# spaceandtimefdn/blitzar

Measured on NVIDIA H100. Metric: MSM throughput (scalar*point terms/sec), ristretto255, n=2^20 per GPU, higher is better.
Workload: dtype u32 limbs (integer modular arithmetic)

## Files before the change

### blitzar_b200/api.py

```python
import ctypes as C
import os

import numpy as np

_HERE = os.path.dirname(os.path.abspath(__file__))
LIB_PATH = os.path.join(_HERE, "lib", "libblitzar_b200.so")

SXT_CPU_BACKEND, SXT_GPU_BACKEND = 1, 2
SXT_CURVE_RISTRETTO255, SXT_CURVE_BLS_381, SXT_CURVE_BN_254, SXT_CURVE_GRUMPKIN = 0, 1, 2, 3
CURVE_SIZES = {0: (160, 160, 32), 1: (144, 104, 48), 2: (96, 72, 72), 3: (96, 72, 72)}
COMPACT_BYTES = {0: 120, 1: 96, 2: 64, 3: 64}

SXT_SYMBOLS = [
    "sxt_init", "sxt_curve25519_compute_pedersen_commitments",
    "sxt_curve25519_compute_pedersen_commitments_with_generators",
    "sxt_bls12_381_g1_compute_pedersen_commitments_with_generators",
    "sxt_bn254_g1_uncompressed_compute_pedersen_commitments_with_generators",
    "sxt_grumpkin_uncompressed_compute_pedersen_commitments_with_generators",
    "sxt_ristretto255_get_generators", "sxt_curve25519_get_one_commit",
    "sxt_curve25519_prove_inner_product", "sxt_curve25519_verify_inner_product",
    "sxt_multiexp_handle_new", "sxt_multiexp_handle_new_from_file",
    "sxt_multiexp_handle_write_to_file", "sxt_multiexp_handle_free",
    "sxt_fixed_multiexponentiation", "sxt_fixed_packed_multiexponentiation",
    "sxt_fixed_vlen_multiexponentiation", "sxt_prove_sumcheck",
]
B200_SYMBOLS = [
    "b200_set_device", "b200_launch_count", "b200_point_bytes", "b200_malloc", "b200_free",
    "b200_memcpy_h2d", "b200_memcpy_d2h", "b200_synchronize", "b200_event_create",
    "b200_event_record", "b200_event_elapsed_ms", "b200_event_destroy", "b200_commit_device",
    "b200_combine_partials_device", "b200_fixed_msm_device",
    "b200_combine_partials_projective_device", "b200_set_tuning", "b200_profile_accumulate",
    "b200_profile_read", "b200_set_reduce_groups", "b200_stream",
    "b200_synthetic_generators_device", "b200_commit_host_partials",
    "b200_fixed_msm_host_partials", "b200_multiexp_handle_new_device",
    "b200_selftest_lane_arithmetic", "b200_field_op", "b200_selftest_sort",
    "b200_partition_table_device",
    "b200_multiexp_handle_write_partition_table",
    "b200_compute_pedersen_commitments_with_offsets", "b200_commit_device_with_offsets",
    "b200_multiexp_handle_add_partition_table", "b200_multiexp_handle_partition_window",
    "b200_curve25519_prove_inner_products", "b200_curve25519_verify_inner_products",
]


class sxt_config(C.Structure):
    _fields_ = [("backend", C.c_int), ("num_precomputed_generators", C.c_uint64)]


class sxt_sequence_descriptor(C.Structure):
    _fields_ = [("element_nbytes", C.c_uint8), ("n", C.c_uint64), ("data", C.c_void_p),
                ("is_signed", C.c_int)]


_lib = None


def lib():
    global _lib
    if _lib is None:
        if not os.path.exists(LIB_PATH):
            raise RuntimeError(f"{LIB_PATH} is missing: run `python -m blitzar_b200.build` "
                               "(blitzar_b200 has no CPU fallback)")
        L = C.CDLL(LIB_PATH)
        L.sxt_init.restype = C.c_int
        L.sxt_ristretto255_get_generators.restype = C.c_int
        L.sxt_curve25519_get_one_commit.restype = C.c_int
        L.sxt_multiexp_handle_new.restype = C.c_void_p
        L.sxt_multiexp_handle_new_from_file.restype = C.c_void_p
        L.b200_launch_count.restype = C.c_ulonglong
        L.b200_point_bytes.restype = C.c_uint
        L.b200_malloc.restype = C.c_void_p
        L.b200_multiexp_handle_new_device.restype = C.c_void_p
        L.b200_event_create.restype = C.c_void_p
        L.b200_stream.restype = C.c_void_p
        L.b200_event_elapsed_ms.restype = C.c_float
        _lib = L
    return _lib


_initialized = False


def sxt_init(backend=SXT_GPU_BACKEND, num_precomputed_generators=0, device=None):
    global _initialized
    if _initialized:
        return 0
    if device is not None:
        lib().b200_set_device(C.c_int(device))
    cfg = sxt_config(backend, num_precomputed_generators)
    rc = lib().sxt_init(C.byref(cfg))
    if rc == 0:
        _initialized = True
    return rc


def make_descriptors(columns, device_ptrs=None):
    arr = (sxt_sequence_descriptor * max(1, len(columns)))()
    keep = []
    for i, (data, is_signed) in enumerate(columns):
        data = np.ascontiguousarray(data, dtype=np.uint8)
        keep.append(data)
        arr[i].element_nbytes = data.shape[1]
        arr[i].n = data.shape[0]
        if device_ptrs is not None:
            arr[i].data = device_ptrs[i]
        else:
            arr[i].data = data.ctypes.data if data.shape[0] else None
        arr[i].is_signed = int(is_signed)
    return arr, keep


def _ptr(a):
    return C.c_void_p(a.ctypes.data) if a is not None else C.c_void_p(None)


def compute_pedersen_commitments(curve_id, columns, generators=None, offset_generators=0):
    L = lib()
    desc, keep = make_descriptors(columns)
    out = np.zeros((len(columns), CURVE_SIZES[curve_id][2]), dtype=np.uint8)
    num = C.c_uint32(len(columns))
    if curve_id == SXT_CURVE_RISTRETTO255:
        if generators is None:
            L.sxt_curve25519_compute_pedersen_commitments(_ptr(out), num, desc,
                                                          C.c_uint64(offset_generators))
        else:
            L.sxt_curve25519_compute_pedersen_commitments_with_generators(_ptr(out), num, desc,
                                                                          _ptr(generators))
    else:
        fn = {1: L.sxt_bls12_381_g1_compute_pedersen_commitments_with_generators,
              2: L.sxt_bn254_g1_uncompressed_compute_pedersen_commitments_with_generators,
              3: L.sxt_grumpkin_uncompressed_compute_pedersen_commitments_with_generators}[curve_id]
        fn(_ptr(out), num, desc, _ptr(generators))
    return out


def _offsets(offsets, num):
    if offsets is None:
        return None
    offsets = np.ascontiguousarray(offsets, dtype=np.uint64)
    if offsets.shape != (num,):
        raise ValueError(f"offsets must hold one entry per column ({num})")
    return offsets


def compute_pedersen_commitments_with_offsets(curve_id, columns, offsets, generators=None):
    desc, keep = make_descriptors(columns)
    offsets = _offsets(offsets, len(columns))
    out = np.zeros((len(columns), CURVE_SIZES[curve_id][2]), dtype=np.uint8)
    lib().b200_compute_pedersen_commitments_with_offsets(
        C.c_uint(curve_id), _ptr(out), C.c_uint32(len(columns)), desc, _ptr(generators),
        _ptr(offsets))
    return out


def get_generators(num_generators, offset_generators=0):
    out = np.zeros((num_generators, 160), dtype=np.uint8)
    rc = lib().sxt_ristretto255_get_generators(_ptr(out), C.c_uint64(num_generators),
                                               C.c_uint64(offset_generators))
    if rc != 0:
        raise RuntimeError("sxt_ristretto255_get_generators failed")
    return out


def get_one_commit(n):
    out = np.zeros((1, 160), dtype=np.uint8)
    rc = lib().sxt_curve25519_get_one_commit(_ptr(out), C.c_uint64(n))
    if rc != 0:
        raise RuntimeError("sxt_curve25519_get_one_commit failed")
    return out


class MultiexpHandle:

    def __init__(self, curve_id, generators=None, filename=None, device_ptr=None, n=None):
        self.curve_id = curve_id
        if device_ptr is not None:
            self.h = lib().b200_multiexp_handle_new_device(C.c_uint(curve_id),
                                                           C.c_void_p(device_ptr), C.c_uint(n))
        elif filename is not None:
            self.h = lib().sxt_multiexp_handle_new_from_file(C.c_uint(curve_id),
                                                             filename.encode())
        else:
            generators = np.ascontiguousarray(generators, dtype=np.uint8)
            self.h = lib().sxt_multiexp_handle_new(C.c_uint(curve_id), _ptr(generators),
                                                   C.c_uint(generators.shape[0]))

    def write_to_file(self, filename):
        lib().sxt_multiexp_handle_write_to_file(C.c_void_p(self.h), filename.encode())

    def write_partition_table(self, filename, window_width=0):
        lib().b200_multiexp_handle_write_partition_table(C.c_void_p(self.h), filename.encode(),
                                                         C.c_uint(window_width))

    def add_partition_table(self, window_width=0):
        return int(lib().b200_multiexp_handle_add_partition_table(C.c_void_p(self.h),
                                                                  C.c_uint(window_width)))

    @property
    def partition_window(self):
        return int(lib().b200_multiexp_handle_partition_window(C.c_void_p(self.h)))

    def free(self):
        if self.h:
            lib().sxt_multiexp_handle_free(C.c_void_p(self.h))
            self.h = None

    def _res(self, num_outputs):
        return np.zeros((num_outputs, CURVE_SIZES[self.curve_id][0]), dtype=np.uint8)

    def fixed_multiexponentiation(self, element_num_bytes, num_outputs, n, scalars):
        res = self._res(num_outputs)
        scalars = np.ascontiguousarray(scalars, dtype=np.uint8)
        lib().sxt_fixed_multiexponentiation(_ptr(res), C.c_void_p(self.h),
                                            C.c_uint(element_num_bytes), C.c_uint(num_outputs),
                                            C.c_uint(n), _ptr(scalars))
        return res

    def fixed_packed_multiexponentiation(self, output_bit_table, n, scalars):
        num_outputs = len(output_bit_table)
        res = self._res(num_outputs)
        bt = (C.c_uint * num_outputs)(*output_bit_table)
        scalars = np.ascontiguousarray(scalars, dtype=np.uint8)
        lib().sxt_fixed_packed_multiexponentiation(_ptr(res), C.c_void_p(self.h), bt,
                                                   C.c_uint(num_outputs), C.c_uint(n),
                                                   _ptr(scalars))
        return res

    def fixed_vlen_multiexponentiation(self, output_bit_table, output_lengths, scalars):
        num_outputs = len(output_bit_table)
        res = self._res(num_outputs)
        bt = (C.c_uint * num_outputs)(*output_bit_table)
        ol = (C.c_uint * num_outputs)(*output_lengths)
        scalars = np.ascontiguousarray(scalars, dtype=np.uint8)
        lib().sxt_fixed_vlen_multiexponentiation(_ptr(res), C.c_void_p(self.h), bt, ol,
                                                 C.c_uint(num_outputs), _ptr(scalars))
        return res


class DeviceBuffer:
    def __init__(self, nbytes=None, host=None):
        if host is not None:
            host = np.ascontiguousarray(host)
            nbytes = host.nbytes
        self.nbytes = nbytes
        self.ptr = lib().b200_malloc(C.c_uint64(max(nbytes, 16)))
        if host is not None and nbytes:
            lib().b200_memcpy_h2d(C.c_void_p(self.ptr), _ptr(host), C.c_uint64(nbytes))

    def to_host(self, shape=None, dtype=np.uint8):
        out = np.zeros(self.nbytes, dtype=np.uint8)
        lib().b200_memcpy_d2h(_ptr(out), C.c_void_p(self.ptr), C.c_uint64(self.nbytes))
        out = out.view(dtype)
        return out.reshape(shape) if shape is not None else out

    def free(self):
        if self.ptr:
            lib().b200_free(C.c_void_p(self.ptr))
            self.ptr = None


class Event:
    def __init__(self):
        self.e = lib().b200_event_create()

    def record(self):
        lib().b200_event_record(C.c_void_p(self.e))

    def elapsed_ms(self, stop):
        return float(lib().b200_event_elapsed_ms(C.c_void_p(self.e), C.c_void_p(stop.e)))


def commit_device(curve_id, columns_shape, scalar_ptrs, generators_ptr, out_commit_ptr=None,
                  out_partial_ptr=None, offset_generators=0):
    num = len(columns_shape)
    arr = (sxt_sequence_descriptor * max(1, num))()
    for i, (n, nbytes, is_signed) in enumerate(columns_shape):
        arr[i].element_nbytes = nbytes
        arr[i].n = n
        arr[i].data = scalar_ptrs[i]
        arr[i].is_signed = int(is_signed)
    lib().b200_commit_device(C.c_uint(curve_id), C.c_void_p(out_commit_ptr),
                             C.c_void_p(out_partial_ptr), C.c_uint32(num), arr,
                             C.c_void_p(generators_ptr), C.c_uint64(offset_generators))


def commit_device_with_offsets(curve_id, columns_shape, scalar_ptrs, generators_ptr, offsets,
                               out_commit_ptr=None, out_partial_ptr=None):
    num = len(columns_shape)
    arr = (sxt_sequence_descriptor * max(1, num))()
    for i, (n, nbytes, is_signed) in enumerate(columns_shape):
        arr[i].element_nbytes = nbytes
        arr[i].n = n
        arr[i].data = scalar_ptrs[i]
        arr[i].is_signed = int(is_signed)
    offsets = _offsets(offsets, num)
    lib().b200_commit_device_with_offsets(C.c_uint(curve_id), C.c_void_p(out_commit_ptr),
                                          C.c_void_p(out_partial_ptr), C.c_uint32(num), arr,
                                          C.c_void_p(generators_ptr), _ptr(offsets))


def selftest_lane_arithmetic(warps=64, seed=1):
    lib().b200_selftest_lane_arithmetic.restype = C.c_uint
    return int(lib().b200_selftest_lane_arithmetic(C.c_uint(warps), C.c_uint(seed)))


FIELD_LIMBS = {0: 8, 1: 12, 2: 8, 3: 8, 4: 8, 5: 10}
FIELD_OPS = {name: code for code, name in enumerate([
    "add", "sub", "neg", "dbl", "mul", "mul_ref", "sqr", "mul_lat", "canonical", "is_negative",
    "invert", "pow22523", "from_radix51", "to_radix51", "sqrt_ratio_m1", "invert_eea", "from_mont",
    "to_mont", "lexicographically_largest", "carry1", "sub2p", "sub4p", "slice", "gather"])}
_BINARY_OPS = {"add", "sub", "mul", "mul_ref", "mul_lat", "sqrt_ratio_m1", "sub2p", "sub4p"}


def field_op_shape(field, op):
    n = FIELD_LIMBS[field]
    a = {"from_radix51": 10, "slice": 8}.get(op, n)
    out = {"is_negative": 1, "lexicographically_largest": 1, "to_radix51": 10,
           "sqrt_ratio_m1": n + 1, "gather": 8}.get(op, n)
    return a, (n if op in _BINARY_OPS else 0), out


def call_field_op(entry, field, op, a, b=None):
    wa, wb, wout = field_op_shape(field, op)
    a = np.ascontiguousarray(a, dtype=np.uint32).reshape(-1, wa)
    n = a.shape[0]
    if wb:
        b = np.ascontiguousarray(b, dtype=np.uint32).reshape(n, wb)
    out = np.zeros((n, wout), dtype=np.uint32)
    entry.restype = C.c_uint
    rc = entry(C.c_uint(field), C.c_uint(FIELD_OPS[op]), C.c_uint64(n), _ptr(a),
               _ptr(b if wb else None), _ptr(out))
    if rc == 0xFFFFFFFF:
        raise ValueError(f"field {field} does not offer {op}")
    return out


def field_op(field, op, a, b=None):
    return call_field_op(lib().b200_field_op, field, op, a, b)


def selftest_sort(columns_shape, scalar_ptrs, window_bits=0):
    num = len(columns_shape)
    arr = (sxt_sequence_descriptor * max(1, num))()
    for i, (n, nbytes, is_signed) in enumerate(columns_shape):
        arr[i].element_nbytes = nbytes
        arr[i].n = n
        arr[i].data = scalar_ptrs[i]
        arr[i].is_signed = int(is_signed)
    lib().b200_selftest_sort.restype = C.c_uint
    return int(lib().b200_selftest_sort(arr, C.c_uint(num), C.c_uint(window_bits)))


def synthetic_generators_device(curve_id, out_ptr, n, first=0, projective=False):
    lib().b200_synthetic_generators_device(C.c_uint(curve_id), C.c_void_p(out_ptr), C.c_uint64(n),
                                           C.c_uint64(first), C.c_int(1 if projective else 0))


def partition_table_bytes(curve_id, n, window_width):
    return -(-n // window_width) * (COMPACT_BYTES[curve_id] << window_width)


def partition_table_device(curve_id, out_ptr, gens_ptr, n, window_width=0):
    lib().b200_partition_table_device(C.c_uint(curve_id), C.c_void_p(out_ptr), C.c_void_p(gens_ptr),
                                      C.c_uint64(n), C.c_uint(window_width))


def synthetic_generators(curve_id, n, first=0, projective=False):
    stride = CURVE_SIZES[curve_id][0 if (projective or curve_id == 0) else 1]
    buf = DeviceBuffer(n * stride)
    synthetic_generators_device(curve_id, buf.ptr, n, first, projective)
    out = buf.to_host((n, stride))
    buf.free()
    return out


def commit_host_partials(curve_id, columns, generators, out_partial_ptr, offset_generators=0):
    desc, keep = make_descriptors(columns)
    lib().b200_commit_host_partials(C.c_uint(curve_id), C.c_void_p(out_partial_ptr),
                                    C.c_uint32(len(columns)), desc, _ptr(generators),
                                    C.c_uint64(offset_generators))


def fixed_msm_device(handle, out_res_ptr, out_partial_ptr, element_num_bytes, num_outputs, n,
                     scalars_ptr, bit_table=None, lengths=None):
    mode, bt, ol = 0, None, None
    if bit_table is not None:
        if len(bit_table) != num_outputs or (lengths is not None and len(lengths) != num_outputs):
            raise ValueError(f"bit_table and lengths must hold one entry per output ({num_outputs})")
        mode = 1 if lengths is None else 2
        bt = (C.c_uint * num_outputs)(*bit_table)
        ol = None if lengths is None else (C.c_uint * num_outputs)(*lengths)
    elif lengths is not None:
        raise ValueError("lengths need a bit_table")
    lib().b200_fixed_msm_device(C.c_void_p(out_res_ptr), C.c_void_p(out_partial_ptr),
                                C.c_void_p(handle.h), C.c_int(mode), C.c_uint(element_num_bytes),
                                bt, ol, C.c_uint(num_outputs), C.c_uint(n),
                                C.c_void_p(scalars_ptr))


def fixed_msm_host_partials(handle, out_partial_ptr, element_num_bytes, num_outputs, n, scalars):
    lib().b200_fixed_msm_host_partials(C.c_void_p(out_partial_ptr), C.c_void_p(handle.h),
                                       C.c_int(0), C.c_uint(element_num_bytes), None, None,
                                       C.c_uint(num_outputs), C.c_uint(n), _ptr(scalars))


def combine_partials_projective_device(curve_id, out_ptr, partials_ptr, num_parts, count):
    lib().b200_combine_partials_projective_device(C.c_uint(curve_id), C.c_void_p(out_ptr),
                                                  C.c_void_p(partials_ptr), C.c_uint32(num_parts),
                                                  C.c_uint32(count))


def synchronize():
    lib().b200_synchronize()


def launch_count():
    return int(lib().b200_launch_count())


def profile_accumulate(enable):
    lib().b200_profile_accumulate(C.c_int(1 if enable else 0))


def profile_read():
    ms, cnt = C.c_float(0), C.c_uint(0)
    lib().b200_profile_read(C.byref(ms), C.byref(cnt))
    return float(ms.value), int(cnt.value)


def set_tuning(window_bits=0, chunk1=0, chunkn=0):
    lib().b200_set_tuning(C.c_uint(window_bits), C.c_uint(chunk1), C.c_uint(chunkn))


def combine_partials_device(curve_id, out_ptr, partials_ptr, num_parts, count):
    lib().b200_combine_partials_device(C.c_uint(curve_id), C.c_void_p(out_ptr),
                                       C.c_void_p(partials_ptr), C.c_uint32(num_parts),
                                       C.c_uint32(count))


def point_bytes(curve_id):
    return int(lib().b200_point_bytes(C.c_uint(curve_id)))


def set_reduce_groups(g1=0, gn=0):
    lib().b200_set_reduce_groups(C.c_uint(g1), C.c_uint(gn))


def stream_ptr():
    return int(lib().b200_stream())


def prove_inner_product(transcript, a, b, generators_offset=0):
    n = a.shape[0]
    rounds = max(0, (n - 1).bit_length())
    lv = np.zeros((max(rounds, 1), 32), dtype=np.uint8)
    rv = np.zeros((max(rounds, 1), 32), dtype=np.uint8)
    ap = np.zeros(32, dtype=np.uint8)
    a = np.ascontiguousarray(a, dtype=np.uint8)
    b = np.ascontiguousarray(b, dtype=np.uint8)
    lib().sxt_curve25519_prove_inner_product(_ptr(lv), _ptr(rv), _ptr(ap), _ptr(transcript),
                                             C.c_uint64(n), C.c_uint64(generators_offset),
                                             _ptr(a), _ptr(b))
    return lv[:rounds], rv[:rounds], ap


def verify_inner_product(transcript, b, product, a_commit, l_vector, r_vector, ap_value,
                         generators_offset=0):
    n = b.shape[0]
    b = np.ascontiguousarray(b, dtype=np.uint8)
    lv = np.ascontiguousarray(l_vector if len(l_vector) else np.zeros((1, 32), np.uint8))
    rv = np.ascontiguousarray(r_vector if len(r_vector) else np.zeros((1, 32), np.uint8))
    lib().sxt_curve25519_verify_inner_product.restype = C.c_int
    return int(lib().sxt_curve25519_verify_inner_product(
        _ptr(transcript), C.c_uint64(n), C.c_uint64(generators_offset), _ptr(b),
        _ptr(np.ascontiguousarray(product)), _ptr(np.ascontiguousarray(a_commit)), _ptr(lv),
        _ptr(rv), _ptr(np.ascontiguousarray(ap_value))))


def _ipa_batch_inputs(vectors, offsets):
    n = np.array([v.shape[0] for v in vectors], dtype=np.uint64)
    offs = np.zeros(len(vectors), np.uint64) if offsets is None else \
        np.ascontiguousarray(offsets, dtype=np.uint64)
    if offs.shape != n.shape:
        raise ValueError("one generators offset per proof")
    flat = np.ascontiguousarray(np.concatenate([np.asarray(v, np.uint8).reshape(-1, 32)
                                                for v in vectors])) if len(vectors) else \
        np.zeros((1, 32), np.uint8)
    rounds = [max(0, (int(m) - 1).bit_length()) for m in n]
    return n, offs, flat, rounds


def prove_inner_products(transcripts, a_list, b_list, offsets=None):
    return call_prove_inner_products(lib().b200_curve25519_prove_inner_products, transcripts,
                                     a_list, b_list, offsets)


def verify_inner_products(transcripts, b_list, products, a_commits, l_list, r_list, ap_values,
                          offsets=None):
    lib().b200_curve25519_verify_inner_products.restype = C.c_uint32
    return call_verify_inner_products(lib().b200_curve25519_verify_inner_products, transcripts,
                                      b_list, products, a_commits, l_list, r_list, ap_values,
                                      offsets)


def call_prove_inner_products(entry, transcripts, a_list, b_list, offsets=None):
    if len(a_list) != len(b_list) or any(a.shape[0] != b.shape[0] for a, b in zip(a_list, b_list)):
        raise ValueError("a_list and b_list must hold vectors of equal lengths")
    if transcripts.shape != (len(a_list), 203) or not transcripts.flags.c_contiguous:
        raise ValueError("transcripts must be a contiguous uint8 [P, 203] array")
    n, offs, a, rounds = _ipa_batch_inputs(a_list, offsets)
    _, _, b, _ = _ipa_batch_inputs(b_list, offsets)
    nk = sum(rounds)
    lv = np.zeros((max(nk, 1), 32), dtype=np.uint8)
    rv = np.zeros((max(nk, 1), 32), dtype=np.uint8)
    ap = np.zeros((max(len(a_list), 1), 32), dtype=np.uint8)
    entry(C.c_uint32(len(a_list)), _ptr(lv), _ptr(rv), _ptr(ap), _ptr(transcripts), _ptr(n),
          _ptr(offs), _ptr(a), _ptr(b))
    out, k0 = [], 0
    for p, k in enumerate(rounds):
        out.append((lv[k0:k0 + k], rv[k0:k0 + k], ap[p]))
        k0 += k
    return out


def call_verify_inner_products(entry, transcripts, b_list, products, a_commits, l_list, r_list,
                               ap_values, offsets=None):
    P = len(b_list)
    if transcripts.shape != (P, 203) or not transcripts.flags.c_contiguous:
        raise ValueError("transcripts must be a contiguous uint8 [P, 203] array")
    n, offs, b, _ = _ipa_batch_inputs(b_list, offsets)
    lrs = [np.concatenate([np.asarray(v, np.uint8).reshape(-1, 32) for v in vs] +
                          [np.zeros((1, 32), np.uint8)]) for vs in (l_list, r_list)]
    results = np.zeros(max(P, 1), dtype=np.int32)
    entry(C.c_uint32(P), _ptr(results), _ptr(transcripts), _ptr(n), _ptr(offs), _ptr(b),
          _ptr(np.ascontiguousarray(products, np.uint8)),
          _ptr(np.ascontiguousarray(a_commits, np.uint8)), _ptr(np.ascontiguousarray(lrs[0])),
          _ptr(np.ascontiguousarray(lrs[1])), _ptr(np.ascontiguousarray(ap_values, np.uint8)))
    return results[:P]
```

### blitzar_b200/csrc/api.cu

```cuda
#include <algorithm>
#include <cctype>
#include <cstdint>
#include <cstdio>
#include <cstdlib>
#include <cstring>
#include <condition_variable>
#include <functional>
#include <mutex>
#include <thread>
#include <memory>
#include <string>
#include <vector>

#include "engine_api.cuh"

using namespace b200;

namespace {

struct State {
  bool initialized = false;
  int device = -1;
  cudaStream_t stream = nullptr;
  cudaStream_t copy_stream = nullptr;
  cudaStream_t tail_stream = nullptr;
  cudaEvent_t range_events[16] = {};
  cudaEvent_t alloc_event = nullptr;
  void* builtin = nullptr;
  uint64_t num_builtin = 0;
  unsigned builtin_window_bits = 0, builtin_windows = 0;
  MsmOptions opt;
};
State g_state;
EngineCtx ctx_of(const State& st) {
  EngineCtx c{st.stream, g_state.opt, st.builtin, st.num_builtin};
  c.builtin_window_bits = st.builtin_window_bits;
  c.builtin_windows = st.builtin_windows;
  static const bool tail_on = [] {
    const char* env = std::getenv("BLITZAR_B200_TAIL_STREAM");
    return env != nullptr && std::atoi(env) != 0;
  }();
  if (tail_on)
    c.tail = st.tail_stream;
  if (const char* env = std::getenv("BLITZAR_B200_GROUP_ENTRIES"))
    c.opt.max_group_entries = std::strtoull(env, nullptr, 10);
  if (const char* env = std::getenv("BLITZAR_B200_UNIFORM_ADD"))
    c.opt.uniform_add = (u32)std::atoi(env);
  if (const char* env = std::getenv("BLITZAR_B200_LANE_TAIL"))
    c.opt.lane_tail = (u32)std::atoi(env);
  if (const char* env = std::getenv("BLITZAR_B200_SCATTER_WM"))
    c.opt.scatter_window_major = (u32)std::atoi(env);
  if (const char* env = std::getenv("BLITZAR_B200_SORT"))
    c.opt.sort_path = (u32)std::atoi(env);
  if (const char* env = std::getenv("BLITZAR_B200_NORMALIZE_GENS"))
    c.opt.normalize_gens = (u32)std::atoi(env);
  if (const char* env = std::getenv("BLITZAR_B200_PAIR_LEVELS"))
    c.opt.pair_levels = std::atoi(env);
  if (const char* env = std::getenv("BLITZAR_B200_PAIR_BATCH"))
    c.opt.pair_batch = (u32)std::atoi(env);
  if (const char* env = std::getenv("BLITZAR_B200_TABLE_POLICY"))
    c.opt.table_policy = (u32)std::atoi(env);
  if (const char* env = std::getenv("BLITZAR_B200_PARTITION_POLICY"))
    c.partition_policy = (u32)std::atoi(env);
  return c;
}
EngineCtx ctx() { return ctx_of(g_state); }
std::mutex g_mutex;

void init_device_state(State& st) {
  B200_CUDA(cudaSetDevice(st.device));
  B200_CUDA(cudaStreamCreateWithFlags(&st.stream, cudaStreamNonBlocking));
  B200_CUDA(cudaStreamCreateWithFlags(&st.copy_stream, cudaStreamNonBlocking));
  int prio_low = 0, prio_high = 0;
  B200_CUDA(cudaDeviceGetStreamPriorityRange(&prio_low, &prio_high));
  B200_CUDA(cudaStreamCreateWithPriority(&st.tail_stream, cudaStreamNonBlocking, prio_high));
  for (auto& e : st.range_events)
    B200_CUDA(cudaEventCreateWithFlags(&e, cudaEventDisableTiming));
  B200_CUDA(cudaEventCreateWithFlags(&st.alloc_event, cudaEventDisableTiming));
  cudaMemPool_t pool;
  B200_CUDA(cudaDeviceGetDefaultMemPool(&pool, st.device));
  uint64_t threshold = UINT64_MAX;
  B200_CUDA(cudaMemPoolSetAttribute(pool, cudaMemPoolAttrReleaseThreshold, &threshold));
}

void ensure_device() {
  if (g_state.stream)
    return;
  int count = 0;
  cudaError_t e = cudaGetDeviceCount(&count);
  if (e != cudaSuccess || count == 0)
    die("no supported GPUs found (this library has no CPU fallback)", __FILE__, __LINE__);
  if (g_state.device < 0) {
    const char* env = std::getenv("BLITZAR_B200_DEVICE");
    if (env)
      g_state.device = std::atoi(env);
    else
      B200_CUDA(cudaGetDevice(&g_state.device));
  }
  init_device_state(g_state);
}

unsigned choose_table_window(uint64_t n, size_t gen_bytes) {
  if (const char* env = std::getenv("BLITZAR_B200_TABLE_WINDOW")) {
    const int c = std::atoi(env);
    if (c <= 0)
      return 0;
    const unsigned cc = (unsigned)std::min(22, std::max(8, c));
    return (uint64_t)(256 / cc + 1) * n < (1ull << 31) ? cc : 0;
  }
  size_t free_b = 0, total_b = 0;
  B200_CUDA(cudaMemGetInfo(&free_b, &total_b));
  return table_window_bits(n, gen_bytes, 0.4 * (double)free_b);
}

void make_builtin_table(State& st, uint64_t np) {
  const CurveVTable& V = kVTableEd25519;
  const unsigned c = choose_table_window(np, V.gen_bytes);
  const unsigned windows = c ? 256 / c + 1 : 1;
  B200_CUDA(cudaMalloc(&st.builtin, (size_t)np * windows * V.gen_bytes));
  EngineCtx cx = ctx_of(st);
  launch_builtin_generators(cx, st.builtin, 0, np);
  V.build_table(cx, st.builtin, np, c, windows);
  stream_sync(st.stream);
  st.num_builtin = np;
  st.builtin_window_bits = c;
  st.builtin_windows = windows;
}

void require_init(const char* fn) {
  if (!g_state.initialized) {
    std::fprintf(stderr, "blitzar_b200: backend uninitialized in `%s`\n", fn);
    std::abort();
  }
  B200_CUDA(cudaSetDevice(g_state.device));
}
struct Entry {
  std::lock_guard<std::mutex> lock{g_mutex};
  explicit Entry(const char* fn) { require_init(fn); }
};


class HostStager {
public:
  static HostStager& get() {
    static thread_local HostStager s;
    return s;
  }
  void copy(void* dst_dev, const void* src_host, size_t bytes, cudaStream_t sc) {
    if (bytes == 0)
      return;
    cudaPointerAttributes attr;
    bool pinned = cudaPointerGetAttributes(&attr, src_host) == cudaSuccess &&
                  (attr.type == cudaMemoryTypeHost || attr.type == cudaMemoryTypeManaged);
    cudaGetLastError();
    static const bool enabled = [] {
      const char* env = std::getenv("BLITZAR_B200_STAGER");
      return env == nullptr || std::atoi(env) != 0;
    }();
    if (!enabled || pinned || bytes < (1u << 20)) {
      B200_CUDA(cudaMemcpyAsync(dst_dev, src_host, bytes, cudaMemcpyHostToDevice, sc));
      return;
    }
    init();
    const unsigned char* src = static_cast<const unsigned char*>(src_host);
    unsigned char* dst = static_cast<unsigned char*>(dst_dev);
    for (size_t off = 0; off < bytes; off += kChunk) {
      const size_t len = std::min(kChunk, bytes - off);
      const int slot = next_++ % kSlots;
      B200_CUDA(cudaEventSynchronize(done_[slot]));
      parallel_memcpy(staging_[slot], src + off, len);
      B200_CUDA(cudaMemcpyAsync(dst + off, staging_[slot], len, cudaMemcpyHostToDevice, sc));
      B200_CUDA(cudaEventRecord(done_[slot], sc));
    }
  }

private:
  static constexpr size_t kChunk = 8u << 20;
  static constexpr int kSlots = 4;
  const int kWorkers = [] {
    const char* env = std::getenv("BLITZAR_B200_STAGER_THREADS");
    const int v = env ? std::atoi(env) : 4;
    return std::max(1, std::min(32, v));
  }();
  unsigned char* staging_[kSlots] = {};
  cudaEvent_t done_[kSlots] = {};
  unsigned next_ = 0;
  bool ready_ = false;
  std::vector<std::thread> workers_;
  std::mutex m_;
  std::condition_variable cv_work_, cv_done_;
  struct Job {
    void* d;
    const void* s;
    size_t n;
  };
  std::vector<Job> jobs_;
  int pending_ = 0;
  bool stop_ = false;

  void init() {
    if (ready_)
      return;
    for (int i = 0; i < kSlots; ++i) {
      B200_CUDA(cudaHostAlloc((void**)&staging_[i], kChunk, cudaHostAllocDefault));
      B200_CUDA(cudaEventCreateWithFlags(&done_[i], cudaEventDisableTiming));
    }
    for (int w = 0; w < kWorkers - 1; ++w)
      workers_.emplace_back([this] { worker(); });
    ready_ = true;
  }
  void worker() {
    for (;;) {
      Job j;
      {
        std::unique_lock<std::mutex> lk(m_);
        cv_work_.wait(lk, [this] { return stop_ || !jobs_.empty(); });
        if (stop_ && jobs_.empty())
          return;
        j = jobs_.back();
        jobs_.pop_back();
      }
      std::memcpy(j.d, j.s, j.n);
      {
        std::lock_guard<std::mutex> lk(m_);
        if (--pending_ == 0)
          cv_done_.notify_all();
      }
    }
  }
  void parallel_memcpy(void* d, const void* s, size_t n) {
    const size_t slice = (n + kWorkers - 1) / kWorkers;
    size_t own = std::min(slice, n);
    {
      std::lock_guard<std::mutex> lk(m_);
      for (size_t off = own; off < n; off += slice) {
        jobs_.push_back(Job{(char*)d + off, (const char*)s + off, std::min(slice, n - off)});
        ++pending_;
      }
    }
    cv_work_.notify_all();
    std::memcpy(d, s, own);
    std::unique_lock<std::mutex> lk(m_);
    cv_done_.wait(lk, [this] { return pending_ == 0; });
  }
  ~HostStager() {
    {
      std::lock_guard<std::mutex> lk(m_);
      stop_ = true;
    }
    cv_work_.notify_all();
    for (auto& t : workers_)
      t.join();
    for (int i = 0; i < kSlots; ++i) {
      if (staging_[i])
        cudaFreeHost(staging_[i]);
      if (done_[i])
        cudaEventDestroy(done_[i]);
    }
  }
};

struct RangeWaitState {
  uint64_t n;
  uint32_t num_ranges;
  int skew;
  const State* st;
  uint32_t uploaded;
  std::function<void(uint32_t)> upload;
};
void wait_for_range(void* user, uint64_t begin, uint64_t end) {
  auto* w = static_cast<RangeWaitState*>(user);
  for (uint32_t r = 0; r < w->num_ranges; ++r) {
    const uint64_t rb = range_begin(w->n, r, w->num_ranges, w->skew);
    const uint64_t re = range_begin(w->n, r + 1, w->num_ranges, w->skew);
    if (rb < end && begin < re) {
      while (w->uploaded <= std::min(r + 1, w->num_ranges - 1))
        w->upload(w->uploaded++);
      B200_CUDA(cudaStreamWaitEvent(w->st->stream, w->st->range_events[r], 0));
    }
  }
}

void commit_on(const State& st, unsigned curve_id, void* commitments, uint32_t num,
               const sxt_sequence_descriptor* d, const void* generators,
               uint64_t offset_generators, void* out_partials_dev = nullptr,
               const uint64_t* offsets = nullptr) {
  const CurveVTable& V = curve_vtable(curve_id);
  StageRange nvtx("commit (host buffers)");
  cudaStream_t s = st.stream, sc = st.copy_stream;
  const uint64_t n = check_descriptors(d, num);
  size_t total_scalar_bytes = 0;
  for (uint32_t i = 0; i < num; ++i)
    total_scalar_bytes += (size_t)d[i].n * d[i].element_nbytes + 32;
  const GenLayout layout(d, num, offsets);
  DevBuf<unsigned char> raw_gens(generators ? layout.total * V.abi_gen_bytes : 1, s);
  DevBuf<unsigned char> scal(total_scalar_bytes, s);
  DevBuf<unsigned char> out((size_t)num * V.abi_commit_bytes, s);
  std::vector<sxt_sequence_descriptor> dd(d, d + num);
  std::vector<size_t> col_off(num);
  size_t off = 0;
  for (uint32_t i = 0; i < num; ++i) {
    col_off[i] = off;
    dd[i].data = scal.p + off;
    off += ((size_t)d[i].n * d[i].element_nbytes + 31) & ~(size_t)31;
  }
  uint32_t num_ranges = (uint32_t)std::min<uint64_t>(n >> 18, num == 1 ? 8 : 4);
  if (num == 1 && n >= (1ull << 18))
    num_ranges = std::max(num_ranges, 2u);
  if (curve_id != SXT_CURVE_RISTRETTO255)
    num_ranges = (uint32_t)std::min<uint64_t>(n >> 21, 4);
  num_ranges = std::max(num_ranges, 1u);
  if (const char* env = std::getenv("BLITZAR_B200_RANGES"))
    num_ranges = (uint32_t)std::max(1, std::min(16, std::atoi(env)));
  int skew = 0;
  if (const char* env = std::getenv("BLITZAR_B200_RANGE_SKEW"))
    skew = std::atoi(env);
  B200_CUDA(cudaEventRecord(st.alloc_event, s));
  B200_CUDA(cudaStreamWaitEvent(sc, st.alloc_event, 0));
  static const bool trace = std::getenv("BLITZAR_B200_TRACE") != nullptr;
  std::vector<cudaEvent_t> tev;
  auto mark = [&](cudaStream_t on) {
    if (!trace)
      return;
    cudaEvent_t e;
    B200_CUDA(cudaEventCreate(&e));
    B200_CUDA(cudaEventRecord(e, on));
    tev.push_back(e);
  };
  mark(sc);
  auto upload = [&](uint32_t r) {
    const uint64_t b = range_begin(n, r, num_ranges, skew), e = range_begin(n, r + 1, num_ranges, skew);
    for (uint32_t i = 0; i < num; ++i) {
      const uint64_t lo = std::min<uint64_t>(b, d[i].n), hi = std::min<uint64_t>(e, d[i].n);
      HostStager::get().copy(scal.p + col_off[i] + lo * d[i].element_nbytes,
                             d[i].data + lo * d[i].element_nbytes,
                             (hi - lo) * d[i].element_nbytes, sc);
    }
    if (generators)
      for (const GenLayout::Piece& p : layout.needed(b, e))
        HostStager::get().copy(raw_gens.p + p.pos * V.abi_gen_bytes,
                               static_cast<const unsigned char*>(generators) + p.src * V.abi_gen_bytes,
                               p.count * V.abi_gen_bytes, sc);
    B200_CUDA(cudaEventRecord(st.range_events[r], sc));
    mark(sc);
  };
  B200_LOG(2, "commit: curve %u, %u columns, n = %llu, device %d, %u upload pieces, generators %s",
           curve_id, num, (unsigned long long)n, st.device, num_ranges,
           generators ? "from the caller" : "built in");
  RangeWaitState w{n, num_ranges, skew, &st, 0, upload};
  EngineCtx cx = ctx_of(st);
  cx.opt.range_skew = skew;
  if (offsets)
    V.commit_device_offsets(cx, out_partials_dev ? nullptr : out.p, out_partials_dev, num, dd.data(),
                            generators ? raw_gens.p : nullptr, offsets, true, num_ranges,
                            &wait_for_range, &w);
  else
    V.commit_device(cx, out_partials_dev ? nullptr : out.p, out_partials_dev, num, dd.data(),
                    generators ? raw_gens.p : nullptr, offset_generators, num_ranges, &wait_for_range,
                    &w);
  mark(s);
  if (!out_partials_dev)
    copy_d2h(commitments, out.p, (size_t)num * V.abi_commit_bytes, s);
  stream_sync(s);
  if (trace) {
    std::fprintf(stderr, "blitzar_b200 trace: n=%llu cols=%u pieces=%u:", (unsigned long long)n, num,
                 num_ranges);
    for (size_t i = 1; i < tev.size(); ++i) {
      float ms = 0;
      B200_CUDA(cudaEventElapsedTime(&ms, tev[0], tev[i]));
      std::fprintf(stderr, " %s%.3f", i + 1 == tev.size() ? "compute_done=" : "upload=", ms);
    }
    std::fprintf(stderr, " ms\n");
    for (auto e : tev)
      cudaEventDestroy(e);
  }
}

class Worker {
public:
  State st;
  explicit Worker(int device) {
    st.device = device;
    th_ = std::thread([this] { run(); });
  }
  void submit(std::function<void()> f) {
    {
      std::lock_guard<std::mutex> lk(m_);
      task_ = std::move(f);
      busy_ = true;
    }
    cv_.notify_all();
  }
  void wait() {
    std::unique_lock<std::mutex> lk(m_);
    cv_.wait(lk, [this] { return !busy_; });
  }
  ~Worker() {
    {
      std::lock_guard<std::mutex> lk(m_);
      stop_ = true;
    }
    cv_.notify_all();
    if (th_.joinable())
      th_.join();
  }

private:
  std::thread th_;
  std::mutex m_;
  std::condition_variable cv_;
  std::function<void()> task_;
  bool busy_ = false, stop_ = false;
  void run() {
    B200_CUDA(cudaSetDevice(st.device));
    for (;;) {
      std::function<void()> f;
      {
        std::unique_lock<std::mutex> lk(m_);
        cv_.wait(lk, [this] { return stop_ || task_; });
        if (stop_ && !task_)
          return;
        f = std::move(task_);
        task_ = nullptr;
      }
      f();
      {
        std::lock_guard<std::mutex> lk(m_);
        busy_ = false;
      }
      cv_.notify_all();
    }
  }
};
std::vector<std::unique_ptr<Worker>> g_workers;

struct Gather {
  void* buf = nullptr;
  size_t capacity = 0;
  void* ensure(size_t bytes) {
    if (bytes > capacity) {
      if (buf) {
        B200_CUDA(cudaStreamSynchronize(g_state.stream));
        B200_CUDA(cudaFree(buf));
      }
      capacity = std::max<size_t>(bytes, 1u << 16);
      B200_CUDA(cudaMalloc(&buf, capacity));
    }
    return buf;
  }
};
Gather g_gather;

size_t range_parts(uint64_t n) {
  static const uint64_t min_terms = [] {
    const char* env = std::getenv("BLITZAR_B200_MIN_SHARD_TERMS");
    return env ? std::strtoull(env, nullptr, 10) : (1ull << 15);
  }();
  return (size_t)std::max<uint64_t>(1, std::min<uint64_t>(g_workers.size() + 1, n / std::max<uint64_t>(min_terms, 1)));
}
State& state_of(size_t part) { return part == 0 ? g_state : g_workers[part - 1]->st; }
template <class F> void on_devices(size_t parts, F f) {
  for (size_t p = 1; p < parts; ++p)
    g_workers[p - 1]->submit([=] { f(p); });
  f(0);
  for (size_t p = 1; p < parts; ++p)
    g_workers[p - 1]->wait();
  B200_CUDA(cudaSetDevice(g_state.device));
}
template <class F>
void sum_over_devices(const CurveVTable& V, size_t parts, uint32_t count, void* sum, F run) {
  const size_t bytes = (size_t)count * V.point_bytes;
  unsigned char* gather = static_cast<unsigned char*>(g_gather.ensure(parts * bytes));
  on_devices(parts, [&](size_t p) {
    const State& st = state_of(p);
    DevBuf<unsigned char> partials(bytes, st.stream);
    run(st, p, partials.p);
    if (p == 0)
      B200_CUDA(cudaMemcpyAsync(gather, partials.p, bytes, cudaMemcpyDeviceToDevice, st.stream));
    else
      B200_CUDA(cudaMemcpyPeerAsync(gather + p * bytes, g_state.device, partials.p, st.device, bytes,
                                    st.stream));
    B200_CUDA(cudaStreamSynchronize(st.stream));
  });
  V.sum_parts(ctx(), gather, (uint32_t)parts, count, sum);
}
void store_to_host(const CurveVTable& V, const void* pts, uint32_t count, bool commit, void* host) {
  cudaStream_t s = g_state.stream;
  const size_t bytes = (size_t)count * (commit ? V.abi_commit_bytes : V.abi_proj_bytes);
  DevBuf<unsigned char> out(bytes, s);
  V.store(ctx(), pts, out.p, count, commit);
  copy_d2h(host, out.p, bytes, s);
  stream_sync(s);
}
void combine_partials(unsigned curve_id, void* out_dev, const void* partials, uint32_t num_parts,
                      uint32_t count, bool commit) {
  const CurveVTable& V = curve_vtable(curve_id);
  DevBuf<unsigned char> sum((size_t)count * V.point_bytes, g_state.stream);
  V.sum_parts(ctx(), partials, num_parts, count, sum.p);
  V.store(ctx(), sum.p, out_dev, count, commit);
}

void commit_host(unsigned curve_id, void* commitments, uint32_t num,
                 const sxt_sequence_descriptor* d, const void* generators,
                 uint64_t offset_generators, const char* fn, void* out_partials_dev = nullptr,
                 const uint64_t* offsets = nullptr) {
  if (num == 0)
    return;
  const Entry entry(fn);
  B200_REQUIRE(commitments != nullptr || out_partials_dev != nullptr, "commitments == nullptr");
  const uint64_t n = check_descriptors(d, num);
  if (curve_id != SXT_CURVE_RISTRETTO255)
    B200_REQUIRE(generators != nullptr, "generators == nullptr");
  if (offsets)
    (void)GenLayout(d, num, offsets);
  const CurveVTable& V = curve_vtable(curve_id);
  const size_t stride = V.abi_commit_bytes;
  const size_t devices = g_workers.size() + 1;
  if (devices <= 1 || out_partials_dev) {
    commit_on(g_state, curve_id, commitments, num, d, generators, offset_generators,
              out_partials_dev, offsets);
    return;
  }
  if (num >= devices) {
    const size_t parts = devices;
    std::vector<uint64_t> prefix(num + 1, 0);
    for (uint32_t i = 0; i < num; ++i)
      prefix[i + 1] = prefix[i] + d[i].n * d[i].element_nbytes + 1;
    std::vector<uint32_t> cut(parts + 1, num);
    cut[0] = 0;
    for (size_t p = 1; p < parts; ++p) {
      uint32_t c = cut[p - 1] + 1;
      while (c < num - (parts - p) && prefix[c] * parts < prefix[num] * p)
        ++c;
      cut[p] = c;
    }
    on_devices(parts, [&, curve_id, commitments, d, generators, offset_generators](size_t p) {
      commit_on(state_of(p), curve_id, static_cast<unsigned char*>(commitments) + cut[p] * stride,
                cut[p + 1] - cut[p], d + cut[p], generators, offset_generators, nullptr,
                offsets ? offsets + cut[p] : nullptr);
    });
    return;
  }
  const size_t parts = range_parts(n);
  if (parts <= 1) {
    commit_on(g_state, curve_id, commitments, num, d, generators, offset_generators, nullptr,
              offsets);
    return;
  }
  DevBuf<unsigned char> sum((size_t)num * V.point_bytes, g_state.stream);
  sum_over_devices(V, parts, num, sum.p, [&](const State& st, size_t p, void* partials) {
    const uint64_t lo = n * p / parts, hi = n * (p + 1) / parts;
    std::vector<sxt_sequence_descriptor> dd(d, d + num);
    std::vector<uint64_t> part_offsets(offsets ? num : 0);
    for (uint32_t j = 0; j < num; ++j) {
      auto& c = dd[j];
      const uint64_t b = std::min<uint64_t>(lo, c.n), e = std::min<uint64_t>(hi, c.n);
      c.data = c.data ? c.data + b * c.element_nbytes : nullptr;
      c.n = e - b;
      if (offsets)
        part_offsets[j] = offsets[j] + b;
    }
    const unsigned char* g = static_cast<const unsigned char*>(generators);
    if (offsets)
      commit_on(st, curve_id, nullptr, num, dd.data(), g, 0, partials, part_offsets.data());
    else
      commit_on(st, curve_id, nullptr, num, dd.data(), g ? g + lo * V.abi_gen_bytes : nullptr,
                offset_generators + lo, partials);
  });
  store_to_host(V, sum.p, num, true, commitments);
}

struct HandleSet {
  unsigned curve_id = 0, n = 0;
  std::vector<Handle*> shards;
  std::vector<unsigned> first;
};
HandleSet* handle_of(const sxt_multiexp_handle* handle) {
  B200_REQUIRE(handle != nullptr, "null handle");
  return reinterpret_cast<HandleSet*>(const_cast<sxt_multiexp_handle*>(handle));
}

Handle* shard_new(const State& st, unsigned curve_id, const void* generators, unsigned n,
                  bool device_resident, unsigned compact_window, size_t compact_bytes) {
  const CurveVTable& V = curve_vtable(curve_id);
  cudaStream_t s = st.stream;
  Handle* h = new Handle{curve_id, n, nullptr};
  h->window_bits = choose_table_window(n, V.gen_bytes);
  h->windows = h->window_bits ? 256 / h->window_bits + 1 : 1;
  B200_CUDA(cudaMalloc(&h->gens, (size_t)(n ? n : 1) * h->windows * V.gen_bytes));
  if (n) {
    B200_REQUIRE(generators != nullptr, "generators == nullptr");
    const EngineCtx cx = ctx_of(st);
    if (compact_window) {
      DevBuf<unsigned char> raw(compact_bytes, s);
      HostStager::get().copy(raw.p, generators, compact_bytes, s);
      V.ingest_compact_table(cx, raw.p, compact_window, h->gens, n);
    } else if (device_resident) {
      V.ingest_projective(cx, generators, h->gens, n);
    } else {
      DevBuf<unsigned char> raw((size_t)n * V.abi_proj_bytes, s);
      HostStager::get().copy(raw.p, generators, (size_t)n * V.abi_proj_bytes, s);
      V.ingest_projective(cx, raw.p, h->gens, n);
    }
    V.build_table(cx, h->gens, n, h->window_bits, h->windows);
    stream_sync(s);
  }
  return h;
}

unsigned partition_window(unsigned w) {
  if (w == 0) {
    const char* env = std::getenv("BLITZAR_PARTITION_WINDOW_WIDTH");
    w = env ? (unsigned)std::strtoul(env, nullptr, 10) : 16u;
  }
  B200_REQUIRE(w >= 1 && w <= 24, "partition table window width must be in 1..24");
  return w;
}
uint64_t partition_chunk_groups(const CurveVTable& V, unsigned w) {
  uint64_t bytes = 64ull << 20;
  if (const char* env = std::getenv("BLITZAR_B200_PTABLE_CHUNK_BYTES"))
    bytes = std::strtoull(env, nullptr, 10);
  return std::max<uint64_t>(1, bytes / ((uint64_t)V.abi_compact_bytes << w));
}
void drop_partition_table(const State& st, Handle* h) {
  stream_sync(st.stream);
  B200_CUDA(cudaFree(h->ptable));
  h->ptable = nullptr;
  h->ptable_w = 0;
  h->ptable_groups = 0;
}
bool shard_add_partition_table(const State& st, Handle* h, unsigned w) {
  const CurveVTable& V = curve_vtable(h->curve_id);
  cudaStream_t s = st.stream;
  drop_partition_table(st, h);
  const uint64_t groups = ((uint64_t)h->n + w - 1) / w;
  if (groups == 0)
    return false;
  size_t free_b = 0, total_b = 0;
  B200_CUDA(cudaMemGetInfo(&free_b, &total_b));
  const double bytes = std::ldexp((double)groups * V.gen_bytes, (int)w);
  if (bytes > 0.4 * (double)free_b)
    return false;
  if (cudaMalloc(&h->ptable, (size_t)bytes) != cudaSuccess) {
    cudaGetLastError();
    h->ptable = nullptr;
    return false;
  }
  const uint64_t step = partition_chunk_groups(V, w);
  for (uint64_t g = 0; g < groups; g += step)
    V.partition_gens(ctx_of(st), h->gens, h->n, w, g, std::min(step, groups - g),
                     static_cast<unsigned char*>(h->ptable) + ((size_t)g << w) * V.gen_bytes);
  stream_sync(s);
  h->ptable_w = w;
  h->ptable_groups = groups;
  return true;
}

unsigned handle_add_partition_table(HandleSet* hs, unsigned window_width) {
  const unsigned w = partition_window(window_width);
  std::vector<char> ok(hs->shards.size(), 0);
  on_devices(hs->shards.size(), [&, hs, w](size_t p) {
    ok[p] = shard_add_partition_table(state_of(p), hs->shards[p], w) ? 1 : 0;
  });
  if (std::find(ok.begin(), ok.end(), 0) == ok.end())
    return w;
  on_devices(hs->shards.size(),
             [hs](size_t p) { drop_partition_table(state_of(p), hs->shards[p]); });
  B200_LOG(1, "partition table of width %u does not fit in 40 %% of the free HBM", w);
  return 0;
}

HandleSet* handle_new(unsigned curve_id, const void* generators, unsigned n,
                      bool device_resident = false, unsigned compact_window = 0) {
  const CurveVTable& V = curve_vtable(curve_id);
  HandleSet* hs = new HandleSet;
  hs->curve_id = curve_id;
  hs->n = n;
  size_t parts = device_resident ? 1 : range_parts(n);
  const unsigned align = compact_window ? compact_window : 1;
  hs->shards.assign(parts, nullptr);
  hs->first.assign(parts + 1, n);
  for (size_t p = 0; p < parts; ++p)
    hs->first[p] = (unsigned)(((uint64_t)n * p / parts) / align * align);
  on_devices(parts, [&, curve_id, generators, device_resident, compact_window](size_t p) {
    const unsigned lo = hs->first[p], cnt = hs->first[p + 1] - lo;
    const unsigned char* g = static_cast<const unsigned char*>(generators);
    size_t off = 0, cbytes = 0;
    if (compact_window) {
      const size_t group_bytes = (size_t)V.abi_compact_bytes << compact_window;
      off = (size_t)(lo / compact_window) * group_bytes;
      cbytes = (size_t)((cnt + compact_window - 1) / compact_window) * group_bytes;
    } else {
      off = (size_t)lo * V.abi_proj_bytes;
    }
    hs->shards[p] = shard_new(state_of(p), curve_id, g ? g + off : nullptr, cnt, device_resident,
                              compact_window, cbytes);
  });
  if (const char* env = std::getenv("BLITZAR_B200_PARTITION_HANDLES"))
    if (std::atoi(env) == 1)
      handle_add_partition_table(hs, 0);
  return hs;
}

struct FixedCall {
  int mode;
  unsigned element_num_bytes;
  const unsigned* bit_table;
  const unsigned* lengths;
  unsigned num_outputs, rows;
  uint64_t row_bytes;
};

void fixed_on(const State& st, void* res, const Handle* h, const FixedCall& c, unsigned lo,
              const uint8_t* scalars, void* out_partials_dev) {
  cudaStream_t s = st.stream;
  const CurveVTable& V = curve_vtable(h->curve_id);
  const unsigned hi = std::min<uint64_t>((uint64_t)lo + h->n, c.rows);
  const unsigned rows = hi > lo ? hi - lo : 0;
  std::vector<unsigned> lens;
  if (c.mode == 2) {
    lens.resize(c.num_outputs);
    for (unsigned j = 0; j < c.num_outputs; ++j)
      lens[j] = c.lengths[j] > lo ? std::min(c.lengths[j] - lo, rows) : 0u;
  }
  const size_t bytes = (size_t)c.row_bytes * rows;
  DevBuf<unsigned char> scal(bytes + 64, s);
  DevBuf<unsigned char> out((size_t)c.num_outputs * V.abi_proj_bytes, s);
  HostStager::get().copy(scal.p, scalars + (size_t)c.row_bytes * lo, bytes, s);
  V.fixed_device(ctx_of(st), out_partials_dev ? nullptr : out.p, out_partials_dev, h, c.mode,
                 c.element_num_bytes, c.bit_table, c.mode == 2 ? lens.data() : nullptr,
                 c.num_outputs, rows, scal.p);
  if (!out_partials_dev)
    copy_d2h(res, out.p, (size_t)c.num_outputs * V.abi_proj_bytes, s);
  stream_sync(s);
}

void fixed_host(void* res, const HandleSet* hs, int mode, unsigned element_num_bytes,
                const unsigned* bit_table, const unsigned* lengths, unsigned num_outputs,
                unsigned n, const uint8_t* scalars, void* out_partials_dev = nullptr) {
  if (num_outputs == 0)
    return;
  FixedCall c{mode, element_num_bytes, bit_table, lengths, num_outputs, n,
              fixed_row_bytes(mode, element_num_bytes, bit_table, num_outputs)};
  if (mode == 2) {
    for (unsigned j = 1; j < num_outputs; ++j)
      B200_REQUIRE(lengths[j] >= lengths[j - 1], "output lengths must be sorted in ascending order");
    c.rows = lengths[num_outputs - 1];
  }
  B200_REQUIRE(c.rows <= hs->n, "more scalars than generators in the handle");
  B200_REQUIRE(c.row_bytes * c.rows == 0 || scalars != nullptr, "scalars == nullptr");
  const size_t parts = hs->shards.size();
  if (parts == 1) {
    fixed_on(g_state, res, hs->shards[0], c, 0, scalars, out_partials_dev);
    return;
  }
  const CurveVTable& V = curve_vtable(hs->curve_id);
  auto shard = [&](const State& st, size_t p, void* partials) {
    fixed_on(st, nullptr, hs->shards[p], c, hs->first[p], scalars, partials);
  };
  if (out_partials_dev) {
    sum_over_devices(V, parts, num_outputs, out_partials_dev, shard);
    stream_sync(g_state.stream);
    return;
  }
  DevBuf<unsigned char> sum((size_t)num_outputs * V.point_bytes, g_state.stream);
  sum_over_devices(V, parts, num_outputs, sum.p, shard);
  store_to_host(V, sum.p, num_outputs, false, res);
}

const uint32_t kHandleMagic = 0x44483242u;

}

extern "C" {

int sxt_init(const struct sxt_config* config) {
  std::lock_guard<std::mutex> lock(g_mutex);
  if (config == nullptr)
    die("config input to `sxt_init` is null", __FILE__, __LINE__);
  if (g_state.initialized)
    die("trying to reinitialize the backend in `sxt_init`", __FILE__, __LINE__);
  int backend = config->backend;
  if (const char* env = std::getenv("BLITZAR_BACKEND")) {
    std::string v(env);
    for (auto& ch : v)
      ch = (char)std::tolower(ch);
    if (v == "cpu")
      backend = SXT_CPU_BACKEND;
    else if (v == "gpu")
      backend = SXT_GPU_BACKEND;
    else
      die("invalid BLITZAR_BACKEND value", __FILE__, __LINE__);
  }
  if (backend == SXT_CPU_BACKEND) {
    std::fprintf(stderr, "blitzar_b200: this library provides only the gpu backend "
                         "(SXT_GPU_BACKEND); link the reference libblitzar for the cpu backend\n");
    return 2;
  }
  if (backend != SXT_GPU_BACKEND)
    return 1;
  ensure_device();
  g_state.initialized = true;
  uint64_t np = config->num_precomputed_generators;
  if (np)
    make_builtin_table(g_state, np);
  if (const char* env = std::getenv("BLITZAR_B200_DEVICES")) {
    int want = std::atoi(env), count = 0;
    B200_CUDA(cudaGetDeviceCount(&count));
    const char* shared = std::getenv("BLITZAR_B200_SHARED_DEVICES");
    if (!(shared && std::atoi(shared) != 0))
      want = std::min(want, count);
    for (int k = 1; k < want; ++k) {
      auto w = std::make_unique<Worker>((g_state.device + k) % count);
      Worker* wp = w.get();
      wp->submit([wp, np] {
        init_device_state(wp->st);
        if (np)
          make_builtin_table(wp->st, np);
        wp->st.initialized = true;
      });
      wp->wait();
      g_workers.push_back(std::move(w));
    }
    B200_CUDA(cudaSetDevice(g_state.device));
  }
  return 0;
}

void sxt_curve25519_compute_pedersen_commitments(struct sxt_ristretto255_compressed* commitments,
                                                 uint32_t num_sequences,
                                                 const struct sxt_sequence_descriptor* descriptors,
                                                 uint64_t offset_generators) {
  commit_host(SXT_CURVE_RISTRETTO255, commitments, num_sequences, descriptors, nullptr,
              offset_generators, "sxt_curve25519_compute_pedersen_commitments");
}
void sxt_curve25519_compute_pedersen_commitments_with_generators(
    struct sxt_ristretto255_compressed* commitments, uint32_t num_sequences,
    const struct sxt_sequence_descriptor* descriptors, const struct sxt_ristretto255* generators) {
  commit_host(SXT_CURVE_RISTRETTO255, commitments, num_sequences, descriptors, generators, 0,
              "sxt_curve25519_compute_pedersen_commitments_with_generators");
}
void sxt_bls12_381_g1_compute_pedersen_commitments_with_generators(
    struct sxt_bls12_381_g1_compressed* commitments, uint32_t num_sequences,
    const struct sxt_sequence_descriptor* descriptors, const struct sxt_bls12_381_g1* generators) {
  commit_host(SXT_CURVE_BLS_381, commitments, num_sequences, descriptors, generators, 0,
              "sxt_bls12_381_g1_compute_pedersen_commitments_with_generators");
}
void sxt_bn254_g1_uncompressed_compute_pedersen_commitments_with_generators(
    struct sxt_bn254_g1* commitments, uint32_t num_sequences,
    const struct sxt_sequence_descriptor* descriptors, const struct sxt_bn254_g1* generators) {
  commit_host(SXT_CURVE_BN_254, commitments, num_sequences, descriptors, generators, 0,
              "sxt_bn254_g1_uncompressed_compute_pedersen_commitments_with_generators");
}
void sxt_grumpkin_uncompressed_compute_pedersen_commitments_with_generators(
    struct sxt_grumpkin* commitments, uint32_t num_sequences,
    const struct sxt_sequence_descriptor* descriptors, const struct sxt_grumpkin* generators) {
  commit_host(SXT_CURVE_GRUMPKIN, commitments, num_sequences, descriptors, generators, 0,
              "sxt_grumpkin_uncompressed_compute_pedersen_commitments_with_generators");
}

int sxt_ristretto255_get_generators(struct sxt_ristretto255* generators, uint64_t num_generators,
                                    uint64_t offset_generators) {
  const Entry entry("sxt_ristretto255_get_generators");
  if (num_generators == 0)
    return 0;
  if (generators == nullptr)
    return 1;
  const CurveVTable& V = kVTableEd25519;
  cudaStream_t s = g_state.stream;
  DevBuf<unsigned char> out(num_generators * V.abi_proj_bytes, s);
  V.synth_generators(ctx(), out.p, num_generators, offset_generators, true);
  copy_d2h(generators, out.p, num_generators * V.abi_proj_bytes, s);
  stream_sync(s);
  return 0;
}

int sxt_curve25519_get_one_commit(struct sxt_ristretto255* one_commit, uint64_t n) {
  const Entry entry("sxt_curve25519_get_one_commit");
  B200_REQUIRE(one_commit != nullptr, "one_commit == nullptr");
  B200_REQUIRE(n < (1ull << 31), "n too large");
  const CurveVTable& V = kVTableEd25519;
  cudaStream_t s = g_state.stream;
  DevBuf<unsigned char> ones(n + 32, s);
  B200_CUDA(cudaMemsetAsync(ones.p, 1, n + 32, s));
  sxt_sequence_descriptor d{1, n, ones.p, 0};
  DevBuf<unsigned char> pt(V.point_bytes, s);
  V.commit_device(ctx(), nullptr, pt.p, 1, &d, nullptr, 0, 1, nullptr, nullptr);
  store_to_host(V, pt.p, 1, false, one_commit);
  return 0;
}

void sxt_curve25519_prove_inner_product(struct sxt_ristretto255_compressed* l_vector,
                                        struct sxt_ristretto255_compressed* r_vector,
                                        struct sxt_curve25519_scalar* ap_value,
                                        struct sxt_transcript* transcript, uint64_t n,
                                        uint64_t generators_offset,
                                        const struct sxt_curve25519_scalar* a_vector,
                                        const struct sxt_curve25519_scalar* b_vector) {
  const Entry entry("sxt_curve25519_prove_inner_product");
  B200_REQUIRE(transcript != nullptr, "transcript must not be null");
  B200_REQUIRE(ap_value != nullptr, "ap_value must not be null");
  B200_REQUIRE(b_vector != nullptr && a_vector != nullptr, "a_vector / b_vector must not be null");
  B200_REQUIRE(n > 0, "a_vector and b_vector lengths must be greater than zero");
  B200_REQUIRE(n == 1 || (l_vector != nullptr && r_vector != nullptr),
               "l_vector and r_vector must not be null when n > 1");
  B200_REQUIRE(n < (1ull << 30), "n too large");
  ipa_prove(ctx(), reinterpret_cast<uint8_t*>(l_vector), reinterpret_cast<uint8_t*>(r_vector),
            ap_value->bytes, transcript->bytes, n, generators_offset,
            reinterpret_cast<const uint8_t*>(a_vector), reinterpret_cast<const uint8_t*>(b_vector));
}
int sxt_curve25519_verify_inner_product(struct sxt_transcript* transcript, uint64_t n,
                                        uint64_t generators_offset,
                                        const struct sxt_curve25519_scalar* b_vector,
                                        const struct sxt_curve25519_scalar* product,
                                        const struct sxt_ristretto255* a_commit,
                                        const struct sxt_ristretto255_compressed* l_vector,
                                        const struct sxt_ristretto255_compressed* r_vector,
                                        const struct sxt_curve25519_scalar* ap_value) {
  const Entry entry("sxt_curve25519_verify_inner_product");
  B200_REQUIRE(transcript != nullptr, "transcript must not be null");
  B200_REQUIRE(ap_value != nullptr && product != nullptr && a_commit != nullptr &&
                   b_vector != nullptr,
               "ap_value / product / a_commit / b_vector must not be null");
  B200_REQUIRE(n > 0, "b_vector length must be greater than zero");
  B200_REQUIRE(n == 1 || (l_vector != nullptr && r_vector != nullptr),
               "l_vector and r_vector must not be null when n > 1");
  B200_REQUIRE(n < (1ull << 30), "n too large");
  return ipa_verify(ctx(), transcript->bytes, n, generators_offset,
                    reinterpret_cast<const uint8_t*>(b_vector), product->bytes,
                    reinterpret_cast<const uint8_t*>(a_commit),
                    reinterpret_cast<const uint8_t*>(l_vector),
                    reinterpret_cast<const uint8_t*>(r_vector), ap_value->bytes);
}
namespace {
unsigned ipa_rounds(uint64_t n) {
  unsigned k = 0;
  while ((1ull << k) < n)
    ++k;
  return k;
}
void check_ipa_batch(uint32_t num_proofs, const uint64_t* n, const uint64_t* generators_offsets,
                     const void* transcripts, bool prover) {
  B200_REQUIRE(transcripts != nullptr && n != nullptr && generators_offsets != nullptr,
               "transcripts / n / generators_offsets must not be null");
  uint64_t arena = 0;
  for (uint32_t p = 0; p < num_proofs; ++p) {
    B200_REQUIRE(n[p] > 0, "a_vector and b_vector lengths must be greater than zero");
    B200_REQUIRE(n[p] < (1ull << 30), "n too large");
    const unsigned k = ipa_rounds(n[p]);
    arena += prover ? (1ull << k) + 1 : (1ull << k) + 2 * k + 3;
  }
  B200_REQUIRE(arena < (1ull << 31), "proofs of the batch need too many generators for one call");
}
bool any_rounds(uint32_t num_proofs, const uint64_t* n) {
  for (uint32_t p = 0; p < num_proofs; ++p)
    if (n[p] > 1)
      return true;
  return false;
}
}

void b200_curve25519_prove_inner_products(
    uint32_t num_proofs, struct sxt_ristretto255_compressed* l_vectors,
    struct sxt_ristretto255_compressed* r_vectors, struct sxt_curve25519_scalar* ap_values,
    struct sxt_transcript* transcripts, const uint64_t* n, const uint64_t* generators_offsets,
    const struct sxt_curve25519_scalar* a_vectors, const struct sxt_curve25519_scalar* b_vectors) {
  const Entry entry("b200_curve25519_prove_inner_products");
  if (num_proofs == 0)
    return;
  check_ipa_batch(num_proofs, n, generators_offsets, transcripts, true);
  B200_REQUIRE(ap_values != nullptr, "ap_values must not be null");
  B200_REQUIRE(b_vectors != nullptr && a_vectors != nullptr, "a_vectors / b_vectors must not be null");
  B200_REQUIRE(!any_rounds(num_proofs, n) || (l_vectors != nullptr && r_vectors != nullptr),
               "l_vectors and r_vectors must not be null when some n > 1");
  ipa_prove_batch(ctx(), num_proofs, reinterpret_cast<uint8_t*>(l_vectors),
                  reinterpret_cast<uint8_t*>(r_vectors), ap_values->bytes, transcripts->bytes, n,
                  generators_offsets, reinterpret_cast<const uint8_t*>(a_vectors),
                  reinterpret_cast<const uint8_t*>(b_vectors));
}
uint32_t b200_curve25519_verify_inner_products(
    uint32_t num_proofs, int* results, struct sxt_transcript* transcripts, const uint64_t* n,
    const uint64_t* generators_offsets, const struct sxt_curve25519_scalar* b_vectors,
    const struct sxt_curve25519_scalar* products, const struct sxt_ristretto255* a_commits,
    const struct sxt_ristretto255_compressed* l_vectors,
    const struct sxt_ristretto255_compressed* r_vectors,
    const struct sxt_curve25519_scalar* ap_values) {
  const Entry entry("b200_curve25519_verify_inner_products");
  if (num_proofs == 0)
    return 0;
  check_ipa_batch(num_proofs, n, generators_offsets, transcripts, false);
  B200_REQUIRE(results != nullptr, "results must not be null");
  B200_REQUIRE(ap_values != nullptr && products != nullptr && a_commits != nullptr &&
                   b_vectors != nullptr,
               "ap_values / products / a_commits / b_vectors must not be null");
  B200_REQUIRE(!any_rounds(num_proofs, n) || (l_vectors != nullptr && r_vectors != nullptr),
               "l_vectors and r_vectors must not be null when some n > 1");
  return ipa_verify_batch(ctx(), num_proofs, results, transcripts->bytes, n, generators_offsets,
                          reinterpret_cast<const uint8_t*>(b_vectors), products->bytes,
                          reinterpret_cast<const uint8_t*>(a_commits),
                          reinterpret_cast<const uint8_t*>(l_vectors),
                          reinterpret_cast<const uint8_t*>(r_vectors), ap_values->bytes);
}

void sxt_prove_sumcheck(void*, void*, unsigned, const struct sumcheck_descriptor*, void*, void*) {
  die("sxt_prove_sumcheck is not provided by blitzar_b200 (MSM hot path only)", __FILE__,
      __LINE__);
}

struct sxt_multiexp_handle* sxt_multiexp_handle_new(unsigned curve_id, const void* generators,
                                                    unsigned n) {
  const Entry entry("sxt_multiexp_handle_new");
  return reinterpret_cast<sxt_multiexp_handle*>(handle_new(curve_id, generators, n));
}

void sxt_multiexp_handle_free(struct sxt_multiexp_handle* handle) {
  if (!handle)
    return;
  std::lock_guard<std::mutex> lock(g_mutex);
  HandleSet* hs = handle_of(handle);
  on_devices(hs->shards.size(), [hs](size_t p) {
    drop_partition_table(state_of(p), hs->shards[p]);
    B200_CUDA(cudaFree(hs->shards[p]->gens));
    delete hs->shards[p];
  });
  delete hs;
}

void sxt_multiexp_handle_write_to_file(const struct sxt_multiexp_handle* handle,
                                       const char* filename) {
  const Entry entry("sxt_multiexp_handle_write_to_file");
  const HandleSet* h = handle_of(handle);
  B200_REQUIRE(filename != nullptr, "null filename");
  const CurveVTable& V = curve_vtable(h->curve_id);
  size_t bytes = (size_t)h->n * V.abi_proj_bytes;
  std::vector<unsigned char> host(bytes);
  on_devices(h->shards.size(), [&, h](size_t p) {
    const State& st = state_of(p);
    const Handle* sh = h->shards[p];
    const size_t sb = (size_t)sh->n * V.abi_proj_bytes;
    DevBuf<unsigned char> out(sb + 16, st.stream);
    V.gens_to_projective(ctx_of(st), sh->gens, out.p, sh->n);
    copy_d2h(host.data() + (size_t)h->first[p] * V.abi_proj_bytes, out.p, sb, st.stream);
    stream_sync(st.stream);
  });
  FILE* f = std::fopen(filename, "wb");
  B200_REQUIRE(f != nullptr, "cannot open handle file for writing");
  uint32_t hdr[4] = {kHandleMagic, 1u, h->curve_id, h->n};
  B200_REQUIRE(std::fwrite(hdr, sizeof(hdr), 1, f) == 1, "short write");
  B200_REQUIRE(bytes == 0 || std::fwrite(host.data(), bytes, 1, f) == 1, "short write");
  std::fclose(f);
}

struct sxt_multiexp_handle* sxt_multiexp_handle_new_from_file(unsigned curve_id,
                                                              const char* filename) {
  const Entry entry("sxt_multiexp_handle_new_from_file");
  B200_REQUIRE(filename != nullptr, "null filename");
  FILE* f = std::fopen(filename, "rb");
  B200_REQUIRE(f != nullptr, "cannot open handle file");
  uint32_t hdr[4] = {0, 0, 0, 0};
  B200_REQUIRE(std::fread(hdr, sizeof(uint32_t), 1, f) == 1, "short handle file");
  if (hdr[0] != kHandleMagic) {
    const unsigned w = hdr[0];
    const size_t esz = curve_vtable(curve_id).abi_compact_bytes;
    B200_REQUIRE(w >= 1 && w <= 24, "not a handle file (bad window width)");
    std::fseek(f, 0, SEEK_END);
    const size_t bytes = (size_t)std::ftell(f) - sizeof(uint32_t);
    std::fseek(f, sizeof(uint32_t), SEEK_SET);
    B200_REQUIRE(bytes % (esz << w) == 0, "partition table size does not match the curve");
    const size_t groups = bytes / (esz << w);
    B200_REQUIRE(groups * w < (1ull << 31), "partition table too large");
    std::vector<unsigned char> host(bytes);
    B200_REQUIRE(bytes == 0 || std::fread(host.data(), bytes, 1, f) == 1, "short handle file");
    std::fclose(f);
    return reinterpret_cast<sxt_multiexp_handle*>(
        handle_new(curve_id, host.data(), (unsigned)(groups * w), false, w));
  }
  B200_REQUIRE(std::fread(hdr + 1, 3 * sizeof(uint32_t), 1, f) == 1, "short handle file");
  B200_REQUIRE(hdr[1] == 1u, "unsupported blitzar_b200 handle file version");
  B200_REQUIRE(hdr[2] == curve_id, "handle file is for another curve");
  size_t bytes = (size_t)hdr[3] * curve_vtable(curve_id).abi_proj_bytes;
  std::vector<unsigned char> host(bytes);
  B200_REQUIRE(bytes == 0 || std::fread(host.data(), bytes, 1, f) == 1, "short handle file");
  std::fclose(f);
  return reinterpret_cast<sxt_multiexp_handle*>(handle_new(curve_id, host.data(), hdr[3]));
}

void sxt_fixed_multiexponentiation(void* res, const struct sxt_multiexp_handle* handle,
                                   unsigned element_num_bytes, unsigned num_outputs, unsigned n,
                                   const uint8_t* scalars) {
  const Entry entry("sxt_fixed_multiexponentiation");
  fixed_host(res, handle_of(handle), 0, element_num_bytes, nullptr, nullptr, num_outputs, n, scalars);
}
void sxt_fixed_packed_multiexponentiation(void* res, const struct sxt_multiexp_handle* handle,
                                          const unsigned* output_bit_table, unsigned num_outputs,
                                          unsigned n, const uint8_t* scalars) {
  const Entry entry("sxt_fixed_packed_multiexponentiation");
  fixed_host(res, handle_of(handle), 1, 0, output_bit_table, nullptr, num_outputs, n, scalars);
}
void sxt_fixed_vlen_multiexponentiation(void* res, const struct sxt_multiexp_handle* handle,
                                        const unsigned* output_bit_table,
                                        const unsigned* output_lengths, unsigned num_outputs,
                                        const uint8_t* scalars) {
  const Entry entry("sxt_fixed_vlen_multiexponentiation");
  fixed_host(res, handle_of(handle), 2, 0, output_bit_table, output_lengths, num_outputs, 0, scalars);
}

void b200_set_device(int device) {
  std::lock_guard<std::mutex> lock(g_mutex);
  B200_REQUIRE(g_state.stream == nullptr, "b200_set_device must precede sxt_init");
  g_state.device = device;
}
unsigned long long b200_launch_count(void) { return LaunchCounter::value(); }
unsigned b200_point_bytes(unsigned curve_id) { return curve_vtable(curve_id).point_bytes; }
void* b200_malloc(uint64_t bytes) {
  const Entry entry("b200_malloc");
  void* p = nullptr;
  B200_CUDA(cudaMalloc(&p, bytes ? bytes : 16));
  return p;
}
void b200_free(void* p) {
  std::lock_guard<std::mutex> lock(g_mutex);
  if (p) {
    B200_CUDA(cudaSetDevice(g_state.device));
    B200_CUDA(cudaStreamSynchronize(g_state.stream));
    B200_CUDA(cudaFree(p));
  }
}
void b200_memcpy_h2d(void* d, const void* h, uint64_t bytes) {
  const Entry entry("b200_memcpy_h2d");
  copy_h2d(d, h, bytes, g_state.stream);
  stream_sync(g_state.stream);
}
void b200_memcpy_d2h(void* h, const void* d, uint64_t bytes) {
  const Entry entry("b200_memcpy_d2h");
  copy_d2h(h, d, bytes, g_state.stream);
  stream_sync(g_state.stream);
}
void* b200_stream(void) {
  require_init("b200_stream");
  return (void*)g_state.stream;
}
void b200_synchronize(void) {
  const Entry entry("b200_synchronize");
  stream_sync(g_state.stream);
}
void* b200_event_create(void) {
  require_init("b200_event_create");
  cudaEvent_t e;
  B200_CUDA(cudaEventCreate(&e));
  return (void*)e;
}
void b200_event_record(void* e) {
  std::lock_guard<std::mutex> lock(g_mutex);
  B200_CUDA(cudaEventRecord((cudaEvent_t)e, g_state.stream));
}
float b200_event_elapsed_ms(void* a, void* b) {
  float ms = 0;
  B200_CUDA(cudaEventSynchronize((cudaEvent_t)b));
  B200_CUDA(cudaEventElapsedTime(&ms, (cudaEvent_t)a, (cudaEvent_t)b));
  return ms;
}
void b200_event_destroy(void* e) { B200_CUDA(cudaEventDestroy((cudaEvent_t)e)); }

void b200_commit_device(unsigned curve_id, void* out_commitments, void* out_partials,
                        uint32_t num_sequences, const struct sxt_sequence_descriptor* descriptors,
                        const void* generators, uint64_t offset_generators) {
  if (num_sequences == 0)
    return;
  const Entry entry("b200_commit_device");
  curve_vtable(curve_id).commit_device(ctx(), out_commitments, out_partials, num_sequences,
                                       descriptors, generators, offset_generators, 1, nullptr,
                                       nullptr);
}
void b200_compute_pedersen_commitments_with_offsets(unsigned curve_id, void* commitments,
                                                    uint32_t num_sequences,
                                                    const struct sxt_sequence_descriptor* descriptors,
                                                    const void* generators, const uint64_t* offsets) {
  commit_host(curve_id, commitments, num_sequences, descriptors, generators, 0,
              "b200_compute_pedersen_commitments_with_offsets", nullptr, offsets);
}
void b200_commit_device_with_offsets(unsigned curve_id, void* out_commitments, void* out_partials,
                                     uint32_t num_sequences,
                                     const struct sxt_sequence_descriptor* descriptors,
                                     const void* generators, const uint64_t* offsets) {
  if (num_sequences == 0)
    return;
  const Entry entry("b200_commit_device_with_offsets");
  const CurveVTable& V = curve_vtable(curve_id);
  if (offsets)
    V.commit_device_offsets(ctx(), out_commitments, out_partials, num_sequences, descriptors,
                            generators, offsets, false, 1, nullptr, nullptr);
  else
    V.commit_device(ctx(), out_commitments, out_partials, num_sequences, descriptors, generators,
                    0, 1, nullptr, nullptr);
}
void b200_commit_host_partials(unsigned curve_id, void* out_partials,
                               uint32_t num_sequences,
                               const struct sxt_sequence_descriptor* descriptors,
                               const void* generators, uint64_t offset_generators) {
  if (num_sequences == 0)
    return;
  const Entry entry("b200_commit_host_partials");
  B200_REQUIRE(out_partials != nullptr, "out_partials == nullptr");
  commit_on(g_state, curve_id, nullptr, num_sequences, descriptors, generators, offset_generators,
            out_partials);
}
void b200_fixed_msm_host_partials(void* out_partials, const struct sxt_multiexp_handle* handle,
                                  int mode, unsigned element_num_bytes,
                                  const unsigned* output_bit_table, const unsigned* output_lengths,
                                  unsigned num_outputs, unsigned n, const uint8_t* scalars) {
  if (num_outputs == 0)
    return;
  const Entry entry("b200_fixed_msm_host_partials");
  const HandleSet* h = handle_of(handle);
  B200_REQUIRE(out_partials != nullptr, "out_partials == nullptr");
  fixed_host(nullptr, h, mode, element_num_bytes, output_bit_table, output_lengths, num_outputs, n,
             scalars, out_partials);
}
struct sxt_multiexp_handle* b200_multiexp_handle_new_device(unsigned curve_id,
                                                            const void* generators_dev,
                                                            unsigned n) {
  const Entry entry("b200_multiexp_handle_new_device");
  return reinterpret_cast<sxt_multiexp_handle*>(handle_new(curve_id, generators_dev, n, true));
}
void b200_combine_partials_device(unsigned curve_id, void* out_commitments, const void* partials,
                                  uint32_t num_parts, uint32_t count) {
  const Entry entry("b200_combine_partials_device");
  combine_partials(curve_id, out_commitments, partials, num_parts, count, true);
}
void b200_combine_partials_projective_device(unsigned curve_id, void* out_res,
                                             const void* partials, uint32_t num_parts,
                                             uint32_t count) {
  const Entry entry("b200_combine_partials_projective_device");
  combine_partials(curve_id, out_res, partials, num_parts, count, false);
}
void b200_fixed_msm_device(void* out_res, void* out_partials,
                           const struct sxt_multiexp_handle* handle, int mode,
                           unsigned element_num_bytes, const unsigned* output_bit_table,
                           const unsigned* output_lengths, unsigned num_outputs, unsigned n,
                           const uint8_t* scalars) {
  if (num_outputs == 0)
    return;
  const Entry entry("b200_fixed_msm_device");
  const HandleSet* hs = handle_of(handle);
  B200_REQUIRE(hs->shards.size() == 1, "device-resident fixed MSM needs a single-device handle");
  const Handle* h = hs->shards[0];
  curve_vtable(h->curve_id).fixed_device(ctx(), out_res, out_partials, h, mode, element_num_bytes,
                                         output_bit_table, output_lengths, num_outputs, n, scalars);
}
void b200_synthetic_generators_device(unsigned curve_id, void* out_generators, uint64_t n,
                                      uint64_t first, int projective) {
  if (n == 0)
    return;
  const Entry entry("b200_synthetic_generators_device");
  B200_REQUIRE(out_generators != nullptr, "out_generators == nullptr");
  curve_vtable(curve_id).synth_generators(ctx(), out_generators, n, first, projective != 0);
}
void b200_partition_table_device(unsigned curve_id, void* out_table_dev, const void* generators_dev,
                                 uint64_t n, unsigned window_width) {
  const Entry entry("b200_partition_table_device");
  const CurveVTable& V = curve_vtable(curve_id);
  const unsigned w = partition_window(window_width);
  if (n == 0)
    return;
  B200_REQUIRE(out_table_dev != nullptr && generators_dev != nullptr,
               "out_table_dev / generators_dev must not be null");
  cudaStream_t s = g_state.stream;
  DevBuf<unsigned char> gens(n * V.gen_bytes, s);
  V.ingest_projective(ctx(), generators_dev, gens.p, n);
  const uint64_t groups = (n + w - 1) / w, step = partition_chunk_groups(V, w);
  const size_t group_bytes = (size_t)V.abi_compact_bytes << w;
  for (uint64_t g = 0; g < groups; g += step)
    V.partition_table(ctx(), gens.p, n, w, g, std::min(step, groups - g),
                      static_cast<unsigned char*>(out_table_dev) + g * group_bytes);
}
void b200_multiexp_handle_write_partition_table(const struct sxt_multiexp_handle* handle,
                                                const char* filename, unsigned window_width) {
  const Entry entry("b200_multiexp_handle_write_partition_table");
  const HandleSet* h = handle_of(handle);
  B200_REQUIRE(filename != nullptr, "null filename");
  const CurveVTable& V = curve_vtable(h->curve_id);
  const unsigned w = partition_window(window_width);
  cudaStream_t s = g_state.stream, sc = g_state.copy_stream;
  DevBuf<unsigned char> gens((size_t)(h->n ? h->n : 1) * V.gen_bytes, s);
  for (size_t p = 0; p < h->shards.size(); ++p) {
    const int device = state_of(p).device;
    const Handle* sh = h->shards[p];
    unsigned char* dst = gens.p + (size_t)h->first[p] * V.gen_bytes;
    const size_t bytes = (size_t)sh->n * V.gen_bytes;
    if (device == g_state.device)
      copy_d2d(dst, sh->gens, bytes, s);
    else if (bytes)
      B200_CUDA(cudaMemcpyPeerAsync(dst, g_state.device, sh->gens, device, bytes, s));
  }
  FILE* f = std::fopen(filename, "wb");
  B200_REQUIRE(f != nullptr, "cannot open partition table file for writing");
  const uint32_t hdr = w;
  B200_REQUIRE(std::fwrite(&hdr, sizeof(hdr), 1, f) == 1, "short write");
  const uint64_t groups = (h->n + w - 1) / w;
  const uint64_t step = std::min<uint64_t>(partition_chunk_groups(V, w), std::max<uint64_t>(groups, 1));
  const size_t group_bytes = (size_t)V.abi_compact_bytes << w, chunk_bytes = step * group_bytes;
  const uint64_t chunks = (groups + step - 1) / step;
  B200_LOG(2, "partition table file: curve %u, n = %u, w = %u, %llu chunks of %llu groups",
           h->curve_id, h->n, w, (unsigned long long)chunks, (unsigned long long)step);
  DevBuf<unsigned char> dev0(chunks ? chunk_bytes : 1, s), dev1(chunks > 1 ? chunk_bytes : 1, s);
  unsigned char* dev[2] = {dev0.p, dev1.p};
  unsigned char* host[2] = {nullptr, nullptr};
  cudaEvent_t built[2], copied[2];
  for (int k = 0; k < 2; ++k) {
    if (chunks > (uint64_t)k)
      B200_CUDA(cudaHostAlloc((void**)&host[k], chunk_bytes, cudaHostAllocDefault));
    B200_CUDA(cudaEventCreateWithFlags(&built[k], cudaEventDisableTiming));
    B200_CUDA(cudaEventCreateWithFlags(&copied[k], cudaEventDisableTiming));
  }
  auto chunk_size = [&](uint64_t i) { return std::min(step, groups - i * step) * group_bytes; };
  for (uint64_t i = 0; i <= chunks; ++i) {
    if (i < chunks) {
      const int k = (int)(i & 1);
      if (i >= 2)
        B200_CUDA(cudaStreamWaitEvent(s, copied[k], 0));
      V.partition_table(ctx(), gens.p, h->n, w, i * step, std::min(step, groups - i * step), dev[k]);
      B200_CUDA(cudaEventRecord(built[k], s));
      B200_CUDA(cudaStreamWaitEvent(sc, built[k], 0));
      copy_d2h(host[k], dev[k], chunk_size(i), sc);
      B200_CUDA(cudaEventRecord(copied[k], sc));
    }
    if (i >= 1) {
      const int k = (int)((i - 1) & 1);
      B200_CUDA(cudaEventSynchronize(copied[k]));
      B200_REQUIRE(std::fwrite(host[k], chunk_size(i - 1), 1, f) == 1, "short write");
    }
  }
  B200_REQUIRE(std::fclose(f) == 0, "short write");
  stream_sync(s);
  for (int k = 0; k < 2; ++k) {
    if (host[k])
      B200_CUDA(cudaFreeHost(host[k]));
    B200_CUDA(cudaEventDestroy(built[k]));
    B200_CUDA(cudaEventDestroy(copied[k]));
  }
}
unsigned b200_multiexp_handle_add_partition_table(struct sxt_multiexp_handle* handle,
                                                  unsigned window_width) {
  const Entry entry("b200_multiexp_handle_add_partition_table");
  return handle_add_partition_table(handle_of(handle), window_width);
}
unsigned b200_multiexp_handle_partition_window(const struct sxt_multiexp_handle* handle) {
  std::lock_guard<std::mutex> lock(g_mutex);
  const HandleSet* hs = handle_of(handle);
  return hs->shards.empty() ? 0u : hs->shards[0]->ptable_w;
}
unsigned b200_selftest_lane_arithmetic(unsigned warps, unsigned seed) {
  const Entry entry("b200_selftest_lane_arithmetic");
  return selftest_lane_arithmetic(ctx(), warps, seed);
}
unsigned b200_field_op(unsigned field, unsigned op, uint64_t n, const uint32_t* a,
                       const uint32_t* b, uint32_t* out) {
  const Entry entry("b200_field_op");
  B200_REQUIRE(n == 0 || (a != nullptr && out != nullptr), "null operand or result array");
  return field_op(ctx(), field, op, n, a, b, out);
}
unsigned b200_selftest_sort(const sxt_sequence_descriptor* columns, unsigned num,
                            unsigned window_bits) {
  const Entry entry("b200_selftest_sort");
  B200_REQUIRE(num == 0 || columns != nullptr, "columns == nullptr");
  B200_REQUIRE(window_bits <= 20, "window_bits in 0..20");
  return selftest_sort(ctx(), columns, num, window_bits);
}
void b200_set_reduce_groups(unsigned g1, unsigned gn) {
  std::lock_guard<std::mutex> lock(g_mutex);
  auto pow2 = [](unsigned v, unsigned dflt) {
    if (v < 2)
      return dflt;
    unsigned p = 2;
    while (p * 2 <= v)
      p *= 2;
    return p;
  };
  g_state.opt.reduce_g1 = pow2(g1, 16u);
  g_state.opt.reduce_gn = pow2(gn, 4u);
}
void b200_profile_accumulate(int enable) {
  std::lock_guard<std::mutex> lock(g_mutex);
  KernelTimer::get().enabled = enable != 0;
}
void b200_profile_read(float* total_ms, unsigned* launches) {
  std::lock_guard<std::mutex> lock(g_mutex);
  KernelTimer::get().read(total_ms, launches);
}
void b200_set_tuning(unsigned window_bits, unsigned chunk1, unsigned chunkn) {
  std::lock_guard<std::mutex> lock(g_mutex);
  g_state.opt.window_bits = window_bits;
  g_state.opt.chunk1 = chunk1;
  g_state.opt.chunkn = chunkn ? chunkn : 8;
}

}
```

### blitzar_b200/csrc/batch_affine.cuh

```cuda
#pragma once
#include "curve.cuh"
#include "runtime.cuh"

namespace b200 {

constexpr u32 kPadIndex = 0x7fffffffu;
B200_HD u64 make_entry(u32 key, u32 gen, bool negate) {
  return ((u64)key << 32) | (u64)((gen << 1) | (negate ? 1u : 0u));
}
B200_HD u64 pad_entry(u32 key) { return make_entry(key, kPadIndex, false); }
B200_HD u32 entry_key(u64 e) { return (u32)(e >> 32); }
B200_HD u32 entry_gen(u64 e) { return (u32)e >> 1; }
B200_HD bool entry_negate(u64 e) { return ((u32)e & 1u) != 0; }

constexpr u32 kBatchGroup = 8;
constexpr u32 kBatchTop = 4;

template <class F> struct BatchUpBody {
  static constexpr int kBlock = 128;
  const typename F::E* vals;
  typename F::E* pre;
  typename F::E* prod;
  u64 n;
  B200_HD void operator()(u64 j) const {
    const u64 b = j * kBatchGroup, e = b + kBatchGroup < n ? b + kBatchGroup : n;
    typename F::E acc = F::one();
    for (u64 i = b; i < e; ++i) {
      pre[i] = acc;
      F::mul(acc, acc, vals[i]);
    }
    prod[j] = acc;
  }
};
template <class F> struct BatchDownBody {
  static constexpr int kBlock = 128;
  typename F::E* vals;
  const typename F::E* pre;
  const typename F::E* prod;
  u64 n;
  B200_HD void operator()(u64 j) const {
    const u64 b = j * kBatchGroup, e = b + kBatchGroup < n ? b + kBatchGroup : n;
    typename F::E inv = prod[j];
    for (u64 i = e; i-- > b;) {
      typename F::E t, v = vals[i];
      F::mul(t, inv, pre[i]);
      F::mul(inv, inv, v);
      vals[i] = t;
    }
  }
};
template <class F> struct BatchTopBody {
  static constexpr int kBlock = 32;
  typename F::E* vals;
  B200_HD void operator()(u64 i) const {
    typename F::E inv;
    F::invert_eea(inv, vals[i]);
    vals[i] = inv;
  }
};
template <class F> inline void batch_invert(stream_t s, typename F::E* vals, u64 n) {
  typedef typename F::E E;
  if (n == 0)
    return;
  if (n <= kBatchTop) {
    launch(BatchTopBody<F>{vals}, n, s);
    return;
  }
  E* pre = (E*)dev_alloc(n * sizeof(E), s);
  const u64 m = (n + kBatchGroup - 1) / kBatchGroup;
  E* prod = (E*)dev_alloc(m * sizeof(E), s);
  launch(BatchUpBody<F>{vals, pre, prod, n}, m, s);
  batch_invert<F>(s, prod, m);
  launch(BatchDownBody<F>{vals, pre, prod, n}, m, s);
  dev_free(prod, s);
  dev_free(pre, s);
}

template <class C> struct PairLevel {
  typedef typename C::F F;
  typedef typename F::E fe;
  typedef typename C::Gen Gen;
  const u64* entries;
  const Gen* gens;
  const Gen* in;
  const u32* m_ptr;
  u32 level;
  u32 B;

  B200_HD u64 valid_pairs() const { return (u64)(*m_ptr) >> (level + 1); }
  B200_HD void load(Gen& a, u64 slot) const {
    if (in) {
      a = in[slot];
      return;
    }
    const u64 ent = entries[slot];
    const u32 idx = entry_gen(ent);
    if (idx == kPadIndex) {
      a.x = F::zero();
      a.y = F::zero();
      return;
    }
    a = gens[idx];
    if (entry_negate(ent) && !C::gen_is_identity(a))
      F::neg(a.y, a.y);
  }
  B200_HD int classify(fe& den, const Gen& a, const Gen& b) const {
    den = F::one();
    if (C::gen_is_identity(b))
      return 1;
    if (C::gen_is_identity(a))
      return 2;
    if (F::equal(a.x, b.x)) {
      fe s;
      F::add(s, a.y, b.y);
      if (F::is_zero(s))
        return 4;
      den = s;
      return 3;
    }
    F::sub(den, b.x, a.x);
    return 0;
  }
};

template <class C> struct PairPass1Body {
  static constexpr int kBlock = 128;
  typedef typename C::F F;
  typedef typename F::E fe;
  PairLevel<C> lv;
  fe* pre;
  fe* totals;
  u64 t0;
  B200_HD void operator()(u64 t) const {
    t += t0;
    const u64 np = lv.valid_pairs();
    const u64 b = t * lv.B, e = b + lv.B < np ? b + lv.B : np;
    fe acc = F::one();
    for (u64 p = b; p < e; ++p) {
      const u32 ia = entry_gen(lv.entries[2 * p]), ib = entry_gen(lv.entries[2 * p + 1]);
      fe den = F::one();
      if (ia != kPadIndex && ib != kPadIndex) {
        const fe xa = lv.gens[ia].x, xb = lv.gens[ib].x;
        if (F::equal(xa, xb) || F::is_zero(xa) || F::is_zero(xb)) {
          typename C::Gen ga, gb;
          lv.load(ga, 2 * p);
          lv.load(gb, 2 * p + 1);
          lv.classify(den, ga, gb);
        } else {
          F::sub(den, xb, xa);
        }
      }
      pre[p] = acc;
      F::mul(acc, acc, den);
    }
    totals[t] = acc;
  }
};

template <class C> struct PairPass2Body {
  static constexpr int kBlock = 128;
  static constexpr int kMinBlocks = C::F::N > 8 ? 2 : 3;
  typedef typename C::F F;
  typedef typename F::E fe;
  typedef typename C::Gen Gen;
  PairLevel<C> lv;
  const fe* pre;
  const fe* totals;
  Gen* out;
  fe* pre_next;
  fe* totals_next;
  u32 descending;
  u64 t0;
  B200_HD void add_pair(Gen& r, const Gen& x, const Gen& y, int kind, const fe& inv) const {
    if (kind == 1) {
      r = x;
    } else if (kind == 2) {
      r = y;
    } else if (kind == 4) {
      r.x = F::zero();
      r.y = F::zero();
    } else {
      fe num, lam, l2, dx;
      if (kind == 3) {
        fe xx;
        F::sqr(xx, x.x);
        F::add(num, xx, xx);
        F::add(num, num, xx);
      } else {
        F::sub(num, y.y, x.y);
      }
      F::mul(lam, num, inv);
      F::sqr(l2, lam);
      F::sub(l2, l2, x.x);
      F::sub(r.x, l2, y.x);
      F::sub(dx, x.x, r.x);
      F::mul(l2, lam, dx);
      F::sub(r.y, l2, x.y);
    }
  }
  B200_HD void operator()(u64 t) const {
    t += t0;
    const u64 np = lv.valid_pairs();
    const u64 b = t * lv.B, e = b + lv.B < np ? b + lv.B : np;
    if (b >= e) {
      if (pre_next)
        totals_next[t] = F::one();
      return;
    }
    const u64 cnt = e - b;
    fe inv_acc = totals[t], acc_next = F::one();
    Gen held;
    u64 p = descending ? e - 1 : b;
    Gen xn, yn;
    fe pn;
    lv.load(xn, 2 * p);
    lv.load(yn, 2 * p + 1);
    pn = pre[p];
    for (u64 k = 0; k < cnt; ++k) {
      const Gen x = xn, y = yn;
      const fe pr = pn;
      const u64 cur = p;
      if (k + 1 < cnt) {
        p = descending ? p - 1 : p + 1;
        lv.load(xn, 2 * p);
        lv.load(yn, 2 * p + 1);
        pn = pre[p];
      }
      fe den, inv;
      Gen r;
      const int kind = lv.classify(den, x, y);
      F::mul(inv, inv_acc, pr);
      F::mul(inv_acc, inv_acc, den);
      add_pair(r, x, y, kind, inv);
      out[cur] = r;
      if (pre_next) {
        const bool second = descending ? (cur & 1u) == 0 : (cur & 1u) != 0;
        if (!second) {
          held = r;
        } else {
          fe den2;
          if (descending)
            lv.classify(den2, r, held);
          else
            lv.classify(den2, held, r);
          pre_next[cur >> 1] = acc_next;
          F::mul(acc_next, acc_next, den2);
        }
      }
    }
    if (pre_next)
      totals_next[t] = acc_next;
  }
};

struct PadCountsBody {
  static constexpr int kBlock = 256;
  u32* counts;
  u32 mask;
  B200_HD void operator()(u64 k) const { counts[k] = (counts[k] + mask) & ~mask; }
};
struct FillPadsBody {
  static constexpr int kBlock = 128;
  const u32* starts;
  const u32* cursor;
  u64* entries;
  B200_HD void operator()(u64 k) const {
    const u64 pad = pad_entry((u32)k);
    for (u32 i = cursor[k]; i < starts[k + 1]; ++i)
      entries[i] = pad;
  }
};
struct FinalEntriesBody {
  static constexpr int kBlock = 256;
  const u64* entries0;
  const u32* m_ptr;
  u32 L;
  u64* entries;
  u32* m_out;
  B200_HD void operator()(u64 j) const {
    const u64 m = (u64)(*m_ptr) >> L;
    if (j == 0)
      *m_out = (u32)m;
    if (j < m)
      entries[j] = make_entry(entry_key(entries0[j << L]), (u32)j, false);
  }
};

template <class C> struct WalkInput {
  const typename C::Gen* gens;
  const u64* entries;
  const u32* m_ptr;
  u64 m_max;
};

template <class C>
WalkInput<C> run_pair_levels(stream_t s, u32 L, const u64* entries, const typename C::Gen* gens,
                             u32* d_m, u64 slots_max, u32 pair_batch) {
  typedef typename C::F F;
  typedef typename F::E fe;
  typedef typename C::Gen Gen;
  u32 B = pair_batch ? pair_batch : 32u;
  while (B < (1u << L))
    B *= 2;
  B = (B >> (L - 1)) << (L - 1);
  const u64 T = ((slots_max >> 1) + B - 1) / B;
  stream_t s2 = aux_stream();
  const u64 Ta = T / 2, Tb = T - Ta;
  const Gen* in = nullptr;
  fe* pre = (fe*)dev_alloc((slots_max >> 1) * sizeof(fe), s);
  fe* totals = (fe*)dev_alloc(T * sizeof(fe), s);
  std::vector<void*> level_bufs = {pre, totals};
  const PairLevel<C> lv0{entries, gens, nullptr, d_m, 0, B};
  launch(PairPass1Body<C>{lv0, pre, totals, 0}, Ta, s);
  stream_follow(s2, s);
  launch(PairPass1Body<C>{lv0, pre, totals, Ta}, Tb, s2);
  for (u32 l = 0; l < L; ++l) {
    const u64 npairs = slots_max >> (l + 1);
    const bool last = l + 1 == L;
    Gen* out = (Gen*)dev_alloc(npairs * sizeof(Gen), s);
    fe* pre_next = last ? nullptr : (fe*)dev_alloc((npairs >> 1) * sizeof(fe), s);
    fe* totals_next = last ? nullptr : (fe*)dev_alloc(T * sizeof(fe), s);
    level_bufs.insert(level_bufs.end(), {out, pre_next, totals_next});
    PairLevel<C> lv{l == 0 ? entries : nullptr, l == 0 ? gens : nullptr, in, d_m, l, B >> l};
    const u32 desc = (l & 1u) ? 0u : 1u;
    batch_invert<F>(s, totals, Ta);
    stream_follow(s, s2);
    launch(PairPass2Body<C>{lv, pre, totals, out, pre_next, totals_next, desc, 0}, Ta, s);
    batch_invert<F>(s2, totals + Ta, Tb);
    stream_follow(s2, s);
    launch(PairPass2Body<C>{lv, pre, totals, out, pre_next, totals_next, desc, Ta}, Tb, s2);
    in = out;
    pre = pre_next;
    totals = totals_next;
  }
  stream_follow(s, s2);
  for (void* ptr : level_bufs)
    if (ptr != (void*)in)
      dev_free(ptr, s);
  const u64 m_max = slots_max >> L;
  u64* entries_l = (u64*)dev_alloc(m_max * sizeof(u64), s);
  launch(FinalEntriesBody{entries, d_m, L, entries_l, d_m + 9}, m_max, s);
  return {in, entries_l, d_m + 9, m_max};
}

}
```

### blitzar_b200/csrc/curve_ed25519.cu

```cuda
#include "engine.cuh"
#include "field_op.cuh"
#include "ipa.cuh"
namespace b200 {
B200_DEFINE_CURVE_VTABLE(kVTableEd25519, Ed25519);

unsigned field_op_ed25519(const EngineCtx& ctx, unsigned field, unsigned op, uint64_t n,
                          const uint32_t* a, const uint32_t* b, uint32_t* out) {
  switch (field) {
  case 0: return run_field_op<F25519>(ctx, op, n, a, b, out);
  case 4: return run_field_op<FSc25>(ctx, op, n, a, b, out);
#ifdef B200_LANE_TAIL
  case 5: {
    const LaneFieldOpBody body{op, LaneFieldOpBody::shape(op), n, a, b, out};
    return run_elementwise(ctx, body, n, (n + 2) / 3 * 32, a, b, out);
  }
#endif
  default: return ~0u;
  }
}
void launch_builtin_generators(const EngineCtx& ctx, void* gens, uint64_t first, uint64_t n) {
  launch(BuiltinGeneratorBody{(Ed25519::Gen*)gens, first}, n, ctx.s);
}
unsigned selftest_lane_arithmetic(const EngineCtx& ctx, unsigned warps, unsigned seed) {
#ifdef B200_LANE_TAIL
  DevBuf<u32> bad(1, ctx.s);
  dev_zero(bad.p, sizeof(u32), ctx.s);
  launch(lane10::SelfTestBody{seed, bad.p}, (u64)warps * 32, ctx.s);
  u32 host = 0;
  copy_d2h(&host, bad.p, sizeof(u32), ctx.s);
  stream_sync(ctx.s);
  return host;
#else
  (void)ctx;
  (void)warps;
  (void)seed;
  return 0;
#endif
}
unsigned selftest_sort(const EngineCtx& ctx, const sxt_sequence_descriptor* d, unsigned num,
                       unsigned window_bits) {
  std::vector<ColumnDesc> cols(num);
  for (unsigned i = 0; i < num; ++i) {
    cols[i] = ColumnDesc{};
    cols[i].base = d[i].data;
    cols[i].row_stride = d[i].element_nbytes;
    cols[i].bit_width = 8u * d[i].element_nbytes;
    cols[i].n = (u32)d[i].n;
    cols[i].is_signed = d[i].is_signed ? 1u : 0u;
  }
  return sort_selftest(ctx.s, std::move(cols), window_bits);
}
void ipa_prove(const EngineCtx& ctx, uint8_t* l_vector, uint8_t* r_vector, uint8_t* ap_value,
               uint8_t* transcript203, uint64_t n, uint64_t generators_offset,
               const uint8_t* a_vector, const uint8_t* b_vector) {
  Ipa::prove(ctx, l_vector, r_vector, ap_value, transcript203, n, generators_offset, a_vector,
             b_vector);
}
int ipa_verify(const EngineCtx& ctx, uint8_t* transcript203, uint64_t n,
               uint64_t generators_offset, const uint8_t* b_vector, const uint8_t* product,
               const uint8_t* a_commit160, const uint8_t* l_vector, const uint8_t* r_vector,
               const uint8_t* ap_value) {
  int result = 0;
  IpaBatch::verify(ctx, 1, &result, transcript203, &n, &generators_offset, b_vector, product,
                   a_commit160, l_vector, r_vector, ap_value);
  return result;
}
void ipa_prove_batch(const EngineCtx& ctx, uint32_t num_proofs, uint8_t* l_vectors,
                     uint8_t* r_vectors, uint8_t* ap_values, uint8_t* transcripts,
                     const uint64_t* n, const uint64_t* generators_offsets,
                     const uint8_t* a_vectors, const uint8_t* b_vectors) {
  IpaBatch::prove(ctx, num_proofs, l_vectors, r_vectors, ap_values, transcripts, n,
                  generators_offsets, a_vectors, b_vectors);
}
uint32_t ipa_verify_batch(const EngineCtx& ctx, uint32_t num_proofs, int* results,
                          uint8_t* transcripts, const uint64_t* n,
                          const uint64_t* generators_offsets, const uint8_t* b_vectors,
                          const uint8_t* products, const uint8_t* a_commits,
                          const uint8_t* l_vectors, const uint8_t* r_vectors,
                          const uint8_t* ap_values) {
  return IpaBatch::verify(ctx, num_proofs, results, transcripts, n, generators_offsets, b_vectors,
                          products, a_commits, l_vectors, r_vectors, ap_values);
}
}
```

### blitzar_b200/csrc/engine_api.cuh

```cuda
#pragma once
#include <algorithm>
#include <cmath>
#include <cstdint>
#include <vector>

#include "../../include/blitzar_b200.h"
#include "runtime.cuh"

namespace b200 {

struct MsmOptions {
  u32 window_bits = 0;
  u32 chunk1 = 0;
  u32 chunkn = 8;
  u32 reduce_g1 = 16;
  u32 reduce_gn = 4;
  u64 quad_threshold = 32768;
  u64 max_group_entries = 1ull << 30;
  u64 max_range_entries = 1ull << 31;
  int pair_levels = -1;
  u32 pair_batch = 0;
  int range_skew = 0;
  u32 uniform_add = 2;
  u32 gens_normalized = 0;
  const u32* unit_veto = nullptr;
  u32 normalize_gens = 1;
  u32 lane_tail = 1;
  u32 scatter_window_major = 0;
  u32 sort_path = 1;
  u32 table_policy = 0;
};

struct EngineCtx {
  stream_t s;
  MsmOptions opt;
  const void* builtin;
  uint64_t num_builtin;
  stream_t tail = stream_t();
  u32 builtin_window_bits = 0, builtin_windows = 0;
  u32 partition_policy = 0;
};

struct Handle {
  unsigned curve_id;
  unsigned n;
  void* gens;
  unsigned window_bits = 0, windows = 1;
  void* ptable = nullptr;
  unsigned ptable_w = 0;
  uint64_t ptable_groups = 0;
};

inline unsigned table_window_bits(uint64_t n, size_t gen_bytes, double budget_bytes) {
  if (n < 1024)
    return 0;
  unsigned best = 0;
  double best_cost = 1e300;
  for (unsigned c = 10; c <= 20; ++c) {
    const double W = 256 / c + 1;
    if (W * (double)n * (double)gen_bytes > budget_bytes || W * (double)n >= 2147483648.0)
      continue;
    const double cost = W * (double)n + 2.5 * (double)(1u << (c - 1));
    if (cost < best_cost) {
      best_cost = cost;
      best = c;
    }
  }
  return best;
}

template <class T> struct DevBuf {
  T* p = nullptr;
  stream_t s;
  DevBuf(size_t count, stream_t s_) : s(s_) { p = (T*)dev_alloc(count * sizeof(T), s); }
  ~DevBuf() { dev_free(p, s); }
  DevBuf(const DevBuf&) = delete;
  DevBuf& operator=(const DevBuf&) = delete;
};

inline uint64_t range_begin(uint64_t n, uint32_t r, uint32_t num_ranges, int skew = 0) {
  if (r == 0)
    return 0;
  if (r >= num_ranges)
    return n;
  if (skew == 0 || n < 64ull * num_ranges)
    return n * r / num_ranges;
  const double t = (double)r / (double)num_ranges;
  const double f = skew > 0 ? 1.0 - (1.0 - t) * std::sqrt(1.0 - t) : t * std::sqrt(t);
  uint64_t b = (uint64_t)((double)n * f);
  const uint64_t lo = r, hi = n - (num_ranges - r);
  return b < lo ? lo : (b > hi ? hi : b);
}
typedef void (*range_wait_fn)(void* user, uint64_t begin, uint64_t end);

inline uint64_t check_descriptors(const sxt_sequence_descriptor* d, uint32_t num) {
  B200_REQUIRE(d != nullptr, "descriptors == nullptr");
  uint64_t longest = 0;
  for (uint32_t i = 0; i < num; ++i) {
    B200_REQUIRE(d[i].n == 0 || d[i].data != nullptr, "descriptor.n > 0 with data == nullptr");
    B200_REQUIRE(d[i].element_nbytes != 0 && d[i].element_nbytes <= 32,
                 "descriptor.element_nbytes must be in 1..32");
    if (d[i].is_signed)
      B200_REQUIRE(d[i].element_nbytes <= 16 &&
                       (d[i].element_nbytes & (d[i].element_nbytes - 1)) == 0,
                   "signed columns need a power-of-two element_nbytes <= 16");
    B200_REQUIRE(d[i].n < (1ull << 31), "column too long");
    longest = longest < d[i].n ? d[i].n : longest;
  }
  return longest;
}

inline uint64_t fixed_row_bytes(int mode, unsigned element_num_bytes, const unsigned* bit_table,
                                unsigned num_outputs) {
  uint64_t row_bits = 0;
  if (mode == 0) {
    B200_REQUIRE(element_num_bytes >= 1 && element_num_bytes <= 32, "element_num_bytes in 1..32");
    row_bits = 8ull * element_num_bytes * num_outputs;
  } else {
    for (unsigned j = 0; j < num_outputs; ++j) {
      B200_REQUIRE(bit_table[j] > 0 && bit_table[j] <= 256, "output bit width must be in 1..256");
      row_bits += bit_table[j];
    }
  }
  return (row_bits + 7) / 8;
}

struct GenLayout {
  struct Piece {
    uint64_t src, pos, count;
  };
  std::vector<Piece> segments;
  std::vector<uint32_t> base;
  uint64_t total = 0;
  uint64_t max_n = 0;

  GenLayout(const sxt_sequence_descriptor* d, uint32_t num, const uint64_t* offsets)
      : base(num, 0), n_(num, 0) {
    std::vector<uint32_t> order;
    for (uint32_t j = 0; j < num; ++j) {
      n_[j] = d[j].n;
      max_n = std::max<uint64_t>(max_n, d[j].n);
      if (d[j].n) {
        B200_REQUIRE(offset(offsets, j) <= ~0ull - d[j].n, "generator offset + column length overflows");
        order.push_back(j);
      }
    }
    std::stable_sort(order.begin(), order.end(), [offsets](uint32_t a, uint32_t b) {
      return offset(offsets, a) < offset(offsets, b);
    });
    for (uint32_t j : order) {
      const uint64_t lo = offset(offsets, j), hi = lo + n_[j];
      if (segments.empty() || lo > segments.back().src + segments.back().count) {
        const uint64_t pos = segments.empty() ? 0 : segments.back().pos + segments.back().count;
        segments.push_back({lo, pos, 0});
      }
      Piece& s = segments.back();
      s.count = std::max(s.count, hi - s.src);
      B200_REQUIRE(s.pos + s.count < (1ull << 31),
                   "merged generator intervals of 2^31 or more generators");
      base[j] = (uint32_t)(s.pos + (lo - s.src));
    }
    total = segments.empty() ? 0 : segments.back().pos + segments.back().count;
  }
  bool within(uint64_t limit) const {
    return segments.empty() || segments.back().src + segments.back().count <= limit;
  }
  std::vector<Piece> needed(uint64_t b, uint64_t e) const {
    std::vector<std::pair<uint64_t, uint64_t>> iv;
    for (size_t j = 0; j < base.size(); ++j)
      if (n_[j] > b)
        iv.push_back({base[j] + b, base[j] + std::min(e, n_[j])});
    std::sort(iv.begin(), iv.end());
    std::vector<Piece> out;
    size_t k = 0;
    for (auto& v : iv) {
      while (segments[k].pos + segments[k].count <= v.first)
        ++k;
      const Piece& s = segments[k];
      if (!out.empty() && out.back().pos + out.back().count >= v.first && out.back().pos >= s.pos) {
        out.back().count = std::max(out.back().count, v.second - out.back().pos);
        continue;
      }
      out.push_back({s.src + (v.first - s.pos), v.first, v.second - v.first});
    }
    return out;
  }

private:
  std::vector<uint64_t> n_;
  static uint64_t offset(const uint64_t* offsets, uint32_t j) { return offsets ? offsets[j] : 0; }
};

struct CurveVTable {
  unsigned curve_id, point_bytes, gen_bytes, abi_gen_bytes, abi_proj_bytes, abi_commit_bytes;
  void (*commit_device)(const EngineCtx&, void* out_commitments, void* out_partials, uint32_t num,
                        const sxt_sequence_descriptor* d, const void* generators_dev,
                        uint64_t offset_generators, uint32_t num_ranges, range_wait_fn wait,
                        void* wait_user);
  void (*commit_device_offsets)(const EngineCtx&, void* out_commitments, void* out_partials,
                                uint32_t num, const sxt_sequence_descriptor* d,
                                const void* generators_dev, const uint64_t* offsets, bool packed,
                                uint32_t num_ranges, range_wait_fn wait, void* wait_user);
  void (*fixed_device)(const EngineCtx&, void* out_res, void* out_partials, const Handle* h,
                       int mode, unsigned element_num_bytes, const unsigned* bit_table,
                       const unsigned* lengths, unsigned num_outputs, unsigned n,
                       const uint8_t* scalars_dev);
  void (*ingest_projective)(const EngineCtx&, const void* raw_dev, void* gens, uint64_t n);
  void (*gens_to_projective)(const EngineCtx&, const void* gens, void* out_dev, uint64_t n);
  void (*store)(const EngineCtx&, const void* pts, void* out_dev, uint64_t count, bool commit);
  void (*sum_parts)(const EngineCtx&, const void* parts, uint32_t nparts, uint32_t count,
                    void* out_pts);
  void (*synth_generators)(const EngineCtx&, void* out_dev, uint64_t n, uint64_t first,
                           bool projective);
  unsigned abi_compact_bytes;
  void (*ingest_compact_table)(const EngineCtx&, const void* table_dev, unsigned window_width,
                               void* gens, uint64_t n);
  void (*build_table)(const EngineCtx&, void* table, uint64_t n, unsigned window_bits,
                      unsigned windows);
  void (*partition_table)(const EngineCtx&, const void* gens, uint64_t n, unsigned w,
                          uint64_t first_group, uint64_t groups, void* out_dev);
  void (*partition_gens)(const EngineCtx&, const void* gens, uint64_t n, unsigned w,
                         uint64_t first_group, uint64_t groups, void* out_gens);
};
extern const CurveVTable kVTableEd25519, kVTableBls12381, kVTableBn254, kVTableGrumpkin;

inline const CurveVTable& curve_vtable(unsigned curve_id) {
  switch (curve_id) {
  case SXT_CURVE_RISTRETTO255:
    return kVTableEd25519;
  case SXT_CURVE_BLS_381:
    return kVTableBls12381;
  case SXT_CURVE_BN_254:
    return kVTableBn254;
  case SXT_CURVE_GRUMPKIN:
    return kVTableGrumpkin;
  default:
    die("unsupported curve id", __FILE__, __LINE__);
  }
}

void ipa_prove(const EngineCtx& ctx, uint8_t* l_vector, uint8_t* r_vector, uint8_t* ap_value,
               uint8_t* transcript203, uint64_t n, uint64_t generators_offset,
               const uint8_t* a_vector, const uint8_t* b_vector);
int ipa_verify(const EngineCtx& ctx, uint8_t* transcript203, uint64_t n,
               uint64_t generators_offset, const uint8_t* b_vector, const uint8_t* product,
               const uint8_t* a_commit160, const uint8_t* l_vector, const uint8_t* r_vector,
               const uint8_t* ap_value);
void ipa_prove_batch(const EngineCtx& ctx, uint32_t num_proofs, uint8_t* l_vectors,
                     uint8_t* r_vectors, uint8_t* ap_values, uint8_t* transcripts,
                     const uint64_t* n, const uint64_t* generators_offsets,
                     const uint8_t* a_vectors, const uint8_t* b_vectors);
uint32_t ipa_verify_batch(const EngineCtx& ctx, uint32_t num_proofs, int* results,
                          uint8_t* transcripts, const uint64_t* n,
                          const uint64_t* generators_offsets, const uint8_t* b_vectors,
                          const uint8_t* products, const uint8_t* a_commits,
                          const uint8_t* l_vectors, const uint8_t* r_vectors,
                          const uint8_t* ap_values);

unsigned selftest_lane_arithmetic(const EngineCtx& ctx, unsigned warps, unsigned seed);
unsigned selftest_sort(const EngineCtx& ctx, const sxt_sequence_descriptor* d, unsigned num,
                       unsigned window_bits);

unsigned field_op_ed25519(const EngineCtx& ctx, unsigned field, unsigned op, uint64_t n,
                          const uint32_t* a, const uint32_t* b, uint32_t* out);
unsigned field_op_bls12381(const EngineCtx& ctx, unsigned op, uint64_t n, const uint32_t* a,
                           const uint32_t* b, uint32_t* out);
unsigned field_op_bn254(const EngineCtx& ctx, unsigned op, uint64_t n, const uint32_t* a,
                        const uint32_t* b, uint32_t* out);
unsigned field_op_grumpkin(const EngineCtx& ctx, unsigned op, uint64_t n, const uint32_t* a,
                           const uint32_t* b, uint32_t* out);
inline unsigned field_op(const EngineCtx& ctx, unsigned field, unsigned op, uint64_t n,
                         const uint32_t* a, const uint32_t* b, uint32_t* out) {
  switch (field) {
  case 1: return field_op_bls12381(ctx, op, n, a, b, out);
  case 2: return field_op_bn254(ctx, op, n, a, b, out);
  case 3: return field_op_grumpkin(ctx, op, n, a, b, out);
  default: return field_op_ed25519(ctx, field, op, n, a, b, out);
  }
}

void launch_builtin_generators(const EngineCtx& ctx, void* gens, uint64_t first, uint64_t n);

}
```

### blitzar_b200/csrc/msm.cuh

```cuda
#pragma once
#include <algorithm>
#include <vector>

#include "batch_affine.cuh"
#include "curve.cuh"
#include "engine_api.cuh"
#include "lanefield.cuh"

namespace b200 {

struct ColumnDesc {
  const unsigned char* base;
  u64 row_stride;
  u32 bit_offset;
  u32 bit_width;
  u32 n;
  u32 is_signed;
  u32 first_window;
  u32 num_windows;
  u32 table_n;
  u32 gen_base;
};
B200_HD u32 bucket_windows(const ColumnDesc& col) { return col.table_n ? (col.num_windows ? 1u : 0u) : col.num_windows; }

B200_HD void load_scalar_bits(u32 v[8], bool& negative, const ColumnDesc& col, u64 i) {
  const unsigned char* row = col.base + i * col.row_stride;
#pragma unroll
  for (int k = 0; k < 8; ++k)
    v[k] = 0;
  const u32 width = col.bit_width;
  const unsigned char* p = row + (col.bit_offset >> 3);
  const u32 sh = col.bit_offset & 7u;
  if (sh == 0 && width == 256 && (((size_t)p) & 15u) == 0) {
    const uint4* q = (const uint4*)p;
    uint4 a = q[0], b = q[1];
    v[0] = a.x; v[1] = a.y; v[2] = a.z; v[3] = a.w;
    v[4] = b.x; v[5] = b.y; v[6] = b.z; v[7] = b.w;
  } else if (sh == 0 && (width & 31u) == 0 && (((size_t)p) & 3u) == 0) {
    const u32* q = (const u32*)p;
#pragma unroll
    for (int k = 0; k < 8; ++k)
      if ((u32)k < (width >> 5))
        v[k] = q[k];
  } else {
    const u32 nbytes = (sh + width + 7u) >> 3;
#pragma unroll
    for (int k = 0; k < 8; ++k) {
      u64 acc = 0;
#pragma unroll
      for (int b = 0; b < 5; ++b) {
        u32 idx = 4u * k + b;
        if (idx < nbytes)
          acc |= (u64)p[idx] << (8 * b);
      }
      v[k] = (u32)(acc >> sh);
    }
#pragma unroll
    for (int k = 0; k < 8; ++k) {
      int lo = 32 * k;
      if ((int)width <= lo)
        v[k] = 0;
      else if ((int)width < lo + 32)
        v[k] &= (1u << (width - lo)) - 1u;
    }
  }
  negative = false;
  if (col.is_signed) {
    u32 top = width - 1;
    bool neg = false;
#pragma unroll
    for (int k = 0; k < 8; ++k)
      if ((top >> 5) == (u32)k)
        neg = (v[k] >> (top & 31u)) & 1u;
    if (neg) {
      u64 c = 1;
#pragma unroll
      for (int k = 0; k < 8; ++k) {
        int lo = 32 * k;
        u32 m = 0;
        if ((int)width >= lo + 32)
          m = 0xffffffffu;
        else if ((int)width > lo)
          m = (1u << (width - lo)) - 1u;
        c += (u64)((~v[k]) & m);
        v[k] = (u32)c & m;
        c = (m == 0xffffffffu) ? (c >> 32) : 0;
      }
      negative = true;
    }
  }
}

constexpr u32 kAllWindows = 0xffffffffu;
template <class Fn>
B200_HD void for_each_digit(const u32 v[8], bool negative, const ColumnDesc& col, u32 c,
                            u32 nbuckets, Fn f, u32 only_window = kAllWindows) {
  const u32 half = nbuckets;
  const u32 mask = (1u << c) - 1u;
  u64 buf = 0;
  u32 nb = 0, w = 0, carry = 0;
  const u32 W = only_window == kAllWindows
                    ? col.num_windows
                    : (only_window < col.num_windows ? only_window + 1 : 0u);
  const auto step = [&] {
    u32 d = ((u32)buf & mask) + carry;
    buf >>= c;
    bool dneg = d > half;
    carry = dneg ? 1u : 0u;
    if (dneg)
      d = (1u << c) - d;
    if (d && (only_window == kAllWindows || w == only_window))
      f((col.first_window + (col.table_n ? 0u : w)) * nbuckets + (d - 1u), negative != dneg, w);
    ++w;
  };
#pragma unroll
  for (int k = 0; k < 8; ++k) {
    buf |= (u64)v[k] << nb;
    nb += 32;
    for (; nb >= c && w < W; nb -= c)
      step();
  }
  while (w < W)
    step();
}

B200_HD u32 column_of(const u64* col_start, u32 ncols, u64 tid) {
  u32 lo = 0, hi = ncols;
  while (hi - lo > 1) {
    const u32 mid = (lo + hi) >> 1;
    if (tid >= col_start[mid])
      lo = mid;
    else
      hi = mid;
  }
  return lo;
}
template <class Fn>
B200_HD void for_each_entry(const ColumnDesc* cols, const u64* col_start, u32 ncols, u32 c,
                            u32 nbuckets, u64 tid, Fn f, u32 only_window = kAllWindows) {
  const u32 j = column_of(col_start, ncols, tid);
  const ColumnDesc col = cols[j];
  if (only_window != kAllWindows && only_window >= col.num_windows)
    return;
  const u64 i = tid - col_start[j];
  u32 v[8];
  bool neg;
  load_scalar_bits(v, neg, col, i);
  const u32 ii = (u32)i + col.gen_base, tn = col.table_n;
  for_each_digit(v, neg, col, c, nbuckets, [&](u32 key, bool negate, u32 w) {
    f(key, make_entry(key, ii + w * tn, negate));
  }, only_window);
}

struct CountBody {
  static constexpr int kBlock = 256;
  const ColumnDesc* cols;
  const u64* col_start;
  u32 ncols, c, nbuckets;
  u32* counts;
  B200_HD void operator()(u64 tid) const {
    u32* cnt = counts;
    for_each_entry(cols, col_start, ncols, c, nbuckets, tid,
                   [cnt](u32 key, u64) { B200_ATOMIC_ADD(&cnt[key], 1u); });
  }
};

struct ScatterBody {
  static constexpr int kBlock = 256;
  const ColumnDesc* cols;
  const u64* col_start;
  u32 ncols, c, nbuckets;
  u32* cursor;
  u64* entries;
  u64 total_terms;
  B200_HD void operator()(u64 tid) const {
    u32 only = kAllWindows;
    if (total_terms) {
      only = (u32)(tid / total_terms);
      tid -= (u64)only * total_terms;
    }
    u32* cur = cursor;
    u64* en = entries;
    for_each_entry(cols, col_start, ncols, c, nbuckets, tid,
                   [cur, en](u32 key, u64 e) { en[B200_ATOMIC_ADD(&cur[key], 1u)] = e; }, only);
  }
};

constexpr u32 kScanChunk = 256, kScanChunkFirst = 64;
struct ScanUpBody {
  static constexpr int kBlock = 128;
  const u32* in;
  u64 n;
  u32* partial;
  u32 chunk;
  B200_HD void operator()(u64 t) const {
    u64 b = t * chunk, e = b + chunk < n ? b + chunk : n;
    u32 s = 0;
    for (u64 i = b; i < e; ++i)
      s += in[i];
    partial[t] = s;
  }
};
struct ScanTopBody {
  static constexpr int kBlock = 32;
  u32* data;
  u64 n;
  B200_HD void operator()(u64) const {
    u32 s = 0;
    for (u64 i = 0; i < n; ++i) {
      u32 v = data[i];
      data[i] = s;
      s += v;
    }
  }
};
struct ScanDownBody {
  static constexpr int kBlock = 128;
  u32* data;
  u64 n;
  const u32* partial_scanned;
  u32 chunk;
  B200_HD void operator()(u64 t) const {
    u64 b = t * chunk, e = b + chunk < n ? b + chunk : n;
    u32 s = partial_scanned[t];
    for (u64 i = b; i < e; ++i) {
      u32 v = data[i];
      data[i] = s;
      s += v;
    }
  }
};

inline void exclusive_scan(u32* data, u64 n, stream_t s, u32 chunk = kScanChunkFirst) {
  if (n <= kScanChunk) {
    launch(ScanTopBody{data, n}, 1, s);
    return;
  }
  u64 m = (n + chunk - 1) / chunk;
  u32* partial = (u32*)dev_alloc(m * sizeof(u32), s);
  launch(ScanUpBody{data, n, partial, chunk}, m, s);
  exclusive_scan(partial, m, s, kScanChunk);
  launch(ScanDownBody{data, n, partial, chunk}, m, s);
  dev_free(partial, s);
}

#if defined(__CUDACC__) && !defined(B200_EMULATE)
#define B200_BINNED_SORT 1
constexpr u32 kMicroBins = 16384, kBinCap = 8192, kBinSpan = 4096, kMaxBinShift = 12;
constexpr u64 kBinnedSortMinEntries = 1ull << 20;

template <int kBlock> __device__ u32 block_exclusive_scan(u32 v, u32* warp_sums, u32* total) {
  const u32 lane = threadIdx.x & 31u, warp = threadIdx.x >> 5;
  u32 x = v;
#pragma unroll
  for (int d = 1; d < 32; d <<= 1) {
    const u32 y = __shfl_up_sync(0xffffffffu, x, d);
    if (lane >= (u32)d)
      x += y;
  }
  if (lane == 31)
    warp_sums[warp] = x;
  __syncthreads();
  if (warp == 0) {
    u32 w = lane < kBlock / 32 ? warp_sums[lane] : 0u;
#pragma unroll
    for (int d = 1; d < 32; d <<= 1) {
      const u32 y = __shfl_up_sync(0xffffffffu, w, d);
      if (lane >= (u32)d)
        w += y;
    }
    if (lane < kBlock / 32)
      warp_sums[lane] = w;
  }
  __syncthreads();
  const u32 pre = (warp ? warp_sums[warp - 1] : 0u) + x - v;
  *total = warp_sums[kBlock / 32 - 1];
  __syncthreads();
  return pre;
}

struct MicroCountBody {
  static constexpr int kBlock = 512;
  const ColumnDesc* cols;
  const u64* col_start;
  u32 ncols, c, nbuckets;
  u64 total_terms;
  u32 tile, shift, nmicro;
  u32* micro_counts;
  __device__ void run(u32 b, unsigned char* smem) const {
    u32* h = (u32*)smem;
    for (u32 m = threadIdx.x; m < nmicro; m += kBlock)
      h[m] = 0;
    __syncthreads();
    const u64 lo = (u64)b * tile, hi = lo + tile < total_terms ? lo + tile : total_terms;
    const u32 sh = shift;
    for (u64 t = lo + threadIdx.x; t < hi; t += kBlock)
      for_each_entry(cols, col_start, ncols, c, nbuckets, t,
                     [h, sh](u32 key, u64) { atomicAdd(&h[key >> sh], 1u); });
    __syncthreads();
    for (u32 m = threadIdx.x; m < nmicro; m += kBlock)
      if (h[m])
        atomicAdd(&micro_counts[m], h[m]);
  }
};

struct PlanBinsBody {
  static constexpr int kBlock = 1024;
  const u32* micro_counts;
  u32 nmicro, span_micro;
  u64 nkeys;
  u32* bin_of;
  u32* bin_start;
  u32* bin_micro;
  u32* bin_cursor;
  u32* nbins_out;
  u32* counts;
  u32* d_m;
  __device__ bool starts_bin(const u32* st, u32 m) const {
    constexpr u32 H = kBinCap / 2;
    return m == 0 || m % span_micro == 0 || micro_counts[m] > H || micro_counts[m - 1] > H ||
           st[m] / H != st[m - 1] / H;
  }
  __device__ void run(u32, unsigned char* smem) const {
    __shared__ u32 ws[32];
    u32* st = (u32*)smem;
    const u32 per = (nmicro + kBlock - 1) / kBlock, m0 = min(threadIdx.x * per, nmicro),
              m1 = min(m0 + per, nmicro);
    u32 sum = 0;
    for (u32 m = m0; m < m1; ++m)
      sum += micro_counts[m];
    u32 total;
    u32 run = block_exclusive_scan<kBlock>(sum, ws, &total);
    for (u32 m = m0; m < m1; ++m) {
      st[m] = run;
      run += micro_counts[m];
    }
    __syncthreads();
    u32 nf = 0;
    for (u32 m = m0; m < m1; ++m)
      nf += starts_bin(st, m) ? 1u : 0u;
    u32 nbins;
    u32 id = block_exclusive_scan<kBlock>(nf, ws, &nbins);
    for (u32 m = m0; m < m1; ++m) {
      if (starts_bin(st, m)) {
        bin_start[id] = st[m];
        bin_micro[id] = m;
        bin_cursor[id] = st[m];
        ++id;
      }
      bin_of[m] = id - 1;
    }
    if (threadIdx.x == 0) {
      bin_start[nbins] = total;
      bin_micro[nbins] = nmicro;
      *nbins_out = nbins;
      counts[nkeys] = total;
      d_m[0] = total;
    }
  }
};

struct CoarseScatterBody {
  static constexpr int kBlock = 1024;
  const ColumnDesc* cols;
  const u64* col_start;
  u32 ncols, c, nbuckets;
  u64 total_terms;
  u32 tile, shift, nmicro;
  const u32* bin_of;
  const u32* nbins_ptr;
  u32* bin_cursor;
  u64* tmp;
  __device__ void run(u32 b, unsigned char* smem) const {
    __shared__ u32 ws[32];
    u32* h = (u32*)smem;
    u32* delta = h + nmicro;
    u64* stage = (u64*)(delta + nmicro + (nmicro & 1u));
    const u32 nbins = *nbins_ptr;
    for (u32 k = threadIdx.x; k < nbins; k += kBlock)
      h[k] = 0;
    __syncthreads();
    const u64 lo = (u64)b * tile, hi = lo + tile < total_terms ? lo + tile : total_terms;
    const u32 sh = shift;
    const u32* map = bin_of;
    for (u64 t = lo + threadIdx.x; t < hi; t += kBlock)
      for_each_entry(cols, col_start, ncols, c, nbuckets, t,
                     [h, sh, map](u32 key, u64) { atomicAdd(&h[__ldg(&map[key >> sh])], 1u); });
    __syncthreads();
    const u32 per = (nbins + kBlock - 1) / kBlock, k0 = min(threadIdx.x * per, nbins),
              k1 = min(k0 + per, nbins);
    u32 sum = 0;
    for (u32 k = k0; k < k1; ++k)
      sum += h[k];
    u32 size;
    u32 run = block_exclusive_scan<kBlock>(sum, ws, &size);
    for (u32 k = k0; k < k1; ++k) {
      const u32 n = h[k];
      if (n)
        delta[k] = atomicAdd(&bin_cursor[k], n) - run;
      h[k] = run;
      run += n;
    }
    __syncthreads();
    for (u64 t = lo + threadIdx.x; t < hi; t += kBlock)
      for_each_entry(cols, col_start, ncols, c, nbuckets, t, [h, sh, map, stage](u32 key, u64 e) {
        stage[atomicAdd(&h[__ldg(&map[key >> sh])], 1u)] = e;
      });
    __syncthreads();
    for (u32 i = threadIdx.x; i < size; i += kBlock) {
      const u64 e = stage[i];
      tmp[delta[__ldg(&map[entry_key(e) >> sh])] + i] = e;
    }
  }
};

struct BinSortBody {
  static constexpr int kBlock = 1024;
  static constexpr size_t kSmem = 2 * kBinCap * sizeof(u64) + kBinSpan * sizeof(u32);
  const u64* tmp;
  const u32* bin_start;
  const u32* bin_micro;
  const u32* nbins_ptr;
  u32 shift;
  u64 nkeys;
  u64* entries;
  u32* counts;
  __device__ void run(u32 b, unsigned char* smem) const {
    __shared__ u32 ws[32];
    if (b >= *nbins_ptr)
      return;
    u64* ent = (u64*)smem;
    u32* h = (u32*)(smem + 2 * kBinCap * sizeof(u64));
    const u32 lo = bin_start[b], size = bin_start[b + 1] - lo;
    const u64 klo = (u64)bin_micro[b] << shift, khi_m = (u64)bin_micro[b + 1] << shift;
    const u32 span = (u32)((khi_m < nkeys ? khi_m : nkeys) - klo);
    const bool local = size <= kBinCap;
    for (u32 k = threadIdx.x; k < span; k += kBlock)
      h[k] = 0;
    if (local) {
#pragma unroll 4
      for (u32 i = threadIdx.x; i < size; i += kBlock)
        ent[i] = tmp[(u64)lo + i];
    }
    __syncthreads();
    for (u32 i = threadIdx.x; i < size; i += kBlock) {
      const u64 e = local ? ent[i] : tmp[(u64)lo + i];
      atomicAdd(&h[entry_key(e) - (u32)klo], 1u);
    }
    __syncthreads();
    const u32 per = (span + kBlock - 1) / kBlock, k0 = min(threadIdx.x * per, span),
              k1 = min(k0 + per, span);
    u32 sum = 0;
    for (u32 k = k0; k < k1; ++k)
      sum += h[k];
    u32 total;
    u32 run = block_exclusive_scan<kBlock>(sum, ws, &total);
    for (u32 k = k0; k < k1; ++k) {
      const u32 n = h[k];
      h[k] = run;
      run += n;
      counts[klo + k] = lo + run;
    }
    __syncthreads();
    if (!local) {
      for (u32 i = threadIdx.x; i < size; i += kBlock) {
        const u64 e = tmp[(u64)lo + i];
        entries[(u64)lo + atomicAdd(&h[entry_key(e) - (u32)klo], 1u)] = e;
      }
      return;
    }
    u64* sorted = ent + kBinCap;
    for (u32 i = threadIdx.x; i < size; i += kBlock) {
      const u64 e = ent[i];
      sorted[atomicAdd(&h[entry_key(e) - (u32)klo], 1u)] = e;
    }
    __syncthreads();
    for (u32 i = threadIdx.x; i < size; i += kBlock)
      entries[(u64)lo + i] = sorted[i];
  }
};

inline u32 binned_sort_shift(u64 nkeys) {
  u32 shift = 0;
  while ((nkeys + (1ull << shift) - 1) >> shift > kMicroBins)
    ++shift;
  return shift;
}

inline void binned_sort(stream_t s, const ColumnDesc* d_cols, const u64* d_col_start, u32 ncols,
                        u32 c, u32 nbuckets, u64 total_terms, u64 max_entries, u32 max_windows,
                        u64 nkeys, u64* entries, u32* counts, u32* d_m) {
  const u32 shift = binned_sort_shift(nkeys);
  const u32 nmicro = (u32)((nkeys + (1ull << shift) - 1) >> shift);
  const u32 span_micro = std::max(1u, kBinSpan >> shift);
  u32* ws = (u32*)dev_alloc((5ull * nmicro + 3) * sizeof(u32), s);
  u32 *micro_counts = ws, *bin_of = ws + nmicro, *bin_cursor = ws + 2ull * nmicro,
      *bin_start = ws + 3ull * nmicro, *bin_micro = ws + 4ull * nmicro + 1,
      *nbins = ws + 5ull * nmicro + 2;
  u64* tmp = (u64*)dev_alloc(std::max<u64>(max_entries, 1) * sizeof(u64), s);
  dev_zero(micro_counts, nmicro * sizeof(u32), s);
  const u64 count_tile = 4096;
  launch_blocks(MicroCountBody{d_cols, d_col_start, ncols, c, nbuckets, total_terms,
                               (u32)count_tile, shift, nmicro, micro_counts},
                (total_terms + count_tile - 1) / count_tile, nmicro * sizeof(u32), s);
  launch_blocks(PlanBinsBody{micro_counts, nmicro, span_micro, nkeys, bin_of, bin_start, bin_micro,
                             bin_cursor, nbins, counts, d_m},
                1, nmicro * sizeof(u32), s);
  const size_t scatter_smem = 220 * 1024;
  const size_t bin_bytes = (2ull * nmicro + 2) * sizeof(u32);
  const u64 stage_entries = (scatter_smem - bin_bytes) / sizeof(u64);
  const u64 scatter_tile = std::max<u64>(1, stage_entries / max_windows);
  launch_blocks(CoarseScatterBody{d_cols, d_col_start, ncols, c, nbuckets, total_terms,
                                  (u32)scatter_tile, shift, nmicro, bin_of, nbins, bin_cursor, tmp},
                (total_terms + scatter_tile - 1) / scatter_tile, scatter_smem, s);
  launch_blocks(BinSortBody{tmp, bin_start, bin_micro, nbins, shift, nkeys, entries, counts}, nmicro,
                BinSortBody::kSmem, s);
  dev_free(tmp, s);
  dev_free(ws, s);
}
#endif

template <class C> struct FillIdentityBody {
  static constexpr int kBlock = 256;
  static constexpr u32 kChunks = sizeof(typename C::Point) / 16;
  static_assert(sizeof(typename C::Point) % 16 == 0, "points are made of 16-byte aligned fields");
  uint4* p;
  B200_HD void operator()(u64 t) const {
    const typename C::Point id = C::identity();
    const u32 k = (u32)(t % kChunks);
    uint4 v = ((const uint4*)&id)[0];
#pragma unroll
    for (u32 j = 1; j < kChunks; ++j)
      if (j == k)
        v = ((const uint4*)&id)[j];
    p[t] = v;
  }
};
template <class C> inline void fill_identity(stream_t s, typename C::Point* p, u64 n) {
  launch(FillIdentityBody<C>{(uint4*)p}, n * FillIdentityBody<C>::kChunks, s);
}

struct BucketOffsets {
  const u32* ends;
  const u32* starts;
  B200_HD u32 begin(u64 k) const { return starts ? starts[k] : (k ? ends[k - 1] : 0u); }
  B200_HD u32 end(u64 k) const { return ends[k]; }
};

template <class C> struct MergeBucketsBody {
  static constexpr int kBlock = 128;
  BucketOffsets offsets;
  const typename C::Point* scratch;
  typename C::Point* buckets;
  B200_HD void operator()(u64 k) const {
    if (offsets.begin(k) == offsets.end(k))
      return;
    typename C::Point b = buckets[k];
    C::add(b, b, scratch[k]);
    buckets[k] = b;
  }
};

template <class C, bool kGather, class X = SeqExec, bool kUniform = false, bool kUnitZ = false>
struct AccumulateBody {
  static constexpr int kBlock = 128;
  static constexpr int kMinBlocks = !kGather ? 1 : (C::F::N > 8 ? 2 : 3);
  typedef typename C::Point Point;
  typedef typename C::Gen Gen;
  const u32* keys;
  const u64* entries;
  const Gen* gens;
  const Point* pieces;
  const u32* m_ptr;
  u32 K;
  u32 final_level;
  Point* buckets;
  u32* out_keys;
  Point* out_pieces;
  u32* out_m_ptr;
  const u32* unit_veto;

  B200_HD void close_run(u64 t, u32 key, const Point& acc, bool writer, bool& first_seg) const {
    if (final_level || !first_seg) {
      if (writer)
        buckets[key] = acc;
    } else if (writer) {
      out_keys[2 * t] = key;
      out_pieces[2 * t] = acc;
    }
    first_seg = false;
  }
  template <bool kUnit> B200_HD Gen load_gen(u32 idx) const {
    if constexpr (kUnit)
      return C::load_unit_gen(gens + idx);
    else
      return gens[idx];
  }
  template <bool kUnit>
  B200_HD void gather_walk(u64 t, u64 b, u64 e, bool writer, u32& cur, Point& acc,
                           bool& first_seg) const {
    u64 ent = entries[b];
    Gen g = load_gen<kUnit>(entry_gen(ent));
    cur = entry_key(ent);
    for (u64 i = b; i < e; ++i) {
      u64 ent_n = ent;
      Gen g_n = g;
      if (i + 1 < e) {
        ent_n = entries[i + 1];
        g_n = load_gen<kUnit>(entry_gen(ent_n));
      }
      const u32 k = entry_key(ent);
      const bool negate = entry_negate(ent);
      if (kUniform) {
        if (i == b || k != cur) {
          if (i != b) {
            close_run(t, cur, acc, writer, first_seg);
            cur = k;
          }
          acc = C::identity();
        }
        C::template add_gen<X>(acc, acc, g, negate, kUnit);
      } else {
        const bool start = i == b || k != cur;
        if (k != cur) {
          close_run(t, cur, acc, writer, first_seg);
          cur = k;
        }
        if (start)
          C::gen_to_point(acc, g, negate);
        else
          C::template add_gen<X>(acc, acc, g, negate, kUnit);
      }
      ent = ent_n;
      g = g_n;
    }
  }
  B200_HD void operator()(u64 tid) const {
    const u64 t = tid / X::kLanes;
    const bool writer = (tid % X::kLanes) == 0;
    const u64 M = *m_ptr;
    const u64 T = (M + K - 1) / K;
    if (tid == 0 && out_m_ptr)
      *out_m_ptr = final_level ? 0u : (u32)(2 * T);
    u64 b = t * K;
    if (b >= M)
      return;
    u64 e = b + K < M ? b + K : M;
    u32 cur;
    Point acc;
    bool first_seg = true;
    if constexpr (kGather) {
      if (kUnitZ && unit_veto && *unit_veto)
        gather_walk<false>(t, b, e, writer, cur, acc, first_seg);
      else
        gather_walk<kUnitZ>(t, b, e, writer, cur, acc, first_seg);
    } else {
      cur = keys[b];
      acc = pieces[b];
      for (u64 i = b + 1; i < e; ++i) {
        const u32 k = keys[i];
        if (k == cur) {
          C::template add<X>(acc, acc, pieces[i]);
        } else {
          close_run(t, cur, acc, writer, first_seg);
          cur = k;
          acc = pieces[i];
        }
      }
    }
    if (final_level) {
      close_run(t, cur, acc, writer, first_seg);
      return;
    }
    if (!writer)
      return;
    if (first_seg) {
      close_run(t, cur, acc, writer, first_seg);
      acc = C::identity();
    }
    out_keys[2 * t + 1] = cur;
    out_pieces[2 * t + 1] = acc;
  }
};

struct WindowUsedBody {
  static constexpr int kBlock = 64;
  BucketOffsets offsets;
  u32 nbuckets;
  u32* window_used;
  B200_HD void operator()(u64 w) const {
    if (offsets.begin(w * nbuckets) != offsets.begin((w + 1) * nbuckets))
      window_used[w] = 1u;
  }
};

template <class C, class Ex = SeqExec> struct ReduceBody {
  static constexpr int kBlock = 64;
  typedef typename C::Point Point;
  const Point* X;
  const Point* Cin;
  u32 m_in, g, log2g;
  Point* Xout;
  Point* Cout;
  const u32* window_used;
  u32 nbuckets;
  B200_HD void operator()(u64 tid) const {
    const u64 t = tid / Ex::kLanes;
    const bool writer = (tid % Ex::kLanes) == 0;
    const u32 m_out = m_in / g;
    const u32 w = (u32)(t / m_out), k = (u32)(t % m_out);
    if (window_used[w] == 0) {
      if (writer) {
        Xout[t] = C::identity();
        Cout[t] = C::identity();
      }
      return;
    }
    const Point* x = X + (u64)w * m_in + (u64)k * g;
    Point run = x[g - 1];
    Point acc = Cin ? C::identity() : run;
    if (Cin) {
      acc = run;
      if (g == 1)
        acc = C::identity();
    }
    for (u32 r = g - 1; r-- > 0;) {
      C::template add<Ex>(run, run, x[r]);
      if (r > 0 || !Cin)
        C::template add<Ex>(acc, acc, run);
    }
    if (Cin) {
      const Point* cin = Cin + (u64)w * m_in + (u64)k * g;
      for (u32 r = 0; r < g; ++r)
        C::template add<Ex>(acc, acc, cin[r]);
    }
    for (u32 i = 0; i < log2g; ++i)
      C::template dbl<Ex>(run, run);
    if (writer) {
      Xout[t] = run;
      Cout[t] = acc;
    }
  }
};

template <class C, class X = SeqExec> struct CombineBody {
  static constexpr int kBlock = 32;
  typedef typename C::Point Point;
  const Point* S;
  const ColumnDesc* cols;
  u32 c;
  Point* out;
  B200_HD void operator()(u64 tid) const {
    const u64 j = tid / X::kLanes;
    const bool writer = (tid % X::kLanes) == 0;
    const ColumnDesc col = cols[j];
    if (col.num_windows == 0 || col.n == 0) {
      if (writer)
        out[j] = C::identity();
      return;
    }
    const u32 nw = bucket_windows(col);
    Point acc = S[col.first_window + nw - 1];
    for (u32 w = nw - 1; w-- > 0;) {
      for (u32 i = 0; i < c; ++i)
        C::template dbl<X>(acc, acc);
      C::template add<X>(acc, acc, S[col.first_window + w]);
    }
    if (writer)
      out[j] = acc;
  }
};

#if defined(__CUDACC__) && !defined(B200_EMULATE)
#define B200_LANE_TAIL 1
struct CombineLaneBody {
  static constexpr int kBlock = 32;
  typedef Ed25519 C;
  const C::Point* S;
  const ColumnDesc* cols;
  u32 c;
  C::Point* out;
  __device__ void operator()(u64 tid) const {
    const u64 j = tid >> 5;
    const ColumnDesc col = cols[j];
    if (col.num_windows == 0 || col.n == 0) {
      if ((tid & 31u) == 0)
        out[j] = C::identity();
      return;
    }
    const lane10::Lane L = lane10::lane_info();
    const u32 nw = bucket_windows(col);
    C::Point acc = S[col.first_window + nw - 1];
    for (u32 w = nw - 1; w-- > 0;) {
      u32 t;
      const u32 v = lane10::dbl_n(L, lane10::slice_point(L, acc), (int)c, t);
      lane10::gather_point(acc, v, t);
      C::add<QuadExecConv>(acc, acc, S[col.first_window + w]);
    }
    if ((tid & 31u) == 0)
      out[j] = acc;
  }
};
struct LanePow {
  static __device__ __forceinline__ void pow22523(F25519::E& r, const F25519::E& a) {
    const lane10::Lane L = lane10::lane_info();
    const u32 g = L.base / 10u;
    lane10::gather(r, lane10::pow22523(L, lane10::slice(L, a)), g < 3 ? g : 0u);
  }
};
struct StoreLaneBody {
  static constexpr int kBlock = 32;
  const Ed25519::Point* pts;
  unsigned char* out;
  u64 count;
  __device__ void operator()(u64 tid) const {
    const u32 lane = (u32)tid & 31u, g = lane / 10u;
    const u64 i = (tid >> 5) * 3 + g;
    const bool live = g < 3 && i < count;
    unsigned char enc[32];
    Ed25519::encode<LanePow>(enc, pts[live ? i : count - 1]);
    if (live && lane == 10u * g) {
      uint4* d = (uint4*)(out + 32 * i);
      const uint4* e = (const uint4*)enc;
      d[0] = e[0];
      d[1] = e[1];
    }
  }
};
#endif

template <class C>
inline void launch_store_commit(stream_t s, const typename C::Point* pts, unsigned char* out,
                                u64 count, bool lane_tail = true);

template <class C, bool kProjective> struct IngestBody {
  static constexpr int kBlock = 128;
  const unsigned char* raw;
  typename C::Gen* gens;
  B200_HD void operator()(u64 i) const {
    typename C::Gen g;
    if (kProjective)
      C::load_proj_abi(g, raw + i * C::kAbiProjBytes);
    else
      C::load_gen_abi(g, raw + i * C::kAbiGenBytes);
    gens[i] = g;
  }
};
constexpr int kMaxTableWindows = 33;
template <class C> struct PrecomputeTableBody {
  static constexpr int kBlock = 64;
  typename C::Gen* table;
  u64 n;
  u32 c, W;
  B200_HD void operator()(u64 i) const {
    typedef typename C::F F;
    typename C::Point p, pts[kMaxTableWindows];
    typename F::E prefix[kMaxTableWindows], acc = F::one(), inv;
    C::gen_to_point(p, table[i], false);
    for (u32 w = 0; w < W; ++w) {
      if (w)
        for (u32 k = 0; k < c; ++k)
          C::dbl(p, p);
      pts[w] = p;
      prefix[w] = acc;
      F::mul(acc, acc, C::denominator(p));
    }
    F::invert(inv, acc);
    for (u32 w = W; w-- > 0;) {
      typename F::E zi;
      F::mul(zi, inv, prefix[w]);
      F::mul(inv, inv, C::denominator(pts[w]));
      typename C::Gen g;
      C::normalized_gen(g, pts[w], zi);
      table[(u64)w * n + i] = g;
    }
  }
};
template <class C> struct IngestCompactBody {
  static constexpr int kBlock = 128;
  const unsigned char* table;
  u32 window_width;
  typename C::Gen* gens;
  B200_HD void operator()(u64 i) const {
    const u64 group = i / window_width, j = i % window_width;
    const u64 entry = (group << window_width) + (1ull << j);
    typename C::Gen g;
    C::load_compact_abi(g, table + entry * C::kAbiCompactBytes);
    gens[i] = g;
  }
};
struct BuiltinGeneratorBody {
  static constexpr int kBlock = 64;
  Ed25519::Gen* gens;
  u64 first;
  B200_HD void operator()(u64 i) const {
    Ed25519::Point g;
    Ed25519::builtin_generator(g, first + i);
    Ed25519::point_to_gen(gens[i], g);
  }
};
struct GenPieces {
  const u64* start;
  const u64* from;
  const u64* to;
  u32 npieces;
};
template <class C> struct IngestPiecesBody {
  static constexpr int kBlock = IngestBody<C, false>::kBlock;
  const unsigned char* raw;
  typename C::Gen* gens;
  GenPieces p;
  B200_HD void operator()(u64 tid) const {
    const u32 k = column_of(p.start, p.npieces, tid);
    IngestBody<C, false>{raw + p.from[k] * C::kAbiGenBytes, gens + p.to[k]}(tid - p.start[k]);
  }
};
struct BuiltinPiecesBody {
  static constexpr int kBlock = BuiltinGeneratorBody::kBlock;
  Ed25519::Gen* gens;
  GenPieces p;
  B200_HD void operator()(u64 tid) const {
    const u32 k = column_of(p.start, p.npieces, tid);
    BuiltinGeneratorBody{gens + p.to[k], p.from[k]}(tid - p.start[k]);
  }
};

struct IngestMap {
  GenPieces p;
  B200_HD void at(u64 i, u64& src, u64& dst) const {
    if (p.npieces == 0) {
      src = dst = i;
      return;
    }
    const u32 k = column_of(p.start, p.npieces, i);
    src = p.from[k] + (i - p.start[k]);
    dst = p.to[k] + (i - p.start[k]);
  }
};
constexpr u32 kNormBlock = 256;
struct NormalizeUpBody {
  static constexpr int kBlock = 128;
  typedef F25519 F;
  const unsigned char* raw;
  IngestMap map;
  u64 n, T;
  F::E* pre;
  F::E* prod;
  u32* invalid;
  B200_HD F::E group(u64 j) const {
    F::E z[kBatchGroup], acc = F::one();
#pragma unroll
    for (u32 k = 0; k < kBatchGroup; ++k) {
      const u64 i = j + k * T;
      z[k] = F::one();
      if (i < n) {
        u64 src, dst;
        map.at(i, src, dst);
        z[k] = Ed25519::load_abi_z(raw + src * Ed25519::kAbiGenBytes);
      }
    }
#pragma unroll
    for (u32 k = 0; k < kBatchGroup; ++k) {
      const u64 i = j + k * T;
      if (i >= n)
        break;
      if (F::is_zero(z[k])) {
        *invalid = 1u;
        z[k] = F::one();
      }
      pre[i] = acc;
      F::mul(acc, acc, z[k]);
    }
    return acc;
  }
  B200_HD void operator()(u64 j) const { prod[j] = group(j); }
};
struct NormalizeDownBody {
  static constexpr int kBlock = 128;
  typedef F25519 F;
  const unsigned char* raw;
  IngestMap map;
  u64 n, T;
  const F::E* pre;
  const F::E* prod;
  const F::E* ps;
  const u32* invalid;
  Ed25519::Gen* gens;
  B200_HD void operator()(u64 j) const {
    const bool scale = *invalid == 0;
    F::E inv = prod[ps ? j / kNormBlock : j];
    if (ps)
      F::mul(inv, inv, ps[j]);
    for (u32 k = kBatchGroup; k-- > 0;) {
      const u64 i = j + k * T;
      if (i >= n)
        continue;
      u64 src, dst;
      map.at(i, src, dst);
      Ed25519::Point p;
      Ed25519::load_point_abi(p, raw + src * Ed25519::kAbiGenBytes);
      if (scale) {
        F::E zi;
        F::mul(zi, inv, pre[i]);
        F::mul(inv, inv, p.Z);
        F::mul(p.X, p.X, zi);
        F::mul(p.Y, p.Y, zi);
        F::mul(p.T, p.T, zi);
        p.Z = F::one();
      }
      Ed25519::Gen g;
      Ed25519::point_to_gen(g, p);
      gens[dst] = g;
    }
  }
};
#ifdef B200_BINNED_SORT
__device__ __forceinline__ F25519::E shfl_up_fe(const F25519::E& a, u32 d) {
  F25519::E r;
#pragma unroll
  for (int k = 0; k < 8; ++k)
    r.l[k] = __shfl_up_sync(0xffffffffu, a.l[k], d);
  return r;
}
__device__ __forceinline__ F25519::E shfl_down_fe(const F25519::E& a, u32 d) {
  F25519::E r;
#pragma unroll
  for (int k = 0; k < 8; ++k)
    r.l[k] = __shfl_down_sync(0xffffffffu, a.l[k], d);
  return r;
}
template <int kBlock>
__device__ void block_prefix_suffix(const F25519::E& x, F25519::E& P, F25519::E& S,
                                    F25519::E& total, F25519::E* ws) {
  typedef F25519 F;
  const u32 lane = threadIdx.x & 31u, warp = threadIdx.x >> 5;
  F::E inc = x, sinc = x;
#pragma unroll
  for (u32 d = 1; d < 32; d <<= 1) {
    const F::E y = shfl_up_fe(inc, d), z = shfl_down_fe(sinc, d);
    if (lane >= d)
      F::mul(inc, inc, y);
    if (lane + d < 32)
      F::mul(sinc, sinc, z);
  }
  F::E pe = shfl_up_fe(inc, 1), se = shfl_down_fe(sinc, 1);
  if (lane == 0)
    pe = F::one();
  if (lane == 31) {
    se = F::one();
    ws[warp] = inc;
  }
  __syncthreads();
  F::E before = F::one(), after = F::one();
  for (u32 w = 0; w < kBlock / 32; ++w) {
    if (w < warp)
      F::mul(before, before, ws[w]);
    else if (w > warp)
      F::mul(after, after, ws[w]);
  }
  F::mul(P, before, pe);
  F::mul(S, se, after);
  F::mul(total, before, ws[warp]);
  F::mul(total, total, after);
  __syncthreads();
}
struct NormalizeUpBlockBody {
  static constexpr int kBlock = kNormBlock;
  typedef F25519 F;
  NormalizeUpBody up;
  F::E* ps;
  F::E* prod;
  __device__ void run(u32 b, unsigned char*) const {
    __shared__ F::E ws[kBlock / 32];
    const u64 j = (u64)b * kBlock + threadIdx.x;
    const F::E g = j < up.T ? up.group(j) : F::one();
    F::E P, S, total;
    block_prefix_suffix<kBlock>(g, P, S, total, ws);
    if (j < up.T)
      F::mul(ps[j], P, S);
    if (threadIdx.x == 0)
      prod[b] = total;
  }
};
struct NormalizeMidBody {
  static constexpr int kBlock = 1024;
  typedef F25519 F;
  F::E* vals;
  F::E* pre;
  u64 m;
  __device__ void run(u32, unsigned char*) const {
    __shared__ F::E ws[kBlock / 32];
    __shared__ F::E inv_total;
    const u64 per = (m + kBlock - 1) / kBlock, lo = min((u64)threadIdx.x * per, m),
              hi = min(lo + per, m);
    F::E c = F::one();
    for (u64 k = lo; k < hi; ++k) {
      pre[k] = c;
      F::mul(c, c, vals[k]);
    }
    F::E P, S, total;
    block_prefix_suffix<kBlock>(c, P, S, total, ws);
    if (threadIdx.x == 0)
      F::invert(inv_total, total);
    __syncthreads();
    F::E inv;
    F::mul(inv, inv_total, P);
    F::mul(inv, inv, S);
    for (u64 k = hi; k-- > lo;) {
      const F::E v = vals[k];
      F::mul(vals[k], inv, pre[k]);
      F::mul(inv, inv, v);
    }
  }
};
#endif
inline void ingest_normalized(stream_t s, const unsigned char* raw, Ed25519::Gen* gens,
                              const IngestMap& map, u64 n, u32* invalid) {
  typedef F25519::E fe;
  if (n == 0)
    return;
  const u64 T = (n + kBatchGroup - 1) / kBatchGroup;
  fe* pre = (fe*)dev_alloc(n * sizeof(fe), s);
  const NormalizeUpBody up{raw, map, n, T, pre, nullptr, invalid};
#ifdef B200_BINNED_SORT
  const u64 blocks = (T + kNormBlock - 1) / kNormBlock;
  fe* ps = (fe*)dev_alloc((T + 2 * blocks) * sizeof(fe), s);
  fe* prod = ps + T;
  launch_blocks(NormalizeUpBlockBody{up, ps, prod}, blocks, 0, s);
  launch_blocks(NormalizeMidBody{prod, prod + blocks, blocks}, 1, 0, s);
  launch(NormalizeDownBody{raw, map, n, T, pre, prod, ps, invalid, gens}, T, s);
  dev_free(ps, s);
#else
  fe* prod = (fe*)dev_alloc(T * sizeof(fe), s);
  NormalizeUpBody u = up;
  u.prod = prod;
  launch(u, T, s);
  batch_invert<F25519>(s, prod, T);
  launch(NormalizeDownBody{raw, map, n, T, pre, prod, nullptr, invalid, gens}, T, s);
  dev_free(prod, s);
#endif
  dev_free(pre, s);
}
template <class C, bool kCommit> struct StoreBody {
  static constexpr int kBlock = 32;
  const typename C::Point* pts;
  unsigned char* out;
  B200_HD void operator()(u64 i) const {
    if (kCommit)
      C::store_commit_abi(out + i * C::kAbiCommitBytes, pts[i]);
    else
      C::store_proj_abi(out + i * C::kAbiProjBytes, pts[i]);
  }
};
template <class C>
inline void launch_store_commit(stream_t s, const typename C::Point* pts, unsigned char* out,
                                u64 count, bool lane_tail) {
#ifdef B200_LANE_TAIL
  if constexpr (C::kCurveId == kRistretto255) {
    if (lane_tail && count && count <= 4096) {
      launch(StoreLaneBody{pts, out, count}, (count + 2) / 3 * 32, s);
      return;
    }
  }
#endif
  launch(StoreBody<C, true>{pts, out}, count, s);
}
template <class C> struct GenToProjBody {
  static constexpr int kBlock = 64;
  const typename C::Gen* gens;
  unsigned char* out;
  B200_HD void operator()(u64 i) const {
    typename C::Point p;
    C::gen_to_point(p, gens[i], false);
    C::store_proj_abi(out + i * C::kAbiProjBytes, p);
  }
};
template <class C> struct SumPartsBody {
  static constexpr int kBlock = 32;
  const typename C::Point* parts;
  u32 nparts, count;
  typename C::Point* out;
  B200_HD void operator()(u64 j) const {
    typename C::Point acc = parts[j];
    for (u32 r = 1; r < nparts; ++r)
      C::add(acc, acc, parts[(u64)r * count + j]);
    out[j] = acc;
  }
};

inline u32 choose_window_bits(u64 max_n, u32 max_width, u32 ncols, size_t point_bytes) {
  const double kMaxBucketBytes = 3.0e9;
  u32 best = 2;
  double best_cost = 1e300;
  for (u32 c = 2; c <= 16; ++c) {
    double W = (double)(max_width / c + 1);
    if (c > 8 && W * (double)(1u << (c - 1)) * (double)ncols * (double)point_bytes > kMaxBucketBytes)
      break;
    double cost = W * ((double)max_n + 2.5 * (double)(1u << (c - 1)));
    if (cost < best_cost) {
      best_cost = cost;
      best = c;
    }
  }
  return best;
}

struct MsmPlan {
  u32 c = 0, nbuckets = 0, ncols = 0, total_windows = 0;
  u64 nkeys = 0, max_n = 0, total_terms = 0, total_entries = 0;
  std::vector<ColumnDesc> cols;
};

inline MsmPlan msm_make_plan(std::vector<ColumnDesc> cols, const MsmOptions& opt,
                             size_t point_bytes) {
  MsmPlan p;
  p.ncols = (u32)cols.size();
  u32 max_width = 1;
  for (auto& col : cols) {
    p.max_n = std::max<u64>(p.max_n, col.n);
    p.total_terms += col.n;
    if (col.n)
      max_width = std::max(max_width, col.bit_width);
  }
  p.c = opt.window_bits ? opt.window_bits
                        : choose_window_bits(p.max_n, max_width, p.ncols, point_bytes);
  p.nbuckets = 1u << (p.c - 1);
  u64 max_entries = 0;
  for (auto& col : cols) {
    col.first_window = p.total_windows;
    col.num_windows = col.n ? col.bit_width / p.c + 1 : 0;
    p.total_windows += bucket_windows(col);
    max_entries += (u64)col.n * col.num_windows;
    if (col.table_n)
      B200_REQUIRE((u64)col.table_n * col.num_windows < (1ull << 31), "generator table too large");
    if (col.n)
      B200_REQUIRE((u64)col.gen_base + col.n + (u64)(col.num_windows - 1) * col.table_n < (1ull << 31),
                   "generator index of a column too large");
  }
  p.nkeys = (u64)p.total_windows * p.nbuckets;
  p.total_entries = max_entries;
  B200_REQUIRE(p.nkeys < (1ull << 32), "too many buckets for one pass");
  p.cols = std::move(cols);
  return p;
}

struct StagedRange {
  const ColumnDesc* d_cols = nullptr;
  const u64* d_col_start = nullptr;
  u64 total_terms = 0, max_entries = 0;
  u32 max_windows = 0;
  StagedRange(stream_t s, const MsmPlan& plan, u64 begin, u64 end) {
    const u32 ncols = plan.ncols;
    std::vector<ColumnDesc> cols(plan.cols);
    std::vector<u64> col_start(ncols + 1, 0);
    for (u32 j = 0; j < ncols; ++j) {
      u64 lo = std::min<u64>(begin, cols[j].n), hi = std::min<u64>(end, cols[j].n);
      cols[j].base += lo * cols[j].row_stride;
      cols[j].n = (u32)(hi - lo);
      col_start[j + 1] = col_start[j] + cols[j].n;
      max_entries += (u64)cols[j].n * cols[j].num_windows;
      max_windows = std::max(max_windows, cols[j].n ? cols[j].num_windows : 0u);
    }
    total_terms = col_start[ncols];
    if (total_terms == 0)
      return;
    B200_REQUIRE(max_entries < (1ull << 32) && end - begin < (1ull << 31),
                 "too many (term, window) entries for one sort pass");
    const size_t desc_bytes = ncols * sizeof(ColumnDesc), start_bytes = (ncols + 1) * sizeof(u64);
    std::vector<unsigned char> stage(desc_bytes + start_bytes);
    std::memcpy(stage.data(), cols.data(), desc_bytes);
    std::memcpy(stage.data() + desc_bytes, col_start.data(), start_bytes);
    d_cols = (const ColumnDesc*)stage_to_device(s, stage.data(), stage.size());
    d_col_start = (const u64*)((const unsigned char*)d_cols + desc_bytes);
  }
};

struct SortedLayout {
  u64* entries;
  u32* counts;
  u32* starts;
  u32* d_m;
  u64 slots_max;
  bool binned;
  BucketOffsets offsets() const { return {counts, starts}; }
};

inline SortedLayout sort_entries(stream_t s, const MsmPlan& plan, const StagedRange& r, u32 L,
                                 const MsmOptions& opt, u32* window_used) {
  const u32 ncols = plan.ncols, c = plan.c, nbuckets = plan.nbuckets;
  const u64 nkeys = plan.nkeys, max_entries = r.max_entries, total_terms = r.total_terms;
  SortedLayout out{};
  out.slots_max = L ? ((max_entries + nkeys * ((1ull << L) - 1) + (1ull << L) - 1) >> L) << L : max_entries;
  out.counts = (u32*)dev_alloc((nkeys + 1) * sizeof(u32), s);
  out.d_m = (u32*)dev_alloc(16 * sizeof(u32), s);
  out.entries = (u64*)dev_alloc(out.slots_max * sizeof(u64), s);
#ifdef B200_BINNED_SORT
  out.binned = L == 0 && opt.sort_path != 0 && binned_sort_shift(nkeys) <= kMaxBinShift &&
               (opt.sort_path == 2 || max_entries >= kBinnedSortMinEntries);
  if (out.binned)
    binned_sort(s, r.d_cols, r.d_col_start, ncols, c, nbuckets, total_terms, max_entries,
                r.max_windows, nkeys, out.entries, out.counts, out.d_m);
#endif
  if (!out.binned) {
    dev_zero(out.counts, (nkeys + 1) * sizeof(u32), s);
    launch(CountBody{r.d_cols, r.d_col_start, ncols, c, nbuckets, out.counts}, total_terms, s);
    if (L)
      launch(PadCountsBody{out.counts, (1u << L) - 1u}, nkeys, s);
    exclusive_scan(out.counts, nkeys + 1, s);
    copy_d2d(out.d_m, out.counts + nkeys, sizeof(u32), s);
    if (L) {
      out.starts = (u32*)dev_alloc((nkeys + 1) * sizeof(u32), s);
      copy_d2d(out.starts, out.counts, (nkeys + 1) * sizeof(u32), s);
    }
    const bool window_major = opt.scatter_window_major && r.max_windows > 1;
    launch(ScatterBody{r.d_cols, r.d_col_start, ncols, c, nbuckets, out.counts, out.entries,
                       window_major ? total_terms : 0},
           window_major ? total_terms * r.max_windows : total_terms, s);
  }
  if (L)
    launch(FillPadsBody{out.starts, out.counts, out.entries}, nkeys, s);
  launch(WindowUsedBody{out.offsets(), nbuckets, window_used}, plan.total_windows, s);
  return out;
}

inline unsigned sort_selftest(stream_t s, std::vector<ColumnDesc> cols, u32 c) {
  MsmOptions opt;
  opt.window_bits = c;
  const MsmPlan plan = msm_make_plan(std::move(cols), opt, 160);
  const StagedRange r(s, plan, 0, plan.max_n);
  if (r.total_terms == 0)
    return ~0u;
  const u64 nkeys = plan.nkeys, M = r.max_entries;
  DevBuf<u32> window_used(plan.total_windows, s);
  opt.sort_path = 0;
  const SortedLayout a = sort_entries(s, plan, r, 0, opt, window_used.p);
  opt.sort_path = 2;
  const SortedLayout b = sort_entries(s, plan, r, 0, opt, window_used.p);
  std::vector<u32> ca(nkeys + 1), cb(nkeys + 1), m(1);
  std::vector<u64> ea(M), eb(M);
  copy_d2h(ca.data(), a.counts, (nkeys + 1) * sizeof(u32), s);
  copy_d2h(cb.data(), b.counts, (nkeys + 1) * sizeof(u32), s);
  copy_d2h(m.data(), b.d_m, sizeof(u32), s);
  copy_d2h(ea.data(), a.entries, M * sizeof(u64), s);
  copy_d2h(eb.data(), b.entries, M * sizeof(u64), s);
  stream_sync(s);
  for (void* p : {(void*)a.entries, (void*)a.counts, (void*)a.d_m, (void*)b.entries, (void*)b.counts,
                  (void*)b.d_m, (void*)r.d_cols})
    dev_free(p, s);
  if (!b.binned)
    return ~0u;
  unsigned bad = m[0] == ca[nkeys] ? 0u : 1u;
  for (u64 k = 0; k < nkeys; ++k) {
    const u32 lo = k ? ca[k - 1] : 0u, hi = ca[k];
    if (cb[k] != hi || hi < lo || hi > M) {
      ++bad;
      continue;
    }
    std::sort(ea.begin() + lo, ea.begin() + hi);
    std::sort(eb.begin() + lo, eb.begin() + hi);
    if (!std::equal(ea.begin() + lo, ea.begin() + hi, eb.begin() + lo))
      ++bad;
  }
  return bad;
}

struct RangeHook {
  virtual void before_range(u64 begin, u64 end) = 0;
  virtual void before_accumulate() {}
  virtual ~RangeHook() {}
};

template <class C>
stream_t chunk_walk(stream_t s, stream_t tail, WalkInput<C> walk, u32* d_m, bool unit,
                    const u32* unit_veto, typename C::Point* target, const MsmOptions& opt,
                    std::vector<void*>& to_free) {
  typedef typename C::Point Point;
  u32 K = opt.chunk1 ? std::max(opt.chunk1, 4u) : (walk.m_max >= (1ull << 23) ? 64u : 32u);
  const u32 chunkn = std::max(opt.chunkn, 4u);
  const u32* lvl_keys = nullptr;
  const Point* lvl_pieces = nullptr;
  stream_t cs = s;
  for (int level = 0;; ++level) {
    const bool final_level = walk.m_max <= K;
    u64 T = (walk.m_max + K - 1) / K;
    u32* out_keys = final_level ? nullptr : (u32*)dev_alloc(2 * T * sizeof(u32), cs);
    Point* out_pieces = final_level ? nullptr : (Point*)dev_alloc(2 * T * sizeof(Point), cs);
    to_free.insert(to_free.end(), {out_keys, out_pieces});
    u32* out_m = d_m + 1 + (level % 8);
    const auto launch_level = [&](auto body, u64 threads, stream_t st) {
      body = {lvl_keys, walk.entries, walk.gens, lvl_pieces, walk.m_ptr, K, final_level, target,
              out_keys, out_pieces, out_m, unit_veto};
      launch(body, threads, st);
    };
    if (level == 0) {
      const bool uniform =
          opt.uniform_add == 2 ? C::kCurveId == kRistretto255 : opt.uniform_add != 0;
      constexpr bool kEd = C::kCurveId == kRistretto255;
      const bool unit_path = kEd && unit;
      if (uniform && unit_path)
        launch_level(AccumulateBody<C, true, SeqExec, true, kEd>{}, T, s);
      else if (uniform)
        launch_level(AccumulateBody<C, true, SeqExec, true>{}, T, s);
      else if (unit_path)
        launch_level(AccumulateBody<C, true, SeqExec, false, kEd>{}, T, s);
      else
        launch_level(AccumulateBody<C, true>{}, T, s);
      KernelTimer::get().end(s);
      if (tail != s)
        stream_follow(tail, s);
      cs = tail;
    } else if (T <= opt.quad_threshold) {
      launch_level(AccumulateBody<C, false, QuadExec>{}, T * QuadExec::kLanes, cs);
    } else {
      launch_level(AccumulateBody<C, false>{}, T, cs);
    }
    if (final_level)
      break;
    lvl_keys = out_keys;
    lvl_pieces = out_pieces;
    walk.m_ptr = out_m;
    walk.m_max = 2 * T;
    K = chunkn;
  }
  return cs;
}

template <class C>
void msm_accumulate_range(stream_t s, const MsmPlan& plan, const typename C::Gen* gens, u64 begin,
                          u64 end, bool add_into, typename C::Point* d_buckets,
                          u32* d_window_used, const MsmOptions& opt, stream_t tail,
                          RangeHook* hook = nullptr) {
  const StagedRange r(s, plan, begin, end);
  if (r.total_terms == 0)
    return;
  gens += begin;
  StageRange nvtx_sort("msm: digit count + scan + scatter");
  const u64 max_entries = r.max_entries, nkeys = plan.nkeys;
  u32 L = 0;
  if constexpr (C::kBatchAffine) {
    const double mean = (double)max_entries / (double)nkeys;
    if (opt.pair_levels >= 0)
      L = (u32)opt.pair_levels;
    else if (max_entries >= (1ull << 23))
      while (L < 6 && (double)(32u << L) <= mean)
        ++L;
    while (L > 0 && max_entries + nkeys * ((1ull << L) - 1) >= (1ull << 32) - (1ull << L))
      --L;
  }
  const SortedLayout sorted = sort_entries(s, plan, r, L, opt, d_window_used);
  B200_LOG(3, "range [%llu, %llu): %llu terms, %llu entries max, c=%u, %llu keys, pair levels %u",
           (unsigned long long)begin, (unsigned long long)end, (unsigned long long)r.total_terms,
           (unsigned long long)max_entries, plan.c, (unsigned long long)nkeys, L);
  WalkInput<C> walk{gens, sorted.entries, sorted.d_m, max_entries};
  std::vector<void*> to_free;
  if (hook)
    hook->before_accumulate();
  KernelTimer::get().begin(s);
  StageRange nvtx_acc("msm: bucket accumulation");
  if constexpr (C::kBatchAffine) {
    if (L) {
      walk = run_pair_levels<C>(s, L, sorted.entries, gens, sorted.d_m, sorted.slots_max,
                                opt.pair_batch);
      to_free = {(void*)walk.gens, (void*)walk.entries};
    }
  }
  typedef typename C::Point Point;
  Point* target = add_into ? (Point*)dev_alloc(nkeys * sizeof(Point), s) : d_buckets;
  const bool unit = walk.gens == gens && opt.gens_normalized;
  const stream_t cs =
      chunk_walk<C>(s, tail, walk, sorted.d_m, unit, opt.unit_veto, target, opt, to_free);
  if (add_into) {
    launch(MergeBucketsBody<C>{sorted.offsets(), target, d_buckets}, nkeys, cs);
    dev_free(target, cs);
  }
  to_free.insert(to_free.end(), {sorted.d_m, sorted.counts, sorted.starts});
  for (void* ptr : to_free)
    dev_free(ptr, cs);
  dev_free(sorted.entries, s);
  dev_free((void*)r.d_cols, s);
}

template <class C>
void msm_finish(stream_t s, const MsmPlan& plan, const typename C::Point* d_buckets,
                const u32* d_window_used, typename C::Point* out, const MsmOptions& opt) {
  typedef typename C::Point Point;
  StageRange nvtx_fin("msm: bucket reduction + window combination");
  const u32 total_windows = plan.total_windows, nbuckets = plan.nbuckets, ncols = plan.ncols;
  ColumnDesc* d_cols =
      (ColumnDesc*)stage_to_device(s, plan.cols.data(), ncols * sizeof(ColumnDesc));
  Point* d_S = nullptr;
  u32 m = nbuckets;
  const Point* X = d_buckets;
  const Point* Cin = nullptr;
  std::vector<void*> to_free;
  if (m == 1) {
    d_S = (Point*)dev_alloc(total_windows * sizeof(Point), s);
    copy_d2d(d_S, d_buckets, total_windows * sizeof(Point), s);
  }
  bool first = true;
  while (m > 1) {
    u32 g = first ? std::min<u32>(opt.reduce_g1, m) : std::min<u32>(opt.reduce_gn, m);
    u32 log2g = 0;
    while ((1u << log2g) < g)
      ++log2g;
    u32 m_out = m / g;
    Point* Xout = (Point*)dev_alloc((u64)total_windows * m_out * sizeof(Point), s);
    Point* Cout = (Point*)dev_alloc((u64)total_windows * m_out * sizeof(Point), s);
    if ((u64)total_windows * m_out <= opt.quad_threshold)
      launch(ReduceBody<C, QuadExecConv>{X, Cin, m, g, log2g, Xout, Cout, d_window_used, nbuckets},
             (u64)total_windows * m_out * QuadExec::kLanes, s);
    else
      launch(ReduceBody<C>{X, Cin, m, g, log2g, Xout, Cout, d_window_used, nbuckets},
             (u64)total_windows * m_out, s);
    to_free.push_back(Xout);
    if (m_out > 1)
      to_free.push_back(Cout);
    X = Xout;
    Cin = Cout;
    m = m_out;
    first = false;
    if (m == 1)
      d_S = Cout;
  }
  for (void* ptr : to_free)
    dev_free(ptr, s);
  bool uniform_windows = true;
  for (u32 j = 1; j < ncols; ++j)
    uniform_windows = uniform_windows && bucket_windows(plan.cols[j]) == bucket_windows(plan.cols[0]);
#ifdef B200_LANE_TAIL
  bool lane_done = false;
  if constexpr (C::kCurveId == kRistretto255) {
    if (ncols <= 2048 && opt.lane_tail) {
      launch(CombineLaneBody{d_S, d_cols, plan.c, out}, (u64)ncols * 32, s);
      lane_done = true;
    }
  }
  if (lane_done) {
  } else
#endif
  if (ncols <= opt.quad_threshold && uniform_windows)
    launch(CombineBody<C, QuadExecConv>{d_S, d_cols, plan.c, out}, (u64)ncols * QuadExec::kLanes,
           s);
  else if (ncols <= opt.quad_threshold)
    launch(CombineBody<C, QuadExec>{d_S, d_cols, plan.c, out}, (u64)ncols * QuadExec::kLanes, s);
  else
    launch(CombineBody<C>{d_S, d_cols, plan.c, out}, ncols, s);
  dev_free(d_S, s);
  dev_free(d_cols, s);
}

template <class C>
void msm_run(stream_t s, const typename C::Gen* gens, std::vector<ColumnDesc> cols,
             typename C::Point* out, const MsmOptions& opt = MsmOptions(), u32 num_ranges = 1,
             RangeHook* hook = nullptr, stream_t tail = stream_t()) {
  typedef typename C::Point Point;
  if (cols.empty())
    return;
  MsmPlan plan = msm_make_plan(std::move(cols), opt, sizeof(Point));
  B200_LOG(2, "msm: curve %u, %u columns, longest %llu, %llu terms, window %u bits, %u bucket sets%s",
           C::kCurveId, plan.ncols, (unsigned long long)plan.max_n,
           (unsigned long long)plan.total_terms, plan.c, plan.total_windows,
           plan.ncols && plan.cols[0].table_n ? " (fixed-base table)" : "");
  if (plan.total_terms == 0 || plan.total_windows == 0) {
    if (hook)
      hook->before_range(0, plan.max_n);
    fill_identity<C>(s, out, plan.ncols);
    return;
  }
  Point* d_buckets = (Point*)dev_alloc(plan.nkeys * sizeof(Point), s);
  fill_identity<C>(s, d_buckets, plan.nkeys);
  u32* d_window_used = (u32*)dev_alloc(plan.total_windows * sizeof(u32), s);
  dev_zero(d_window_used, plan.total_windows * sizeof(u32), s);
  if (num_ranges < 1)
    num_ranges = 1;
  const u64 limit = opt.max_range_entries ? opt.max_range_entries : (1ull << 31);
  const u64 needed = (plan.total_entries + limit - 1) / limit;
  if (needed > num_ranges)
    num_ranges = (u32)std::min<u64>(needed, plan.max_n);
  const bool overlap = num_ranges > 1 && tail != stream_t() && tail != s;
  for (u32 r = 0; r < num_ranges; ++r) {
    u64 begin = range_begin(plan.max_n, r, num_ranges, opt.range_skew),
        end = range_begin(plan.max_n, r + 1, num_ranges, opt.range_skew);
    if (hook)
      hook->before_range(begin, end);
    msm_accumulate_range<C>(s, plan, gens, begin, end, r > 0, d_buckets, d_window_used, opt,
                            overlap ? tail : s, hook);
  }
  if (overlap)
    stream_follow(s, tail);
  msm_finish<C>(s, plan, d_buckets, d_window_used, out, opt);
  dev_free(d_window_used, s);
  dev_free(d_buckets, s);
}

}
```

### include/blitzar_b200.h

```cpp
#ifndef BLITZAR_B200_H
#define BLITZAR_B200_H

#include <stdint.h>

#ifdef __cplusplus
extern "C" {
#endif

#define SXT_CPU_BACKEND 1
#define SXT_GPU_BACKEND 2
#define SXT_CURVE_RISTRETTO255 0
#define SXT_CURVE_BLS_381 1
#define SXT_CURVE_BN_254 2
#define SXT_CURVE_GRUMPKIN 3
#define SXT_FIELD_SCALAR255 0
#define SXT_FIELD_GRUMPKIN 1

struct sxt_config { int backend; uint64_t num_precomputed_generators; };
struct sxt_ristretto255_compressed { uint8_t ristretto_bytes[32]; };
struct sxt_bls12_381_g1_compressed { uint8_t g1_bytes[48]; };
struct sxt_curve25519_scalar { uint8_t bytes[32]; };
struct sxt_transcript { uint8_t bytes[203]; };
struct sxt_ristretto255 { uint64_t X[5]; uint64_t Y[5]; uint64_t Z[5]; uint64_t T[5]; };
struct sxt_bls12_381_g1 { uint64_t X[6]; uint64_t Y[6]; };
struct sxt_bls12_381_g1_p2 { uint64_t X[6]; uint64_t Y[6]; uint64_t Z[6]; };
struct sxt_bn254_g1 { uint64_t X[4]; uint64_t Y[4]; uint8_t infinity; };
struct sxt_bn254_g1_p2 { uint64_t X[4]; uint64_t Y[4]; uint64_t Z[4]; };
struct sxt_grumpkin { uint64_t X[4]; uint64_t Y[4]; uint8_t infinity; };
struct sxt_grumpkin_p2 { uint64_t X[4]; uint64_t Y[4]; uint64_t Z[4]; };
struct sxt_sequence_descriptor {
  uint8_t element_nbytes;
  uint64_t n;
  const uint8_t* data;
  int is_signed;
};
struct sumcheck_descriptor {
  const void* mles;
  const void* product_table;
  const unsigned* product_terms;
  unsigned n;
  unsigned num_mles;
  unsigned num_products;
  unsigned num_product_terms;
  unsigned round_degree;
};
struct sxt_multiexp_handle;


int sxt_init(const struct sxt_config* config);

void sxt_curve25519_compute_pedersen_commitments(struct sxt_ristretto255_compressed* commitments,
                                                 uint32_t num_sequences,
                                                 const struct sxt_sequence_descriptor* descriptors,
                                                 uint64_t offset_generators);
void sxt_curve25519_compute_pedersen_commitments_with_generators(
    struct sxt_ristretto255_compressed* commitments, uint32_t num_sequences,
    const struct sxt_sequence_descriptor* descriptors, const struct sxt_ristretto255* generators);
void sxt_bls12_381_g1_compute_pedersen_commitments_with_generators(
    struct sxt_bls12_381_g1_compressed* commitments, uint32_t num_sequences,
    const struct sxt_sequence_descriptor* descriptors, const struct sxt_bls12_381_g1* generators);
void sxt_bn254_g1_uncompressed_compute_pedersen_commitments_with_generators(
    struct sxt_bn254_g1* commitments, uint32_t num_sequences,
    const struct sxt_sequence_descriptor* descriptors, const struct sxt_bn254_g1* generators);
void sxt_grumpkin_uncompressed_compute_pedersen_commitments_with_generators(
    struct sxt_grumpkin* commitments, uint32_t num_sequences,
    const struct sxt_sequence_descriptor* descriptors, const struct sxt_grumpkin* generators);

int sxt_ristretto255_get_generators(struct sxt_ristretto255* generators, uint64_t num_generators,
                                    uint64_t offset_generators);
int sxt_curve25519_get_one_commit(struct sxt_ristretto255* one_commit, uint64_t n);

void sxt_curve25519_prove_inner_product(struct sxt_ristretto255_compressed* l_vector,
                                        struct sxt_ristretto255_compressed* r_vector,
                                        struct sxt_curve25519_scalar* ap_value,
                                        struct sxt_transcript* transcript, uint64_t n,
                                        uint64_t generators_offset,
                                        const struct sxt_curve25519_scalar* a_vector,
                                        const struct sxt_curve25519_scalar* b_vector);
int sxt_curve25519_verify_inner_product(struct sxt_transcript* transcript, uint64_t n,
                                        uint64_t generators_offset,
                                        const struct sxt_curve25519_scalar* b_vector,
                                        const struct sxt_curve25519_scalar* product,
                                        const struct sxt_ristretto255* a_commit,
                                        const struct sxt_ristretto255_compressed* l_vector,
                                        const struct sxt_ristretto255_compressed* r_vector,
                                        const struct sxt_curve25519_scalar* ap_value);

struct sxt_multiexp_handle* sxt_multiexp_handle_new(unsigned curve_id, const void* generators,
                                                    unsigned n);
struct sxt_multiexp_handle* sxt_multiexp_handle_new_from_file(unsigned curve_id,
                                                              const char* filename);
void sxt_multiexp_handle_write_to_file(const struct sxt_multiexp_handle* handle,
                                       const char* filename);
void sxt_multiexp_handle_free(struct sxt_multiexp_handle* handle);

void sxt_fixed_multiexponentiation(void* res, const struct sxt_multiexp_handle* handle,
                                   unsigned element_num_bytes, unsigned num_outputs, unsigned n,
                                   const uint8_t* scalars);
void sxt_fixed_packed_multiexponentiation(void* res, const struct sxt_multiexp_handle* handle,
                                          const unsigned* output_bit_table, unsigned num_outputs,
                                          unsigned n, const uint8_t* scalars);
void sxt_fixed_vlen_multiexponentiation(void* res, const struct sxt_multiexp_handle* handle,
                                        const unsigned* output_bit_table,
                                        const unsigned* output_lengths, unsigned num_outputs,
                                        const uint8_t* scalars);
void sxt_prove_sumcheck(void* polynomials, void* evaluation_point, unsigned field_id,
                        const struct sumcheck_descriptor* descriptor, void* transcript_callback,
                        void* transcript_context);


void b200_set_device(int device);
unsigned long long b200_launch_count(void);
unsigned b200_point_bytes(unsigned curve_id);
void* b200_malloc(uint64_t bytes);
void b200_free(void* device_ptr);
void b200_memcpy_h2d(void* device_dst, const void* host_src, uint64_t bytes);
void b200_memcpy_d2h(void* host_dst, const void* device_src, uint64_t bytes);
void b200_synchronize(void);
void* b200_stream(void);
void* b200_event_create(void);
void b200_event_record(void* event);
float b200_event_elapsed_ms(void* start, void* stop);
void b200_event_destroy(void* event);

void b200_commit_device(unsigned curve_id, void* out_commitments, void* out_partials,
                        uint32_t num_sequences, const struct sxt_sequence_descriptor* descriptors,
                        const void* generators, uint64_t offset_generators);
void b200_commit_host_partials(unsigned curve_id, void* out_partials, uint32_t num_sequences,
                               const struct sxt_sequence_descriptor* descriptors,
                               const void* generators, uint64_t offset_generators);
void b200_compute_pedersen_commitments_with_offsets(unsigned curve_id, void* commitments,
                                                    uint32_t num_sequences,
                                                    const struct sxt_sequence_descriptor* descriptors,
                                                    const void* generators, const uint64_t* offsets);
void b200_commit_device_with_offsets(unsigned curve_id, void* out_commitments, void* out_partials,
                                     uint32_t num_sequences,
                                     const struct sxt_sequence_descriptor* descriptors,
                                     const void* generators, const uint64_t* offsets);
void b200_fixed_msm_host_partials(void* out_partials, const struct sxt_multiexp_handle* handle,
                                  int mode, unsigned element_num_bytes,
                                  const unsigned* output_bit_table, const unsigned* output_lengths,
                                  unsigned num_outputs, unsigned n, const uint8_t* scalars);
struct sxt_multiexp_handle* b200_multiexp_handle_new_device(unsigned curve_id,
                                                            const void* generators_dev,
                                                            unsigned n);
void b200_combine_partials_device(unsigned curve_id, void* out_commitments, const void* partials,
                                  uint32_t num_parts, uint32_t count);
void b200_fixed_msm_device(void* out_res, void* out_partials,
                           const struct sxt_multiexp_handle* handle, int mode,
                           unsigned element_num_bytes, const unsigned* output_bit_table,
                           const unsigned* output_lengths, unsigned num_outputs, unsigned n,
                           const uint8_t* scalars);
void b200_combine_partials_projective_device(unsigned curve_id, void* out_res,
                                             const void* partials, uint32_t num_parts,
                                             uint32_t count);
void b200_synthetic_generators_device(unsigned curve_id, void* out_generators, uint64_t n,
                                      uint64_t first, int projective);
void b200_partition_table_device(unsigned curve_id, void* out_table_dev, const void* generators_dev,
                                 uint64_t n, unsigned window_width);
void b200_multiexp_handle_write_partition_table(const struct sxt_multiexp_handle* handle,
                                                const char* filename, unsigned window_width);
unsigned b200_multiexp_handle_add_partition_table(struct sxt_multiexp_handle* handle,
                                                  unsigned window_width);
unsigned b200_multiexp_handle_partition_window(const struct sxt_multiexp_handle* handle);
void b200_curve25519_prove_inner_products(
    uint32_t num_proofs, struct sxt_ristretto255_compressed* l_vectors ,
    struct sxt_ristretto255_compressed* r_vectors ,
    struct sxt_curve25519_scalar* ap_values ,
    struct sxt_transcript* transcripts , const uint64_t* n,
    const uint64_t* generators_offsets, const struct sxt_curve25519_scalar* a_vectors ,
    const struct sxt_curve25519_scalar* b_vectors );
uint32_t b200_curve25519_verify_inner_products(
    uint32_t num_proofs, int* results, struct sxt_transcript* transcripts, const uint64_t* n,
    const uint64_t* generators_offsets, const struct sxt_curve25519_scalar* b_vectors ,
    const struct sxt_curve25519_scalar* products, const struct sxt_ristretto255* a_commits,
    const struct sxt_ristretto255_compressed* l_vectors ,
    const struct sxt_ristretto255_compressed* r_vectors ,
    const struct sxt_curve25519_scalar* ap_values);
unsigned b200_selftest_lane_arithmetic(unsigned warps, unsigned seed);
unsigned b200_field_op(unsigned field, unsigned op, uint64_t n, const uint32_t* a,
                       const uint32_t* b, uint32_t* out);
unsigned b200_selftest_sort(const struct sxt_sequence_descriptor* columns, unsigned num,
                            unsigned window_bits);
void b200_profile_accumulate(int enable);
void b200_profile_read(float* total_ms, unsigned* launches);
void b200_set_tuning(unsigned window_bits, unsigned chunk1, unsigned chunkn);
void b200_set_reduce_groups(unsigned g1, unsigned gn);

#ifdef __cplusplus
}
#endif
#endif
```

Baseline: 351.4 million.

## Shrink sorted MSM entries from 64-bit to 32-bit, derive bucket keys from offsets

Sorted bucket entries now hold only the generator index and negate bit in 32 bits. The bucket key is no longer stored; accumulation works out bucket boundaries from the per-bucket end offsets, using a per-chunk binary search plus an exponential search at each boundary. The binned sort packs a bin-relative key into the free high bits of the 32-bit word and keeps a 16-bit bin id in shared memory. Together these halve entry memory traffic and staging shared memory, at the cost of extra search kernels, boundary logic and a limit on how many generator bits fit.

New measurement: 360.1 million, median of 6. +2.5%, better.

```diff
diff --git a/blitzar_b200/api.py b/blitzar_b200/api.py
--- a/blitzar_b200/api.py
+++ b/blitzar_b200/api.py
@@ -338,7 +338,7 @@
     return call_field_op(lib().b200_field_op, field, op, a, b)
 
 
-def selftest_sort(columns_shape, scalar_ptrs, window_bits=0):
+def selftest_sort(columns_shape, scalar_ptrs, window_bits=0, generator_offset=0):
     num = len(columns_shape)
     arr = (sxt_sequence_descriptor * max(1, num))()
     for i, (n, nbytes, is_signed) in enumerate(columns_shape):
@@ -347,7 +347,8 @@
         arr[i].data = scalar_ptrs[i]
         arr[i].is_signed = int(is_signed)
     lib().b200_selftest_sort.restype = C.c_uint
-    return int(lib().b200_selftest_sort(arr, C.c_uint(num), C.c_uint(window_bits)))
+    return int(lib().b200_selftest_sort(arr, C.c_uint(num), C.c_uint(window_bits),
+                                        C.c_uint(generator_offset)))
 
 
 def synthetic_generators_device(curve_id, out_ptr, n, first=0, projective=False):
diff --git a/blitzar_b200/csrc/api.cu b/blitzar_b200/csrc/api.cu
--- a/blitzar_b200/csrc/api.cu
+++ b/blitzar_b200/csrc/api.cu
@@ -1361,11 +1361,11 @@
   return field_op(ctx(), field, op, n, a, b, out);
 }
 unsigned b200_selftest_sort(const sxt_sequence_descriptor* columns, unsigned num,
-                            unsigned window_bits) {
+                            unsigned window_bits, unsigned generator_offset) {
   const Entry entry("b200_selftest_sort");
   B200_REQUIRE(num == 0 || columns != nullptr, "columns == nullptr");
   B200_REQUIRE(window_bits <= 20, "window_bits in 0..20");
-  return selftest_sort(ctx(), columns, num, window_bits);
+  return selftest_sort(ctx(), columns, num, window_bits, generator_offset);
 }
 void b200_set_reduce_groups(unsigned g1, unsigned gn) {
   std::lock_guard<std::mutex> lock(g_mutex);
diff --git a/blitzar_b200/csrc/batch_affine.cuh b/blitzar_b200/csrc/batch_affine.cuh
--- a/blitzar_b200/csrc/batch_affine.cuh
+++ b/blitzar_b200/csrc/batch_affine.cuh
@@ -1,17 +1,9 @@
 #pragma once
 #include "curve.cuh"
+#include "entry.cuh"
 #include "runtime.cuh"
 
 namespace b200 {
-
-constexpr u32 kPadIndex = 0x7fffffffu;
-B200_HD u64 make_entry(u32 key, u32 gen, bool negate) {
-  return ((u64)key << 32) | (u64)((gen << 1) | (negate ? 1u : 0u));
-}
-B200_HD u64 pad_entry(u32 key) { return make_entry(key, kPadIndex, false); }
-B200_HD u32 entry_key(u64 e) { return (u32)(e >> 32); }
-B200_HD u32 entry_gen(u64 e) { return (u32)e >> 1; }
-B200_HD bool entry_negate(u64 e) { return ((u32)e & 1u) != 0; }
 
 constexpr u32 kBatchGroup = 8;
 constexpr u32 kBatchTop = 4;
@@ -80,7 +72,7 @@
   typedef typename C::F F;
   typedef typename F::E fe;
   typedef typename C::Gen Gen;
-  const u64* entries;
+  const u32* entries;
   const Gen* gens;
   const Gen* in;
   const u32* m_ptr;
@@ -93,7 +85,7 @@
       a = in[slot];
       return;
     }
-    const u64 ent = entries[slot];
+    const u32 ent = entries[slot];
     const u32 idx = entry_gen(ent);
     if (idx == kPadIndex) {
       a.x = F::zero();
@@ -263,39 +255,44 @@
   static constexpr int kBlock = 128;
   const u32* starts;
   const u32* cursor;
-  u64* entries;
+  u32* entries;
   B200_HD void operator()(u64 k) const {
-    const u64 pad = pad_entry((u32)k);
     for (u32 i = cursor[k]; i < starts[k + 1]; ++i)
-      entries[i] = pad;
-  }
-};
-struct FinalEntriesBody {
+      entries[i] = pad_entry();
+  }
+};
+struct FinalLevelBody {
   static constexpr int kBlock = 256;
-  const u64* entries0;
+  const u32* starts;
   const u32* m_ptr;
   u32 L;
-  u64* entries;
+  u64 nkeys;
+  u32* entries;
+  u32* ends;
   u32* m_out;
   B200_HD void operator()(u64 j) const {
     const u64 m = (u64)(*m_ptr) >> L;
     if (j == 0)
       *m_out = (u32)m;
     if (j < m)
-      entries[j] = make_entry(entry_key(entries0[j << L]), (u32)j, false);
+      entries[j] = make_entry((u32)j, false);
+    if (j < nkeys)
+      ends[j] = starts[j + 1] >> L;
   }
 };
 
 template <class C> struct WalkInput {
   const typename C::Gen* gens;
-  const u64* entries;
+  const u32* entries;
+  const u32* ends;
+  u64 nkeys;
   const u32* m_ptr;
   u64 m_max;
 };
 
 template <class C>
-WalkInput<C> run_pair_levels(stream_t s, u32 L, const u64* entries, const typename C::Gen* gens,
-                             u32* d_m, u64 slots_max, u32 pair_batch) {
+WalkInput<C> run_pair_levels(stream_t s, u32 L, const u32* entries, const u32* starts, u64 nkeys,
+                             const typename C::Gen* gens, u32* d_m, u64 slots_max, u32 pair_batch) {
   typedef typename C::F F;
   typedef typename F::E fe;
   typedef typename C::Gen Gen;
@@ -338,9 +335,10 @@
     if (ptr != (void*)in)
       dev_free(ptr, s);
   const u64 m_max = slots_max >> L;
-  u64* entries_l = (u64*)dev_alloc(m_max * sizeof(u64), s);
-  launch(FinalEntriesBody{entries, d_m, L, entries_l, d_m + 9}, m_max, s);
-  return {in, entries_l, d_m + 9, m_max};
+  u32* entries_l = (u32*)dev_alloc(m_max * sizeof(u32), s);
+  u32* ends_l = (u32*)dev_alloc(nkeys * sizeof(u32), s);
+  launch(FinalLevelBody{starts, d_m, L, nkeys, entries_l, ends_l, d_m + 9}, std::max(m_max, nkeys), s);
+  return {in, entries_l, ends_l, nkeys, d_m + 9, m_max};
 }
 
 }
diff --git a/blitzar_b200/csrc/curve_ed25519.cu b/blitzar_b200/csrc/curve_ed25519.cu
--- a/blitzar_b200/csrc/curve_ed25519.cu
+++ b/blitzar_b200/csrc/curve_ed25519.cu
@@ -38,7 +38,7 @@
 #endif
 }
 unsigned selftest_sort(const EngineCtx& ctx, const sxt_sequence_descriptor* d, unsigned num,
-                       unsigned window_bits) {
+                       unsigned window_bits, unsigned generator_offset) {
   std::vector<ColumnDesc> cols(num);
   for (unsigned i = 0; i < num; ++i) {
     cols[i] = ColumnDesc{};
@@ -47,6 +47,7 @@
     cols[i].bit_width = 8u * d[i].element_nbytes;
     cols[i].n = (u32)d[i].n;
     cols[i].is_signed = d[i].is_signed ? 1u : 0u;
+    cols[i].gen_base = generator_offset;
   }
   return sort_selftest(ctx.s, std::move(cols), window_bits);
 }
diff --git a/blitzar_b200/csrc/engine_api.cuh b/blitzar_b200/csrc/engine_api.cuh
--- a/blitzar_b200/csrc/engine_api.cuh
+++ b/blitzar_b200/csrc/engine_api.cuh
@@ -259,7 +259,7 @@
 
 unsigned selftest_lane_arithmetic(const EngineCtx& ctx, unsigned warps, unsigned seed);
 unsigned selftest_sort(const EngineCtx& ctx, const sxt_sequence_descriptor* d, unsigned num,
-                       unsigned window_bits);
+                       unsigned window_bits, unsigned generator_offset);
 
 unsigned field_op_ed25519(const EngineCtx& ctx, unsigned field, unsigned op, uint64_t n,
                           const uint32_t* a, const uint32_t* b, uint32_t* out);
diff --git a/blitzar_b200/csrc/entry.cuh b/blitzar_b200/csrc/entry.cuh
--- /dev/null
+++ b/blitzar_b200/csrc/entry.cuh
@@ -0,0 +1,23 @@
+#pragma once
+#include "runtime.cuh"
+
+namespace b200 {
+
+constexpr u32 kPadIndex = 0x7fffffffu;
+B200_HD u32 make_entry(u32 gen, bool negate) { return (gen << 1) | (negate ? 1u : 0u); }
+B200_HD u32 pad_entry() { return make_entry(kPadIndex, false); }
+B200_HD u32 entry_gen(u32 e) { return e >> 1; }
+B200_HD bool entry_negate(u32 e) { return (e & 1u) != 0; }
+
+inline u32 entry_bits(u64 max_gen) {
+  u32 bits = 1;
+  while (bits < 32 && (max_gen >> (bits - 1)) != 0)
+    ++bits;
+  return bits;
+}
+inline u32 entry_bin_span_log2(u32 bits) { return 32 - bits; }
+B200_HD u32 pack_bin_entry(u32 rel_key, u32 e, u32 bits) { return (u32)((u64)rel_key << bits) | e; }
+B200_HD u32 bin_entry_key(u32 t, u32 bits) { return (u32)((u64)t >> bits); }
+B200_HD u32 bin_entry_sorted(u32 t, u32 bits) { return (u32)(t & (((u64)1 << bits) - 1)); }
+
+}
diff --git a/blitzar_b200/csrc/msm.cuh b/blitzar_b200/csrc/msm.cuh
--- a/blitzar_b200/csrc/msm.cuh
+++ b/blitzar_b200/csrc/msm.cuh
@@ -148,7 +148,7 @@
   load_scalar_bits(v, neg, col, i);
   const u32 ii = (u32)i + col.gen_base, tn = col.table_n;
   for_each_digit(v, neg, col, c, nbuckets, [&](u32 key, bool negate, u32 w) {
-    f(key, make_entry(key, ii + w * tn, negate));
+    f(key, make_entry(ii + w * tn, negate));
   }, only_window);
 }
 
@@ -161,7 +161,7 @@
   B200_HD void operator()(u64 tid) const {
     u32* cnt = counts;
     for_each_entry(cols, col_start, ncols, c, nbuckets, tid,
-                   [cnt](u32 key, u64) { B200_ATOMIC_ADD(&cnt[key], 1u); });
+                   [cnt](u32 key, u32) { B200_ATOMIC_ADD(&cnt[key], 1u); });
   }
 };
 
@@ -171,7 +171,7 @@
   const u64* col_start;
   u32 ncols, c, nbuckets;
   u32* cursor;
-  u64* entries;
+  u32* entries;
   u64 total_terms;
   B200_HD void operator()(u64 tid) const {
     u32 only = kAllWindows;
@@ -180,9 +180,9 @@
       tid -= (u64)only * total_terms;
     }
     u32* cur = cursor;
-    u64* en = entries;
+    u32* en = entries;
     for_each_entry(cols, col_start, ncols, c, nbuckets, tid,
-                   [cur, en](u32 key, u64 e) { en[B200_ATOMIC_ADD(&cur[key], 1u)] = e; }, only);
+                   [cur, en](u32 key, u32 e) { en[B200_ATOMIC_ADD(&cur[key], 1u)] = e; }, only);
   }
 };
 
@@ -296,7 +296,7 @@
     const u32 sh = shift;
     for (u64 t = lo + threadIdx.x; t < hi; t += kBlock)
       for_each_entry(cols, col_start, ncols, c, nbuckets, t,
-                     [h, sh](u32 key, u64) { atomicAdd(&h[key >> sh], 1u); });
+                     [h, sh](u32 key, u32) { atomicAdd(&h[key >> sh], 1u); });
     __syncthreads();
     for (u32 m = threadIdx.x; m < nmicro; m += kBlock)
       if (h[m])
@@ -366,26 +366,32 @@
   const u64* col_start;
   u32 ncols, c, nbuckets;
   u64 total_terms;
-  u32 tile, shift, nmicro;
+  u32 tile, shift;
+  u32 bins_max;
+  u32 stage_cap;
+  u32 bits;
   const u32* bin_of;
+  const u32* bin_micro;
   const u32* nbins_ptr;
   u32* bin_cursor;
-  u64* tmp;
+  u32* tmp;
   __device__ void run(u32 b, unsigned char* smem) const {
     __shared__ u32 ws[32];
     u32* h = (u32*)smem;
-    u32* delta = h + nmicro;
-    u64* stage = (u64*)(delta + nmicro + (nmicro & 1u));
+    u32* delta = h + bins_max;
+    u32* stage = delta + bins_max;
+    unsigned short* stage_bin = (unsigned short*)(stage + stage_cap);
     const u32 nbins = *nbins_ptr;
     for (u32 k = threadIdx.x; k < nbins; k += kBlock)
       h[k] = 0;
     __syncthreads();
     const u64 lo = (u64)b * tile, hi = lo + tile < total_terms ? lo + tile : total_terms;
-    const u32 sh = shift;
+    const u32 sh = shift, nb = bits;
     const u32* map = bin_of;
+    const u32* first = bin_micro;
     for (u64 t = lo + threadIdx.x; t < hi; t += kBlock)
       for_each_entry(cols, col_start, ncols, c, nbuckets, t,
-                     [h, sh, map](u32 key, u64) { atomicAdd(&h[__ldg(&map[key >> sh])], 1u); });
+                     [h, sh, map](u32 key, u32) { atomicAdd(&h[__ldg(&map[key >> sh])], 1u); });
     __syncthreads();
     const u32 per = (nbins + kBlock - 1) / kBlock, k0 = min(threadIdx.x * per, nbins),
               k1 = min(k0 + per, nbins);
@@ -403,35 +409,37 @@
     }
     __syncthreads();
     for (u64 t = lo + threadIdx.x; t < hi; t += kBlock)
-      for_each_entry(cols, col_start, ncols, c, nbuckets, t, [h, sh, map, stage](u32 key, u64 e) {
-        stage[atomicAdd(&h[__ldg(&map[key >> sh])], 1u)] = e;
-      });
+      for_each_entry(cols, col_start, ncols, c, nbuckets, t,
+                     [h, sh, nb, map, first, stage, stage_bin](u32 key, u32 e) {
+                       const u32 k = __ldg(&map[key >> sh]);
+                       const u32 i = atomicAdd(&h[k], 1u);
+                       stage[i] = pack_bin_entry(key - (__ldg(&first[k]) << sh), e, nb);
+                       stage_bin[i] = (unsigned short)k;
+                     });
     __syncthreads();
-    for (u32 i = threadIdx.x; i < size; i += kBlock) {
-      const u64 e = stage[i];
-      tmp[delta[__ldg(&map[entry_key(e) >> sh])] + i] = e;
-    }
+    for (u32 i = threadIdx.x; i < size; i += kBlock)
+      tmp[delta[stage_bin[i]] + i] = stage[i];
   }
 };
 
 struct BinSortBody {
   static constexpr int kBlock = 1024;
-  static constexpr size_t kSmem = 2 * kBinCap * sizeof(u64) + kBinSpan * sizeof(u32);
-  const u64* tmp;
+  static constexpr size_t kSmem = 2 * kBinCap * sizeof(u32) + kBinSpan * sizeof(u32);
+  const u32* tmp;
   const u32* bin_start;
   const u32* bin_micro;
   const u32* nbins_ptr;
-  u32 shift;
+  u32 shift, bits;
   u64 nkeys;
-  u64* entries;
+  u32* entries;
   u32* counts;
   __device__ void run(u32 b, unsigned char* smem) const {
     __shared__ u32 ws[32];
     if (b >= *nbins_ptr)
       return;
-    u64* ent = (u64*)smem;
-    u32* h = (u32*)(smem + 2 * kBinCap * sizeof(u64));
-    const u32 lo = bin_start[b], size = bin_start[b + 1] - lo;
+    u32* ent = (u32*)smem;
+    u32* h = ent + 2 * kBinCap;
+    const u32 lo = bin_start[b], size = bin_start[b + 1] - lo, nb = bits;
     const u64 klo = (u64)bin_micro[b] << shift, khi_m = (u64)bin_micro[b + 1] << shift;
     const u32 span = (u32)((khi_m < nkeys ? khi_m : nkeys) - klo);
     const bool local = size <= kBinCap;
@@ -444,8 +452,8 @@
     }
     __syncthreads();
     for (u32 i = threadIdx.x; i < size; i += kBlock) {
-      const u64 e = local ? ent[i] : tmp[(u64)lo + i];
-      atomicAdd(&h[entry_key(e) - (u32)klo], 1u);
+      const u32 e = local ? ent[i] : tmp[(u64)lo + i];
+      atomicAdd(&h[bin_entry_key(e, nb)], 1u);
     }
     __syncthreads();
     const u32 per = (span + kBlock - 1) / kBlock, k0 = min(threadIdx.x * per, span),
@@ -464,15 +472,15 @@
     __syncthreads();
     if (!local) {
       for (u32 i = threadIdx.x; i < size; i += kBlock) {
-        const u64 e = tmp[(u64)lo + i];
-        entries[(u64)lo + atomicAdd(&h[entry_key(e) - (u32)klo], 1u)] = e;
+        const u32 e = tmp[(u64)lo + i];
+        entries[(u64)lo + atomicAdd(&h[bin_entry_key(e, nb)], 1u)] = bin_entry_sorted(e, nb);
       }
       return;
     }
-    u64* sorted = ent + kBinCap;
+    u32* sorted = ent + kBinCap;
     for (u32 i = threadIdx.x; i < size; i += kBlock) {
-      const u64 e = ent[i];
-      sorted[atomicAdd(&h[entry_key(e) - (u32)klo], 1u)] = e;
+      const u32 e = ent[i];
+      sorted[atomicAdd(&h[bin_entry_key(e, nb)], 1u)] = bin_entry_sorted(e, nb);
     }
     __syncthreads();
     for (u32 i = threadIdx.x; i < size; i += kBlock)
@@ -486,18 +494,27 @@
     ++shift;
   return shift;
 }
+inline u32 binned_span_micro(u64 nkeys, u64 max_gen) {
+  const u32 shift = binned_sort_shift(nkeys), span_log2 = entry_bin_span_log2(entry_bits(max_gen));
+  if (shift > kMaxBinShift || span_log2 < shift)
+    return 0;
+  return (u32)(std::min<u64>(kBinSpan, 1ull << span_log2) >> shift);
+}
 
 inline void binned_sort(stream_t s, const ColumnDesc* d_cols, const u64* d_col_start, u32 ncols,
                         u32 c, u32 nbuckets, u64 total_terms, u64 max_entries, u32 max_windows,
-                        u64 nkeys, u64* entries, u32* counts, u32* d_m) {
-  const u32 shift = binned_sort_shift(nkeys);
+                        u64 max_gen, u64 nkeys, u32* entries, u32* counts, u32* d_m) {
+  const u32 shift = binned_sort_shift(nkeys), bits = entry_bits(max_gen);
   const u32 nmicro = (u32)((nkeys + (1ull << shift) - 1) >> shift);
-  const u32 span_micro = std::max(1u, kBinSpan >> shift);
+  const u32 span_micro = binned_span_micro(nkeys, max_gen);
+  const u64 half_cap = kBinCap / 2;
+  const u32 bins_max = (u32)std::min<u64>(
+      nmicro, (nmicro + span_micro - 1) / span_micro + 2 * (max_entries / half_cap));
   u32* ws = (u32*)dev_alloc((5ull * nmicro + 3) * sizeof(u32), s);
   u32 *micro_counts = ws, *bin_of = ws + nmicro, *bin_cursor = ws + 2ull * nmicro,
       *bin_start = ws + 3ull * nmicro, *bin_micro = ws + 4ull * nmicro + 1,
       *nbins = ws + 5ull * nmicro + 2;
-  u64* tmp = (u64*)dev_alloc(std::max<u64>(max_entries, 1) * sizeof(u64), s);
+  u32* tmp = (u32*)dev_alloc(std::max<u64>(max_entries, 1) * sizeof(u32), s);
   dev_zero(micro_counts, nmicro * sizeof(u32), s);
   const u64 count_tile = 4096;
   launch_blocks(MicroCountBody{d_cols, d_col_start, ncols, c, nbuckets, total_terms,
@@ -507,14 +524,15 @@
                              bin_cursor, nbins, counts, d_m},
                 1, nmicro * sizeof(u32), s);
   const size_t scatter_smem = 220 * 1024;
-  const size_t bin_bytes = (2ull * nmicro + 2) * sizeof(u32);
-  const u64 stage_entries = (scatter_smem - bin_bytes) / sizeof(u64);
-  const u64 scatter_tile = std::max<u64>(1, stage_entries / max_windows);
+  const size_t bin_bytes = 2ull * bins_max * sizeof(u32);
+  const u32 stage_cap = (u32)((scatter_smem - bin_bytes) / (sizeof(u32) + sizeof(unsigned short)));
+  const u64 scatter_tile = std::max<u64>(1, stage_cap / max_windows);
   launch_blocks(CoarseScatterBody{d_cols, d_col_start, ncols, c, nbuckets, total_terms,
-                                  (u32)scatter_tile, shift, nmicro, bin_of, nbins, bin_cursor, tmp},
+                                  (u32)scatter_tile, shift, bins_max, stage_cap, bits, bin_of,
+                                  bin_micro, nbins, bin_cursor, tmp},
                 (total_terms + scatter_tile - 1) / scatter_tile, scatter_smem, s);
-  launch_blocks(BinSortBody{tmp, bin_start, bin_micro, nbins, shift, nkeys, entries, counts}, nmicro,
-                BinSortBody::kSmem, s);
+  launch_blocks(BinSortBody{tmp, bin_start, bin_micro, nbins, shift, bits, nkeys, entries, counts},
+                nmicro, BinSortBody::kSmem, s);
   dev_free(tmp, s);
   dev_free(ws, s);
 }
@@ -561,6 +579,29 @@
   }
 };
 
+struct ChunkBucketBody {
+  static constexpr int kBlock = 256;
+  const u32* ends;
+  u64 nkeys;
+  const u32* m_ptr;
+  u32 K;
+  u32* chunk_bucket;
+  B200_HD void operator()(u64 t) const {
+    const u64 b = t * K;
+    if (b >= *m_ptr)
+      return;
+    u64 lo = 0, hi = nkeys - 1;
+    while (lo < hi) {
+      const u64 mid = (lo + hi) >> 1;
+      if (ends[mid] > b)
+        hi = mid;
+      else
+        lo = mid + 1;
+    }
+    chunk_bucket[t] = (u32)lo;
+  }
+};
+
 template <class C, bool kGather, class X = SeqExec, bool kUniform = false, bool kUnitZ = false>
 struct AccumulateBody {
   static constexpr int kBlock = 128;
@@ -568,7 +609,10 @@
   typedef typename C::Point Point;
   typedef typename C::Gen Gen;
   const u32* keys;
-  const u64* entries;
+  const u32* entries;
+  const u32* ends;
+  u64 nkeys;
+  const u32* chunk_bucket;
   const Gen* gens;
   const Point* pieces;
   const u32* m_ptr;
@@ -596,37 +640,56 @@
     else
       return gens[idx];
   }
+  B200_HD u32 bucket_after(u32 i, u32 lo) const {
+    const u32 last = (u32)(nkeys - 1);
+    u32 hi = lo, step = 1;
+    while (ends[hi] <= i) {
+      lo = hi + 1;
+      hi = step < last - hi ? hi + step : last;
+      step <<= 1;
+    }
+    while (lo < hi) {
+      const u32 mid = lo + ((hi - lo) >> 1);
+      if (ends[mid] > i)
+        hi = mid;
+      else
+        lo = mid + 1;
+    }
+    return (u32)lo;
+  }
   template <bool kUnit>
   B200_HD void gather_walk(u64 t, u64 b, u64 e, bool writer, u32& cur, Point& acc,
                            bool& first_seg) const {
-    u64 ent = entries[b];
+    const u32 last = (u32)(nkeys - 1);
+    u32 ent = entries[b];
     Gen g = load_gen<kUnit>(entry_gen(ent));
-    cur = entry_key(ent);
-    for (u64 i = b; i < e; ++i) {
-      u64 ent_n = ent;
+    cur = chunk_bucket[t];
+    u32 end = ends[cur], end_n = ends[cur < last ? cur + 1 : last];
+    for (u32 i = (u32)b; i < (u32)e; ++i) {
+      u32 ent_n = ent;
       Gen g_n = g;
-      if (i + 1 < e) {
+      if (i + 1 < (u32)e) {
         ent_n = entries[i + 1];
         g_n = load_gen<kUnit>(entry_gen(ent_n));
       }
-      const u32 k = entry_key(ent);
       const bool negate = entry_negate(ent);
+      const bool boundary = i >= end;
+      if (boundary) {
+        close_run(t, cur, acc, writer, first_seg);
+        ++cur;
+        end = end_n;
+        if (i >= end) {
+          cur = bucket_after(i, cur + 1);
+          end = ends[cur];
+        }
+        end_n = ends[cur < last ? cur + 1 : last];
+      }
       if (kUniform) {
-        if (i == b || k != cur) {
-          if (i != b) {
-            close_run(t, cur, acc, writer, first_seg);
-            cur = k;
-          }
+        if (i == b || boundary)
           acc = C::identity();
-        }
         C::template add_gen<X>(acc, acc, g, negate, kUnit);
       } else {
-        const bool start = i == b || k != cur;
-        if (k != cur) {
-          close_run(t, cur, acc, writer, first_seg);
-          cur = k;
-        }
-        if (start)
+        if (i == b || boundary)
           C::gen_to_point(acc, g, negate);
         else
           C::template add_gen<X>(acc, acc, g, negate, kUnit);
@@ -1248,6 +1311,7 @@
   const ColumnDesc* d_cols = nullptr;
   const u64* d_col_start = nullptr;
   u64 total_terms = 0, max_entries = 0;
+  u64 max_gen = 0;
   u32 max_windows = 0;
   StagedRange(stream_t s, const MsmPlan& plan, u64 begin, u64 end) {
     const u32 ncols = plan.ncols;
@@ -1260,6 +1324,9 @@
       col_start[j + 1] = col_start[j] + cols[j].n;
       max_entries += (u64)cols[j].n * cols[j].num_windows;
       max_windows = std::max(max_windows, cols[j].n ? cols[j].num_windows : 0u);
+      if (cols[j].n)
+        max_gen = std::max<u64>(max_gen, (u64)cols[j].gen_base + cols[j].n - 1 +
+                                             (u64)(cols[j].num_windows - 1) * cols[j].table_n);
     }
     total_terms = col_start[ncols];
     if (total_terms == 0)
@@ -1276,7 +1343,7 @@
 };
 
 struct SortedLayout {
-  u64* entries;
+  u32* entries;
   u32* counts;
   u32* starts;
   u32* d_m;
@@ -1293,13 +1360,13 @@
   out.slots_max = L ? ((max_entries + nkeys * ((1ull << L) - 1) + (1ull << L) - 1) >> L) << L : max_entries;
   out.counts = (u32*)dev_alloc((nkeys + 1) * sizeof(u32), s);
   out.d_m = (u32*)dev_alloc(16 * sizeof(u32), s);
-  out.entries = (u64*)dev_alloc(out.slots_max * sizeof(u64), s);
+  out.entries = (u32*)dev_alloc(out.slots_max * sizeof(u32), s);
 #ifdef B200_BINNED_SORT
-  out.binned = L == 0 && opt.sort_path != 0 && binned_sort_shift(nkeys) <= kMaxBinShift &&
+  out.binned = L == 0 && opt.sort_path != 0 && binned_span_micro(nkeys, r.max_gen) != 0 &&
                (opt.sort_path == 2 || max_entries >= kBinnedSortMinEntries);
   if (out.binned)
     binned_sort(s, r.d_cols, r.d_col_start, ncols, c, nbuckets, total_terms, max_entries,
-                r.max_windows, nkeys, out.entries, out.counts, out.d_m);
+                r.max_windows, r.max_gen, nkeys, out.entries, out.counts, out.d_m);
 #endif
   if (!out.binned) {
     dev_zero(out.counts, (nkeys + 1) * sizeof(u32), s);
@@ -1337,12 +1404,12 @@
   opt.sort_path = 2;
   const SortedLayout b = sort_entries(s, plan, r, 0, opt, window_used.p);
   std::vector<u32> ca(nkeys + 1), cb(nkeys + 1), m(1);
-  std::vector<u64> ea(M), eb(M);
+  std::vector<u32> ea(M), eb(M);
   copy_d2h(ca.data(), a.counts, (nkeys + 1) * sizeof(u32), s);
   copy_d2h(cb.data(), b.counts, (nkeys + 1) * sizeof(u32), s);
   copy_d2h(m.data(), b.d_m, sizeof(u32), s);
-  copy_d2h(ea.data(), a.entries, M * sizeof(u64), s);
-  copy_d2h(eb.data(), b.entries, M * sizeof(u64), s);
+  copy_d2h(ea.data(), a.entries, M * sizeof(u32), s);
+  copy_d2h(eb.data(), b.entries, M * sizeof(u32), s);
   stream_sync(s);
   for (void* p : {(void*)a.entries, (void*)a.counts, (void*)a.d_m, (void*)b.entries, (void*)b.counts,
                   (void*)b.d_m, (void*)r.d_cols})
@@ -1379,6 +1446,7 @@
   const u32 chunkn = std::max(opt.chunkn, 4u);
   const u32* lvl_keys = nullptr;
   const Point* lvl_pieces = nullptr;
+  u32* chunk_bucket = nullptr;
   stream_t cs = s;
   for (int level = 0;; ++level) {
     const bool final_level = walk.m_max <= K;
@@ -1388,11 +1456,14 @@
     to_free.insert(to_free.end(), {out_keys, out_pieces});
     u32* out_m = d_m + 1 + (level % 8);
     const auto launch_level = [&](auto body, u64 threads, stream_t st) {
-      body = {lvl_keys, walk.entries, walk.gens, lvl_pieces, walk.m_ptr, K, final_level, target,
-              out_keys, out_pieces, out_m, unit_veto};
+      body = {lvl_keys, walk.entries, walk.ends, walk.nkeys, chunk_bucket, walk.gens, lvl_pieces,
+              walk.m_ptr, K, final_level, target, out_keys, out_pieces, out_m, unit_veto};
       launch(body, threads, st);
     };
     if (level == 0) {
+      chunk_bucket = (u32*)dev_alloc(T * sizeof(u32), s);
+      to_free.push_back(chunk_bucket);
+      launch(ChunkBucketBody{walk.ends, walk.nkeys, walk.m_ptr, K, chunk_bucket}, T, s);
       const bool uniform =
           opt.uniform_add == 2 ? C::kCurveId == kRistretto255 : opt.uniform_add != 0;
       constexpr bool kEd = C::kCurveId == kRistretto255;
@@ -1451,7 +1522,7 @@
   B200_LOG(3, "range [%llu, %llu): %llu terms, %llu entries max, c=%u, %llu keys, pair levels %u",
            (unsigned long long)begin, (unsigned long long)end, (unsigned long long)r.total_terms,
            (unsigned long long)max_entries, plan.c, (unsigned long long)nkeys, L);
-  WalkInput<C> walk{gens, sorted.entries, sorted.d_m, max_entries};
+  WalkInput<C> walk{gens, sorted.entries, sorted.counts, nkeys, sorted.d_m, max_entries};
   std::vector<void*> to_free;
   if (hook)
     hook->before_accumulate();
@@ -1459,9 +1530,9 @@
   StageRange nvtx_acc("msm: bucket accumulation");
   if constexpr (C::kBatchAffine) {
     if (L) {
-      walk = run_pair_levels<C>(s, L, sorted.entries, gens, sorted.d_m, sorted.slots_max,
-                                opt.pair_batch);
-      to_free = {(void*)walk.gens, (void*)walk.entries};
+      walk = run_pair_levels<C>(s, L, sorted.entries, sorted.starts, nkeys, gens, sorted.d_m,
+                                sorted.slots_max, opt.pair_batch);
+      to_free = {(void*)walk.gens, (void*)walk.entries, (void*)walk.ends};
     }
   }
   typedef typename C::Point Point;
diff --git a/include/blitzar_b200.h b/include/blitzar_b200.h
--- a/include/blitzar_b200.h
+++ b/include/blitzar_b200.h
@@ -181,7 +181,7 @@
 unsigned b200_field_op(unsigned field, unsigned op, uint64_t n, const uint32_t* a,
                        const uint32_t* b, uint32_t* out);
 unsigned b200_selftest_sort(const struct sxt_sequence_descriptor* columns, unsigned num,
-                            unsigned window_bits);
+                            unsigned window_bits, unsigned generator_offset);
 void b200_profile_accumulate(int enable);
 void b200_profile_read(float* total_ms, unsigned* launches);
 void b200_set_tuning(unsigned window_bits, unsigned chunk1, unsigned chunkn);
```
